# cc-ai/climategan

Measured on AMD Instinct MI355X. Metric: 640x640 images/sec (G+D step): per-domain sample slots per second of the joint Masker+Painter training step (update_G + update_D), global batch 32 per domain, higher is better.
Workload: dtype bf16

## Files before the change

climategan_amd/_lib.py:

```python
import ctypes as C
import os
from pathlib import Path

_HERE = Path(__file__).resolve().parent
LIB_PATH = Path(os.environ["CGAN_LIB"]).resolve() if os.environ.get("CGAN_LIB") else _HERE / "libcgan_hip.so"

CGAN_F16, CGAN_BF16, CGAN_F32 = 0, 1, 2
ACT_NONE, ACT_RELU, ACT_LRELU, ACT_TANH, ACT_SIGMOID = 0, 1, 2, 3, 4
PAD_ZERO, PAD_REFLECT = 0, 1
ABI_VERSION = 1


class ConvDesc(C.Structure):
    _fields_ = [
        ("dtype", C.c_int32), ("n", C.c_int32), ("h_in", C.c_int32), ("w_in", C.c_int32),
        ("c_in", C.c_int32), ("c_out", C.c_int32),
        ("kh", C.c_int32), ("kw", C.c_int32), ("stride", C.c_int32), ("pad", C.c_int32), ("dilation", C.c_int32),
        ("pad_mode", C.c_int32), ("h_out", C.c_int32), ("w_out", C.c_int32), ("in_upsample", C.c_int32),
        ("act", C.c_int32), ("act_slope", C.c_float), ("has_bias", C.c_int32), ("has_residual", C.c_int32),
        ("residual_upsample", C.c_int32),
    ]


class NormStatsDesc(C.Structure):
# ... 131 lines not shown
    "cgan_norm_act_apply": (C.c_int, [_P, _P, _P, _P, C.POINTER(NormStatsDesc), C.c_int32, C.c_float, _P]),
    "cgan_make_m_cond_bwd_nhwc": (C.c_int, [_P, _P, _P, _P, _P, C.c_int32, C.c_int32, C.c_int32, C.c_int32, C.c_int32,
                                            C.c_int32, _P]),
    "cgan_resize_nearest_bwd_nhwc": (C.c_int, [_P, _P, C.c_int32, C.c_int32, C.c_int32, C.c_int32, C.c_int32, C.c_int32,
                                               C.c_int32, C.c_int32, C.c_int32, _P]),
    "cgan_norm_add_act_apply": (C.c_int, [_P, _P, _P, _P, _P, C.POINTER(NormStatsDesc), C.c_int32, C.c_float, _P]),
    "cgan_spade_packed_weight_bytes": (C.c_size_t, [C.POINTER(SpadeDesc)]),
    "cgan_spade_pack_weights": (C.c_int, [_P, _P, _P, _P, _P, _P, _P, C.POINTER(SpadeDesc), _P]),
    "cgan_spade_fused_fwd": (C.c_int, [_P, _P, _P, _P, _P, _P, C.POINTER(SpadeDesc), _P]),
    "cgan_spade_fused_fwd_train": (C.c_int, [_P, _P, _P, _P, _P, _P, _P, C.POINTER(SpadeDesc), _P]),
    "cgan_spectral_norm_workspace_bytes": (C.c_size_t, [C.c_int32, C.c_int32]),
    "cgan_spectral_norm_power_iter": (C.c_int, [_P, _P, _P, _P, C.c_int32, C.c_int32, _P, C.c_size_t, _P]),
    "cgan_spectral_norm_power_iter_batched": (C.c_int, [_P, C.c_int32, C.c_int32, C.c_int32, _P]),
    "cgan_extra_adam_multi_tensor": (C.c_int, [_P, C.c_int32, C.c_int64, C.c_int32, C.c_int32, C.c_int32, C.c_double,
                                               C.c_double, C.c_double, C.c_double, C.c_double, _P]),
    "cgan_grads_nonfinite_check_multi_tensor": (C.c_int, [_P, C.c_int32, C.c_int64, C.c_double, C.c_int32, _P, _P]),
    "cgan_adam_multi_tensor": (C.c_int, [_P, C.c_int32, C.c_int64] + [C.c_double] * 6 + [_P, _P]),
    "cgan_rmsprop_multi_tensor": (C.c_int, [_P, C.c_int32, C.c_int64] + [C.c_double] * 5 + [_P, _P]),
    "cgan_amp_optim_finish": (C.c_int, [_P, C.c_int32, _P, _P]),
    "cgan_nchw_to_nhwc": (C.c_int, [_P, _P, _P, C.c_int32, C.c_int32, C.c_int32, C.c_int32, C.c_int32, C.c_int32, _P]),
    "cgan_nhwc_to_nchw": (C.c_int, [_P, _P, _P, _P, C.c_int32, C.c_int32, C.c_int32, C.c_int32, C.c_int32, C.c_int32, _P]),
    "cgan_resize_nearest_nhwc": (C.c_int, [_P, _P, C.c_int32, C.c_int32, C.c_int32, C.c_int32, C.c_int32, C.c_int32,
                                           C.c_int32, C.c_int32, C.c_int32, _P]),
    "cgan_avgpool3x3s2_nhwc": (C.c_int, [_P, _P, C.c_int32, C.c_int32, C.c_int32, C.c_int32, C.c_int32, _P]),
    "cgan_maxpool3x3s2_nhwc": (C.c_int, [_P, _P, C.c_int32, C.c_int32, C.c_int32, C.c_int32, C.c_int32, _P]),
    "cgan_resize_bilinear_nhwc": (C.c_int, [_P, _P, C.c_int32, C.c_int32, C.c_int32, C.c_int32, C.c_int32, C.c_int32,
                                            C.c_int32, C.c_int32, _P]),
    "cgan_resize_bicubic_nhwc": (C.c_int, [_P, _P, C.c_int32, C.c_int32, C.c_int32, C.c_int32, C.c_int32, C.c_int32,
                                           C.c_int32, _P]),
    "cgan_sumpool2x2_nhwc": (C.c_int, [_P, _P, C.c_int32, C.c_int32, C.c_int32, C.c_int32, C.c_int32, _P]),
    "cgan_reflect_pad_bwd_nhwc": (C.c_int, [_P, _P, C.c_int32, C.c_int32, C.c_int32, C.c_int32, C.c_int32, C.c_int32, _P]),
    "cgan_copy_channels_nhwc": (C.c_int, [_P, _P, C.c_int64, C.c_int32, C.c_int32, C.c_int32, C.c_int32, _P]),
    "cgan_eltwise_nhwc": (C.c_int, [_P, _P, _P, C.c_int32, C.c_int32, C.c_int64, _P]),
    "cgan_fold_bn": (C.c_int, [_P, _P, _P, _P, _P, _P, C.c_float, _P, _P, C.c_int32, C.c_int64, _P]),
    "cgan_act_bwd": (C.c_int, [_P, _P, _P, C.c_int32, C.c_int32, C.c_float, C.c_int64, _P]),
    "cgan_instnorm_act_bwd_workspace_bytes": (C.c_size_t, [C.POINTER(NormStatsDesc)]),
    "cgan_instnorm_act_bwd": (C.c_int, [_P, _P, _P, _P, C.POINTER(NormStatsDesc), C.c_int32, C.c_float, _P, C.c_size_t,
                                        _P]),
    "cgan_spade_bwd_prepare": (C.c_int, [_P, _P, _P, _P, _P, _P, _P, _P, _P, C.POINTER(SpadeDesc), _P]),
    "cgan_spade_hidden_bwd_workspace_bytes": (C.c_size_t, [C.POINTER(SpadeDesc)]),
    "cgan_spade_hidden_bwd": (C.c_int, [_P, _P, _P, _P, _P, _P, _P, _P, C.c_size_t, C.POINTER(SpadeDesc), _P]),
    "cgan_batchnorm_train_stats": (C.c_int, [_P, _P, _P, C.c_float, _P, _P, _P, _P, _P, _P, _P, C.POINTER(NormStatsDesc), _P,
                                             C.c_size_t, _P]),
    "cgan_batchnorm_train_stats_from_partials": (C.c_int, [_P, C.c_int32, _P, _P, C.c_float, _P, _P, _P, _P, _P, _P, _P,
                                                           C.POINTER(NormStatsDesc), _P]),
    "cgan_conv2d_stats_chunk_pixels": (C.c_int32, [C.POINTER(ConvDesc)]),
    "cgan_conv2d_nhwc_fwd_stats": (C.c_int, [_P, _P, _P, _P, _P, C.c_size_t, C.POINTER(ConvDesc), _P]),
    "cgan_bn_train_prepare": (C.c_int, [_P, _P, _P, _P, C.c_float, C.c_float, C.c_int64, _P, _P, _P, _P, _P, C.c_int32, _P]),
    "cgan_batchnorm_act_bwd_workspace_bytes": (C.c_size_t, [C.c_int32]),
    "cgan_batchnorm_act_bwd": (C.c_int, [_P, _P, _P, _P, _P, _P, _P, _P, _P, _P, _P, _P, C.c_int32, C.c_int64, C.c_int32,
                                         C.c_int32, C.c_float, _P, C.c_size_t, _P]),
    "cgan_batchnorm_act_bwd_grouped": (C.c_int, [_P, _P, _P, _P, _P, _P, _P, _P, _P, _P, _P, _P, C.c_int32, C.c_int64,
                                                 C.c_int32, C.c_int32, C.c_int32, C.c_float, _P, C.c_size_t, _P]),
    "cgan_bce_logits_nhwc": (C.c_int, [_P, C.c_int32, C.c_int64, C.c_int32, C.c_float, C.c_float, _P, _P, _P]),
    "cgan_hinge_nhwc": (C.c_int, [_P, C.c_int32, C.c_int64, C.c_int32, C.c_int32, C.c_int32, C.c_float, _P, _P, _P]),
    "cgan_l1_nhwc": (C.c_int, [_P, _P, C.c_int32, C.c_int64, C.c_float, _P, _P, _P]),
    "cgan_mse_const_nhwc": (C.c_int, [_P, C.c_int32, C.c_int64, C.c_int32, C.c_float, C.c_float, _P, _P, _P]),
    "cgan_painter_aux_losses": (C.c_int, [_P, _P, _P, C.c_int32, C.c_int32, C.c_int32, C.c_int32, C.c_float, C.c_float,
                                          C.c_float, C.c_float, _P, _P, _P]),
    "cgan_resize_bicubic_bwd_nhwc": (C.c_int, [_P, _P, C.c_int32, C.c_int32, C.c_int32, C.c_int32, C.c_int32, C.c_int32,
                                               C.c_int32, _P]),
    "cgan_spectral_norm_bwd": (C.c_int, [_P, _P, _P, _P, _P, C.c_int32, C.c_int32, _P, _P]),
    "cgan_painter_heads_fwd": (C.c_int, [_P, _P, _P, _P, _P, C.c_int32, C.c_int32, C.c_int32, C.c_int32, _P]),
    "cgan_painter_heads_bwd": (C.c_int, [_P, _P, _P, _P, C.c_int32, C.c_int32, C.c_int32, C.c_int32, _P]),
    "cgan_diffaug_fwd": (C.c_int, [_P, _P, _P, _P, C.c_int32, C.c_int32, C.c_int32, C.c_int32, C.c_int32, C.c_int32,
                                   C.c_int32, _P, _P]),
    "cgan_diffaug_bwd": (C.c_int, [_P, _P, _P, _P, C.c_int32, C.c_int32, C.c_int32, C.c_int32, C.c_int32, C.c_int32,
                                   C.c_int32, _P, _P]),
    "cgan_painter_heads_diffaug_fwd": (C.c_int, [_P, _P, _P, _P, _P, _P, _P, C.c_int32, C.c_int32, C.c_int32, C.c_int32,
                                                 C.c_int32, C.c_int32, C.c_int32, _P, _P]),
    "cgan_painter_heads_diffaug_bwd": (C.c_int, [_P, _P, _P, _P, _P, _P, C.c_int32, C.c_int32, C.c_int32, C.c_int32,
                                                 C.c_int32, C.c_int32, C.c_int32, _P, _P]),
    "cgan_data_transform": (C.c_int, [_P, _P, C.c_int32, C.c_int32, C.c_int32, C.c_int32, _P, _P, _P, C.c_int32, _P, _P]),
    "cgan_data_source_minmax": (C.c_int, [_P, _P, C.c_int32, C.c_int32, _P, _P]),
    "cgan_data_jitter": (C.c_int, [_P, _P, _P, C.c_int32, C.c_int32, C.c_int32, C.c_int32, _P, _P, _P, _P]),
    "cgan_avgpool3x3s2_bwd_nhwc": (C.c_int, [_P, _P, C.c_int32, C.c_int32, C.c_int32, C.c_int32, C.c_int32, _P]),
    "cgan_maxpool2x2_nhwc": (C.c_int, [_P, _P, C.c_int32, C.c_int32, C.c_int32, C.c_int32, C.c_int32, _P]),
    "cgan_maxpool2x2_bwd_nhwc": (C.c_int, [_P, _P, _P, C.c_int32, C.c_int32, C.c_int32, C.c_int32, C.c_int32, _P]),
    "cgan_maxpool2x2_relu_bwd_nhwc": (C.c_int, [_P, _P, _P, C.c_int32, C.c_int32, C.c_int32, C.c_int32, C.c_int32, _P]),
    "cgan_softmax_nhwc": (C.c_int, [_P, _P, C.c_int32, C.c_int64, C.c_int32, _P]),
    "cgan_softmax_bwd_nhwc": (C.c_int, [_P, _P, _P, C.c_int32, C.c_int64, C.c_int32, _P]),
    "cgan_sigmoid_pair_nhwc": (C.c_int, [_P, _P, C.c_int32, C.c_int64, _P]),
    "cgan_sigmoid_pair_bwd_nhwc": (C.c_int, [_P, _P, _P, C.c_int32, C.c_int64, _P]),
    "cgan_softmax_ce_nhwc": (C.c_int, [_P, _P, C.c_int32, C.c_int64, C.c_int32, C.c_float, _P, _P, _P]),
    "cgan_tv_nhwc": (C.c_int, [_P, C.c_int32, C.c_int32, C.c_int32, C.c_int32, C.c_int32, C.c_float, C.c_float, _P, _P, _P]),
    "cgan_advent_entropy_pair_nhwc": (C.c_int, [_P, _P, _P, C.c_int32, C.c_int64, C.c_int32, C.c_int32, _P]),
    "cgan_entropy_pair_from_nchw": (C.c_int, [_P, _P, _P, C.c_int32, C.c_int32, C.c_int32, C.c_int32, C.c_int32, _P]),
    "cgan_entropy_pair_from_nchw_bwd": (C.c_int, [_P, _P, _P, _P, C.c_int32, C.c_int32, C.c_int32, C.c_int32, C.c_int32, _P]),
    "cgan_advent_entropy_pair_bwd_nhwc": (C.c_int, [_P, _P, _P, _P, C.c_int32, C.c_int64, C.c_int32, C.c_int32, _P]),
    "cgan_entropy_map_nhwc": (C.c_int, [_P, _P, _P, C.c_int32, C.c_int64, C.c_int32, _P]),
    "cgan_entropy_map_bwd_nhwc": (C.c_int, [_P, _P, _P, _P, C.c_int32, C.c_int64, C.c_int32, _P]),
    "cgan_minent_nhwc": (C.c_int, [_P, C.c_int32, C.c_int64, C.c_int32, C.c_int32, C.c_float, C.c_float, _P, _P, _P, _P]),
    "cgan_bce_logits_map_nhwc": (C.c_int, [_P, _P, C.c_int32, C.c_int64, C.c_float, _P, _P, _P]),
    "cgan_ground_intersection_nhwc": (C.c_int, [_P, _P, C.c_int32, C.c_int64, C.c_float, _P, _P]),
    "cgan_affine_sum_nhwc": (C.c_int, [_P, C.c_int32, C.c_int64, C.c_int32, C.c_float, C.c_float, _P, _P, _P]),
    "cgan_resize_bilinear_bwd_workspace_bytes": (C.c_size_t, [C.c_int32] * 4),
    "cgan_resize_bilinear_bwd_nhwc": (C.c_int, [_P, _P] + [C.c_int32] * 8 + [_P, C.c_size_t, _P]),
    "cgan_maxpool3x3s2_bwd_nhwc": (C.c_int, [_P, _P, _P, C.c_int32, C.c_int32, C.c_int32, C.c_int32, C.c_int32, _P]),
    "cgan_add_act_nhwc": (C.c_int, [_P, _P, _P, C.c_int32, C.c_int32, C.c_float, C.c_int64, _P]),
    "cgan_slice_channels_nhwc": (C.c_int, [_P, _P, C.c_int64, C.c_int32, C.c_int32, C.c_int32, _P]),
    "cgan_sigm_loss_workspace_bytes": (C.c_size_t, [C.c_int32, C.c_int32, C.c_int32]),
    "cgan_sigm_loss_nhwc": (C.c_int, [_P, _P, C.c_int32, C.c_int32, C.c_int32, C.c_int32, C.c_float, C.c_int32, C.c_float,
                                      _P, _P, _P, C.c_size_t, _P]),
    "cgan_normalize_u8_workspace_bytes": (C.c_size_t, [C.c_int32]),
    "cgan_normalize_u8_nhwc": (C.c_int, [_P, C.c_int32, _P, C.c_int32, C.c_int32, C.c_int32, C.c_int32, _P, C.c_size_t,
                                         _P]),
# ... 133 lines not shown
```

climategan_amd/autograd.py:

```python
import ctypes as C

import os

import torch

from . import ops


GRAD_SCALE = 1.0


def set_grad_scale(s: float):
    global GRAD_SCALE
    GRAD_SCALE = float(s)


BN_GROUPS = 1


class bn_groups:

    def __init__(self, groups: int):
        self.groups = int(groups)

# ... 87 lines not shown
        ctx.cfg = (c, x_t.shape[1], x_t.shape[2], x_t.shape[3])
        return ops.resize_nearest(ops.NHWC(x_t, c), size, cs_out=cs_out).t

    @staticmethod
    def backward(ctx, dy_t):
        c, h, w, cs = ctx.cfg
        return ops.resize_nearest_bwd(ops.NHWC(dy_t.contiguous(), c), (h, w), cs).t, None, None, None


class ConvFn(torch.autograd.Function):

    @staticmethod
    def forward(ctx, x_t, weight, bias, res_t, packed, cfg, sn):
        x = ops.NHWC(x_t, cfg["c_in"])
        res = ops.NHWC(res_t, weight.shape[0]) if res_t is not None else None
        if cfg.get("mask_input") and (cfg.get("in_upsample", False) or cfg.get("pair_in", False)):
            raise NotImplementedError("ConvFn: mask_input with a folded upsample / a pair map")
        if cfg.get("want_stats") and res is None and cfg["act"] == ops.ACT_NONE and not cfg.get("in_upsample", False):
            y, cfg["stats_out"] = ops.conv2d_with_stats(x, packed, stride=cfg["stride"], pad=cfg["pad"],
                                                        dilation=cfg["dilation"], pad_mode=cfg.get("pad_mode", ops.PAD_ZERO),
                                                        groups=BN_GROUPS)
        else:
            y = ops.conv2d(x, packed, stride=cfg["stride"], pad=cfg["pad"], dilation=cfg["dilation"], act=cfg["act"],
                           slope=cfg["slope"], residual=res, in_upsample=cfg.get("in_upsample", False),
                           residual_upsample=cfg.get("residual_upsample", False),
                           pad_mode=cfg.get("pad_mode", ops.PAD_ZERO))
        ctx.cfg = cfg
        ctx.has_bias = bias is not None
        ctx.has_res = res_t is not None
        ctx.premasked = False
        ctx.sn = None if sn is None else (tuple(sn) if cfg.get("sn_owned") else tuple(t.clone() for t in sn))
        ctx.dgrad = None
        if ctx.needs_input_grad[0] and not cfg.get("pair_in", False):
            ctx.dgrad = ops.dgrad_register(weight, ctx.sn[0] if ctx.sn is not None else None, x_t.dtype, cfg["stride"])
        ctx.save_for_backward(x_t, weight, y.t if cfg["act"] != ops.ACT_NONE else None)
        return y.t

    @staticmethod
    def backward(ctx, dy_t):
        cfg = ctx.cfg
        x_t, weight, y_t = ctx.saved_tensors
        c_out = weight.shape[0]
        ups = cfg.get("in_upsample", False)
        dy = ops.NHWC(dy_t.contiguous(), c_out)
        if y_t is not None and not ctx.premasked:
            dy = ops.act_bwd(ops.NHWC(y_t, c_out), dy, cfg["act"], cfg["slope"])
        sigma = ctx.sn[0] if ctx.sn is not None else None
        dx_t = dres_t = None
        pair = cfg.get("pair_in", False)
        w_eff = torch.cat([weight.detach(), weight.detach()], 1) if pair else weight
        if ctx.needs_input_grad[0]:
            h_in, w_in = (x_t.shape[1] * 2, x_t.shape[2] * 2) if ups else (x_t.shape[1], x_t.shape[2])
            relu_out = ops.NHWC(x_t, cfg["c_in"]) if cfg.get("mask_input") else None
            dx = ops.conv2d_bwd_data(dy, w_eff, (x_t.shape[0], h_in, w_in), stride=cfg["stride"], pad=cfg["pad"],
                                     dilation=cfg["dilation"], sigma=sigma, pad_mode=cfg.get("pad_mode", ops.PAD_ZERO),
                                     prepacked=ctx.dgrad, relu_out=relu_out)
            dx_t = (ops.sumpool2x2(dx) if ups else dx).t
        if ctx.has_res and ctx.needs_input_grad[3]:
            dres_t = (ops.sumpool2x2(dy) if cfg.get("residual_upsample", False) else dy).t
        dw = db = None
        if ctx.needs_input_grad[1] or (ctx.has_bias and ctx.needs_input_grad[2]):
            def wgrad():
                dw, db = ops.conv2d_bwd_weight(ops.NHWC(x_t, cfg["c_in"]), dy, tuple(w_eff.shape), stride=cfg["stride"],
                                               pad=cfg["pad"], dilation=cfg["dilation"], want_bias=ctx.has_bias,
                                               in_upsample=ups, pad_mode=cfg.get("pad_mode", ops.PAD_ZERO))
                if pair:
                    dw = dw[:, :weight.shape[1]] + dw[:, weight.shape[1]:]
                if ctx.sn is not None:
                    dw = ops.spectral_norm_bwd(dw, weight.detach(), ctx.sn[1], ctx.sn[2], ctx.sn[0])
                return dw, db
            dw, db = wgrad()
        return dx_t, dw, db, dres_t, None, None, None


class ConvPassFn(torch.autograd.Function):

    @staticmethod
    def forward(ctx, x_t, weight, bias, packed, cfg):
        x = ops.NHWC(x_t, cfg["c_in"])
        if cfg.get("want_stats") and cfg.get("act", ops.ACT_NONE) != ops.ACT_NONE:
            raise NotImplementedError("ConvPassFn: the statistics epilogue belongs to a conv without an activation")
        if cfg.get("want_stats"):
            y, cfg["stats_out"] = ops.conv2d_with_stats(x, packed, stride=cfg["stride"], pad=cfg["pad"],
                                                        dilation=cfg["dilation"], pad_mode=cfg.get("pad_mode", ops.PAD_ZERO),
                                                        groups=BN_GROUPS)
        else:
            y = ops.conv2d(x, packed, stride=cfg["stride"], pad=cfg["pad"], dilation=cfg["dilation"],
                           act=cfg.get("act", ops.ACT_NONE), slope=cfg.get("slope", 0.0),
                           pad_mode=cfg.get("pad_mode", ops.PAD_ZERO))
        ctx.cfg = cfg
        ctx.has_bias = bias is not None
        ctx.premasked = False
        ctx.dgrad = ops.dgrad_register(weight, None, x_t.dtype, cfg["stride"]) if ctx.needs_input_grad[0] else None
        ctx.save_for_backward(x_t, weight, y.t if cfg.get("act", ops.ACT_NONE) != ops.ACT_NONE else None)
        return y.t, x_t

    @staticmethod
    def backward(ctx, dy_t, dpass_t):
        cfg = ctx.cfg
        x_t, weight, y_t = ctx.saved_tensors
        c_out = weight.shape[0]
        dy = ops.NHWC(dy_t.contiguous(), c_out)
        if y_t is not None and not ctx.premasked:
            dy = ops.act_bwd(ops.NHWC(y_t, c_out), dy, cfg["act"], cfg.get("slope", 0.0))
        dx_t = None
        if ctx.needs_input_grad[0]:
            add = ops.NHWC(dpass_t.contiguous(), cfg["c_in"]) if dpass_t is not None else None
            relu_out = ops.NHWC(x_t, cfg["c_in"]) if cfg.get("mask_input") else None
            dx_t = ops.conv2d_bwd_data(dy, weight, (x_t.shape[0], x_t.shape[1], x_t.shape[2]), stride=cfg["stride"],
                                       pad=cfg["pad"], dilation=cfg["dilation"],
                                       pad_mode=cfg.get("pad_mode", ops.PAD_ZERO), add=add, prepacked=ctx.dgrad,
                                       relu_out=relu_out).t
        dw = db = None
        if ctx.needs_input_grad[1] or (ctx.has_bias and ctx.needs_input_grad[2]):
            dw, db = ops.conv2d_bwd_weight(
                ops.NHWC(x_t, cfg["c_in"]), dy, tuple(weight.shape), stride=cfg["stride"], pad=cfg["pad"],
                dilation=cfg["dilation"], want_bias=ctx.has_bias, pad_mode=cfg.get("pad_mode", ops.PAD_ZERO))
        return dx_t, dw, db, None, None


class InstNormActFn(torch.autograd.Function):

    @staticmethod
    def forward(ctx, x_t, c, eps, act, slope):
        x = ops.NHWC(x_t, c)
        mean, rstd = ops.instnorm_stats(x, eps=eps)
        out = ops.norm_act_apply(x, mean, rstd, act=act, slope=slope)
        ctx.c, ctx.act, ctx.slope = c, act, slope
        ctx.save_for_backward(out.t, rstd)
        return out.t

    @staticmethod
    def backward(ctx, dy_t):
        out_t, rstd = ctx.saved_tensors
        dx = ops.instnorm_act_bwd(ops.NHWC(out_t, ctx.c), ops.NHWC(dy_t.contiguous(), ctx.c), rstd, act=ctx.act,
                                  slope=ctx.slope)
        return dx.t, None, None, None, None


_SPADE_REMAT_GAMMA = os.environ.get("CGAN_SPADE_REMAT_GAMMA") == "1"


_SPADE_FUSED_BWD = os.environ.get("CGAN_SPADE_FUSED_BWD", "1") != "0"


class SpadeFn(torch.autograd.Function):

    @staticmethod
    def forward(ctx, x_t, cond_t, mean, rstd, w_sh, b_sh, w_g, b_g, w_b, b_b, packed, cfg):
        x = ops.NHWC(x_t, cfg["c"])
        cond = ops.NHWC(cond_t, cfg["cond_c"])
        gamma_t = None
        if _SPADE_REMAT_GAMMA or not any(ctx.needs_input_grad):
            y = ops.spade_fused(x, mean, rstd, cond, packed, act=cfg["act"], slope=cfg["slope"],
                                x_upsample=cfg["x_upsample"])
        else:
            y, gamma = ops.spade_fused(x, mean, rstd, cond, packed, act=cfg["act"], slope=cfg["slope"],
                                       x_upsample=cfg["x_upsample"], want_gamma=True)
            gamma_t = gamma.t
        ctx.cfg = cfg
        ctx.save_for_backward(x_t, cond_t, mean, rstd, y.t, w_sh, b_sh, w_g, b_g, w_b, b_b, gamma_t)
        return y.t

    @staticmethod
    def backward(ctx, dy_t):
# ... 121 lines not shown
        ctx.c, ctx.hw = c, (x_t.shape[1], x_t.shape[2])
        return ops.avgpool3x3s2(ops.NHWC(x_t, c)).t

    @staticmethod
    def backward(ctx, dy_t):
        return ops.avgpool3x3s2_bwd(ops.NHWC(dy_t.contiguous(), ctx.c), ctx.hw).t, None


class MaxPool2x2Fn(torch.autograd.Function):

    @staticmethod
    def forward(ctx, x_t, c, mask_input=False):
        ctx.c = c
        ctx.mask_input = bool(mask_input)
        ctx.save_for_backward(x_t)
        return ops.maxpool2x2(ops.NHWC(x_t, c)).t

    @staticmethod
    def backward(ctx, dy_t):
        (x_t,) = ctx.saved_tensors
        return ops.maxpool2x2_bwd(ops.NHWC(x_t, ctx.c), ops.NHWC(dy_t.contiguous(), ctx.c), relu_input=ctx.mask_input).t, None, None


_BN_BWD_READS_OUT = os.environ.get("CGAN_BN_BWD_OUT") == "1"


class BatchNormActFn(torch.autograd.Function):

    @staticmethod
    def forward(ctx, x_t, gamma, beta, running_mean, running_var, c, eps, momentum, act, slope, nbt=None, res_t=None,
                conv_stats=None):
        n, h, w, cs = x_t.shape
        G = BN_GROUPS
        if n % G:
            raise ValueError("BatchNormActFn: batch %d does not divide into %d groups" % (n, G))
        npix = n * h * w // G
        x_t = x_t.contiguous()
        flat = ops.NHWC(x_t.view(G, npix, 1, cs), c)
        if conv_stats is not None and npix % conv_stats.chunk_pixels == 0:
            mean, rstd, mean_f, rstd_f = ops.batchnorm_train_stats_from_partials(
                conv_stats, G, npix, c, gamma, beta, running_mean, running_var, nbt, eps, momentum)
        else:
            mean, rstd, mean_f, rstd_f = ops.batchnorm_train_stats(flat, gamma, beta, running_mean, running_var, nbt, eps,
                                                                   momentum)
        res = None
        if res_t is not None:
            if res_t.shape != x_t.shape:
                raise ValueError("BatchNormActFn: residual %s does not match %s" % (tuple(res_t.shape), tuple(x_t.shape)))
            res = ops.NHWC(res_t.contiguous().view(G, npix, 1, cs), c)
        out = ops.norm_act_apply(flat, mean_f, rstd_f, act=act, slope=slope, residual=res).t.view(n, h, w, cs)
        ctx.cfg = (c, act, slope, G)
        ctx.has_res = res_t is not None
        ctx.premasked = False
        keep_out = res_t is not None or _BN_BWD_READS_OUT
        ctx.save_for_backward(x_t, out if keep_out else None, mean, rstd, gamma,
                              None if keep_out else mean_f, None if keep_out else rstd_f)
        return out

    @staticmethod
    def backward(ctx, dy_t):
        from . import _lib
        lib = _lib.load()
        x_t, out, mean, rstd, gamma, mean_f, rstd_f = ctx.saved_tensors
        c, act, slope, G = ctx.cfg
        if ctx.premasked:
            act = ops.ACT_NONE
        n, h, w, cs = x_t.shape
        nbytes = G * lib.cgan_batchnorm_act_bwd_workspace_bytes(c)
        ws = torch.empty(nbytes, dtype=torch.uint8, device=x_t.device)
        dx = torch.empty_like(x_t)
        want_res = ctx.has_res and ctx.needs_input_grad[11]
        dy_t = dy_t.contiguous()
        if want_res and act == ops.ACT_NONE:
            dres = dy_t
        else:
            dres = torch.empty_like(x_t) if want_res else None
        dg = db = None
        if gamma is not None:
            dg, db = torch.empty((2, c), dtype=torch.float32, device=x_t.device).unbind(0)
        _lib.check(lib.cgan_batchnorm_act_bwd_grouped(
            ops._ptr(x_t), ops._ptr(out), ops._ptr(dy_t), ops._ptr(mean), ops._ptr(rstd), ops._ptr(gamma),
            ops._ptr(mean_f), ops._ptr(rstd_f), ops._ptr(dx), ops._ptr(dg), ops._ptr(db), ops._ptr(dres) if dres is not None and dres is not dy_t else None,
            ops._DT[x_t.dtype], n * h * w, c, G, act, slope, ops._ptr(ws), nbytes, ops._stream()),
            "cgan_batchnorm_act_bwd_grouped")
        return dx, dg, db, None, None, None, None, None, None, None, None, dres, None


def claim_relu_mask(out_t: torch.Tensor) -> bool:
    fn = out_t.grad_fn
    if fn is None:
        return False
    if isinstance(fn, BatchNormActFn._backward_cls):
        if not fn.has_res or fn.cfg[1] != ops.ACT_RELU:
            return False
    elif isinstance(fn, (ConvFn._backward_cls, ConvPassFn._backward_cls)):
        if fn.cfg.get("act", ops.ACT_NONE) != ops.ACT_RELU:
            return False
    else:
        return False
    fn.premasked = True
    return True


def _scaled(dx, c, g):
    return None if dx is None else ops.scale_by_scalar(ops.NHWC(dx, c), g.reshape(1).float().contiguous()).t


class PainterAuxFn(torch.autograd.Function):

    @staticmethod
    def forward(ctx, fake_t, x, m, lam_tv, lam_ctx, lam_rec):
        from . import _lib
        n, h, w = fake_t.shape[0], fake_t.shape[1], fake_t.shape[2]
        x = x.contiguous().float()
        m = m.contiguous().float()
        cnt = float(n * 3 * h * w)
        wh = GRAD_SCALE * lam_tv * 2.0 / (3 * (h - 1) * w) / n
        ww = GRAD_SCALE * lam_tv * 2.0 / (3 * h * (w - 1)) / n
        acc = torch.zeros(3, dtype=torch.float32, device=fake_t.device)
        dfake = torch.empty_like(fake_t) if ctx.needs_input_grad[0] else None
        _lib.check(_lib.load().cgan_painter_aux_losses(ops._ptr(fake_t), ops._ptr(x), ops._ptr(m), ops._DT[fake_t.dtype], n, h, w,
                                                       wh, ww, GRAD_SCALE * lam_ctx / cnt, GRAD_SCALE * lam_rec / cnt,
                                                       ops._ptr(acc), ops._ptr(dfake), ops._stream()), "cgan_painter_aux_losses")
        ctx.save_for_backward(dfake)
        if GRAD_SCALE != 1.0:
            acc = acc / GRAD_SCALE
        ctx.mark_non_differentiable(acc)
        return acc.sum(), acc

    @staticmethod
    def backward(ctx, g, _g_parts):
        (dfake,) = ctx.saved_tensors
        return _scaled(dfake, 3, g), None, None, None, None, None


class ResizeBicubicFn(torch.autograd.Function):

    @staticmethod
# ... 363 lines not shown
```

climategan_amd/csrc/cgan_common.h:

```cpp
#pragma once
#include <hip/hip_runtime.h>
#include <stdarg.h>
#include <stdint.h>
#include <stdio.h>

#include "climategan_hip.h"

void cgan_set_error(const char* fmt, ...);

#define CGAN_REQUIRE(cond, ...)            \
  do {                                     \
    if (!(cond)) {                         \
      cgan_set_error(__VA_ARGS__);         \
      return CGAN_ERR_BAD_ARG;             \
    }                                      \
  } while (0)

#define CGAN_CHECK_LAUNCH(name)                                                    \
  do {                                                                             \
    hipError_t e__ = hipGetLastError();                                            \
    if (e__ != hipSuccess) {                                                       \
      cgan_set_error("%s: HIP launch failed: %s", name, hipGetErrorString(e__));   \
      return CGAN_ERR_HIP;                                                         \
    }                                                                              \
  } while (0)

__device__ __forceinline__ float cgan_res_apply(float v, float r, int mode) { return mode == 2 ? (r > 0.f ? v : 0.f) : v + r; }
__device__ __forceinline__ float cgan_res_apply3(float v, float r, float m) { return m > 0.f ? v + r : 0.f; }

#ifdef CGAN_DEV
#define CGAN_KNOB(type, name, init) type name = init
#define CGAN_DEV_ONLY(...) __VA_ARGS__
#define CGAN_DBG(p) ((p).dbg)
#define CGAN_TSBUF(p) ((p).tsbuf)
#else
#define CGAN_KNOB(type, name, init) [[maybe_unused]] constexpr type name = init
#define CGAN_DEV_ONLY(...)
#define CGAN_DBG(p) 0
#define CGAN_TSBUF(p) ((unsigned long long*)nullptr)
#endif

#ifndef CGAN_NO_NT
#define CGAN_LD_STREAM(p) __builtin_nontemporal_load(p)
#define CGAN_ST_STREAM(v, p) __builtin_nontemporal_store(v, p)
#else
#define CGAN_LD_STREAM(p) (*(p))
#define CGAN_ST_STREAM(v, p) (*(p) = (v))
#endif

typedef _Float16 f16x8 __attribute__((ext_vector_type(8)));
typedef __bf16 bf16x8 __attribute__((ext_vector_type(8)));
typedef float f32x4 __attribute__((ext_vector_type(4)));
typedef unsigned int u32x4 __attribute__((ext_vector_type(4)));
typedef unsigned int u32x2 __attribute__((ext_vector_type(2)));

struct F16 {
  using scalar = _Float16;
  using vec8 = f16x8;
  static constexpr int id = CGAN_F16;
};
struct BF16 {
  using scalar = __bf16;
  using vec8 = bf16x8;
  static constexpr int id = CGAN_BF16;
};

template <typename T> struct Split;
template <> struct Split<F16> {
  static constexpr int NC = 2, NB = 3, NS = 2;
  __host__ __device__ static constexpr int xcomp(int b) { return b == 1 ? 1 : 0; }
  __host__ __device__ static constexpr int wcomp(int b) { return b == 2 ? 1 : 0; }
};
template <> struct Split<BF16> {
  static constexpr int NC = 3, NB = 6, NS = 3;
  __host__ __device__ static constexpr int xcomp(int b) { return b == 1 || b == 4 ? 1 : (b == 2 ? 2 : 0); }
  __host__ __device__ static constexpr int wcomp(int b) { return b < 3 ? 0 : (b < 5 ? 1 : 2); }
};
static inline int cgan_split_blocks(int dtype) { return dtype == CGAN_BF16 ? 6 : 3; }
static inline int cgan_split_store_blocks(int dtype) { return dtype == CGAN_BF16 ? 3 : 2; }

__device__ __forceinline__ f32x4 mfma16(f16x8 a, f16x8 b, f32x4 c) {
// ... 69 lines not shown
```

climategan_amd/csrc/conv_gemm.h:

```cpp
#pragma once
#include "cgan_common.h"

struct ConvGemmArgs {
  const uint16_t* x;
  const u32x4* w;
  const float* bias;
  const uint16_t* res;
  const uint16_t* res2;
  uint16_t* y;
  int n, h_in, w_in, cin_s;
  int cout, cout_s, ctiles, ksteps;
  int kh, kw, stride, pad, dil, pad_mode;
  int h_out, w_out, npix;
  int act, has_res, res_ups;
  float slope;
  float* stats;
};

struct ConvGemmCls {
  int koff;
  int kh, kw;
  int offy, offx;
};
struct ConvGemmExtArgs {
  ConvGemmArgs a;
  int cls_s;
  int ksplit;
  int ks_per;
  float* ws;
  int pair;
  ConvGemmCls cls[4];
};
bool conv_gemm_ext_shape_ok(const ConvGemmArgs& a);
int conv_gemm_splitk_plan(const ConvGemmArgs& a);
size_t conv_gemm_splitk_workspace_bytes(const ConvGemmArgs& a, int ksplit);
int conv_gemm_splitk_launch(const ConvGemmArgs& a, int ksplit, float* ws, int dtype, hipStream_t s);
int conv_gemm_cls_launch(const ConvGemmArgs& a, int cls_s, const ConvGemmCls* cls, int dtype, hipStream_t s);
int conv_gemm_pair_launch(const ConvGemmArgs& a, int dtype, hipStream_t s);

bool conv_gemm_applicable(const CganConvDesc* d);
int conv_gemm_launch(const ConvGemmArgs& a, int dtype, hipStream_t s);
bool conv_gemm_res2_ok(const ConvGemmArgs& a, int dtype);
int conv_gemm_stats_chunk_pixels(const ConvGemmArgs& a, int dtype);
bool conv_gemm_big_ok(const ConvGemmArgs& a);
bool conv1x1_allc_ok(const ConvGemmArgs& a);
int conv1x1_allc_launch(const ConvGemmArgs& a, int dtype, hipStream_t s);
int conv_gemm_big_launch(const ConvGemmArgs& a, int dtype, hipStream_t s);
bool conv_gemm_big_pair_ok(const ConvGemmArgs& a, int dtype);
int conv_gemm_big_pair_launch(const ConvGemmArgs& a, int dtype, hipStream_t s);
bool conv1x1_xres_ok(const ConvGemmArgs& a);
int conv1x1_xres_launch(const ConvGemmArgs& a, int dtype, hipStream_t s);

#ifdef __HIPCC__
typedef float f32x2 __attribute__((ext_vector_type(2)));

__device__ __forceinline__ float row16_sum(float v) {
  v += __builtin_bit_cast(float, __builtin_amdgcn_update_dpp(0, __builtin_bit_cast(int, v), 0x128, 0xf, 0xf, false));
  v += __builtin_bit_cast(float, __builtin_amdgcn_update_dpp(0, __builtin_bit_cast(int, v), 0x124, 0xf, 0xf, false));
  v += __builtin_bit_cast(float, __builtin_amdgcn_update_dpp(0, __builtin_bit_cast(int, v), 0x122, 0xf, 0xf, false));
  v += __builtin_bit_cast(float, __builtin_amdgcn_update_dpp(0, __builtin_bit_cast(int, v), 0x121, 0xf, 0xf, false));
  return v;
}

template <typename T, int WC, int WP>
__device__ __forceinline__ void conv_gemm_stats_epilogue(f32x4 (&acc)[WC][WP], const ConvGemmArgs& p, int cout_base,
                                                         int chunk, int j, int g) {
  if (p.bias) {
#pragma unroll
    for (int c = 0; c < WC; ++c) {
      const int chb = cout_base + c * 16 + 4 * g;
      const f32x4 b = chb < p.cout_s ? *reinterpret_cast<const f32x4*>(p.bias + chb) : (f32x4){0.f, 0.f, 0.f, 0.f};
#pragma unroll
      for (int t = 0; t < WP; ++t) acc[c][t] += b;
    }
  }
  constexpr float inv_cnt = 1.f / (float)(WP * 16);
#pragma unroll
  for (int c = 0; c < WC; ++c) {
    f32x2 vr[WP][2];
#pragma unroll
    for (int t = 0; t < WP; ++t) {
#pragma unroll
      for (int hh = 0; hh < 2; ++hh) {
        float r0, r1;
        unpack2<T>(pack2<T>(acc[c][t][2 * hh], acc[c][t][2 * hh + 1]), r0, r1);
        vr[t][hh] = (f32x2){r0, r1};
      }
    }
    f32x2 s0[2] = {vr[0][0], vr[0][1]};
#pragma unroll
    for (int t = 1; t < WP; ++t) {
      s0[0] += vr[t][0];
      s0[1] += vr[t][1];
    }
    float sm[4], sq[4];
#pragma unroll
    for (int r = 0; r < 4; ++r) sm[r] = row16_sum(s0[r >> 1][r & 1]) * inv_cnt;
    const f32x2 m2[2] = {(f32x2){sm[0], sm[1]}, (f32x2){sm[2], sm[3]}};
    f32x2 s1[2];
#pragma unroll
    for (int hh = 0; hh < 2; ++hh) {
      const f32x2 dv = vr[0][hh] - m2[hh];
      s1[hh] = dv * dv;
    }
#pragma unroll
    for (int t = 1; t < WP; ++t)
#pragma unroll
      for (int hh = 0; hh < 2; ++hh) {
        const f32x2 dv = vr[t][hh] - m2[hh];
        s1[hh] += dv * dv;
      }
#pragma unroll
    for (int r = 0; r < 4; ++r) sq[r] = row16_sum(s1[r >> 1][r & 1]);
    const int ch = cout_base + c * 16 + 4 * g;
    if (j == 0 && ch < p.cout_s) {
      float o[8];
#pragma unroll
      for (int r = 0; r < 4; ++r) {
        o[2 * r] = sm[r];
        o[2 * r + 1] = sq[r];
      }
      float* dst = p.stats + ((size_t)chunk * p.cout_s + ch) * 2;
      *reinterpret_cast<f32x4*>(dst) = (f32x4){o[0], o[1], o[2], o[3]};
      *reinterpret_cast<f32x4*>(dst + 4) = (f32x4){o[4], o[5], o[6], o[7]};
    }
  }
}

template <typename T, int WC, int WP, int PP, bool RES2 = false>
__device__ __forceinline__ void conv_gemm_staged_store(const f32x4 (&acc)[WC][WP], const ConvGemmArgs& p,
                                                       unsigned char* stg, int pix0, int cout_base, const float* bias_ep,
                                                       int lane, int j, int g) {
  constexpr int ROWB = WC * 64 + 16;
  constexpr int CH = WC * 2;
  constexpr int NIT = PP * 16 * CH / 64;
  constexpr int NPASS = WP / PP;
  constexpr int PSTEP = 64 / CH;
  static_assert(64 % CH == 0 && WP % PP == 0, "a lane keeps its channel chunk over the iterations");
  const int qc = lane % CH, pl0 = lane / CH;
  const int ch = cout_base + qc * 8;
  const bool ch_ok = ch < p.cout_s;
  const bool plain = !bias_ep && !p.has_res && p.act == CGAN_ACT_NONE && p.cout == p.cout_s;
  f32x4 bb0 = (f32x4){0.f, 0.f, 0.f, 0.f}, bb1 = bb0;
  if (bias_ep && ch_ok) {
    bb0 = *reinterpret_cast<const f32x4*>(bias_ep + ch);
    bb1 = *reinterpret_cast<const f32x4*>(bias_ep + ch + 4);
  }
  u32x4 rv[NPASS][NIT];
  u32x4 rm[RES2 ? (NPASS > 1 ? 2 : 1) : 1][RES2 ? NIT : 1];
  auto load_rm = [&](int pass, u32x4 (&dst)[RES2 ? NIT : 1]) {
#pragma unroll
    for (int it = 0; it < (RES2 ? NIT : 0); ++it) {
      const int pix = pix0 + pass * PP * 16 + it * PSTEP + pl0;
      dst[it] = (u32x4){0u, 0u, 0u, 0u};
      if (pix < p.npix && ch_ok) dst[it] = CGAN_LD_STREAM(reinterpret_cast<const u32x4*>(p.res2 + (size_t)pix * p.cout_s + ch));
    }
  };
  if (p.has_res) {
#pragma unroll
    for (int pass = 0; pass < NPASS; ++pass)
#pragma unroll
      for (int it = 0; it < NIT; ++it) {
        const int pix = pix0 + pass * PP * 16 + it * PSTEP + pl0;
        rv[pass][it] = (u32x4){0u, 0u, 0u, 0u};
        if (pix < p.npix && ch_ok) {
          size_t rbase;
          if (p.res_ups) {
            const int ox = pix % p.w_out;
            const int r = pix / p.w_out;
            const int oy = r % p.h_out;
            const int nn = r / p.h_out;
            rbase = (((size_t)nn * (p.h_out >> 1) + (oy >> 1)) * (p.w_out >> 1) + (ox >> 1)) * p.cout_s;
          } else {
            rbase = (size_t)pix * p.cout_s;
          }
          rv[pass][it] = CGAN_LD_STREAM(reinterpret_cast<const u32x4*>(p.res + rbase + ch));
        }
      }
    if (RES2 && p.has_res == 3) load_rm(0, rm[0]);
    __builtin_amdgcn_sched_barrier(0);
  }
#pragma unroll
  for (int pass = 0; pass < NPASS; ++pass) {
#pragma unroll
    for (int tt = 0; tt < PP; ++tt)
#pragma unroll
      for (int c = 0; c < WC; ++c)
        *reinterpret_cast<f32x4*>(stg + (tt * 16 + j) * ROWB + c * 64 + g * 16) = acc[c][pass * PP + tt];
    asm volatile("s_waitcnt lgkmcnt(0)" ::: "memory");
    if (RES2 && NPASS > 1 && p.has_res == 3 && pass + 1 < NPASS) {
      __builtin_amdgcn_sched_barrier(0);
      load_rm(pass + 1, rm[(pass + 1) & 1]);
      __builtin_amdgcn_sched_barrier(0);
    }
    if (pass == 0 || (RES2 && p.has_res == 3 && pass >= 2)) __builtin_amdgcn_s_waitcnt(0x0F70);
#pragma unroll
    for (int it = 0; it < NIT; ++it) {
      const int pl = it * PSTEP + pl0;
      const int pix = pix0 + pass * PP * 16 + pl;
      const f32x4 v0 = *reinterpret_cast<const f32x4*>(stg + pl * ROWB + qc * 32);
      const f32x4 v1 = *reinterpret_cast<const f32x4*>(stg + pl * ROWB + qc * 32 + 16);
      float v[8] = {v0[0], v0[1], v0[2], v0[3], v1[0], v1[1], v1[2], v1[3]};
      if (!plain) {
        if (bias_ep) {
#pragma unroll
          for (int r = 0; r < 4; ++r) {
            v[r] += bb0[r];
            v[4 + r] += bb1[r];
          }
        }
        if (RES2 && p.has_res == 3) {
#pragma unroll
          for (int e = 0; e < 4; ++e) {
            float r0, r1, m0, m1;
            unpack2<T>(rv[pass][it][e], r0, r1);
            unpack2<T>(rm[RES2 && NPASS > 1 ? (pass & 1) : 0][RES2 ? it : 0][e], m0, m1);
            v[2 * e] = cgan_res_apply3(v[2 * e], r0, m0);
            v[2 * e + 1] = cgan_res_apply3(v[2 * e + 1], r1, m1);
          }
        } else if (p.has_res) {
#pragma unroll
          for (int e = 0; e < 4; ++e) {
            float r0, r1;
            unpack2<T>(rv[pass][it][e], r0, r1);
            v[2 * e] = cgan_res_apply(v[2 * e], r0, p.has_res);
            v[2 * e + 1] = cgan_res_apply(v[2 * e + 1], r1, p.has_res);
          }
        }
        act_apply_n(v, p.act, p.slope);
        if (p.cout < p.cout_s) {
#pragma unroll
          for (int r = 0; r < 8; ++r)
            if (ch + r >= p.cout) v[r] = 0.f;
        }
      }
      u32x4 o;
#pragma unroll
      for (int e = 0; e < 4; ++e) o[e] = pack2<T>(v[2 * e], v[2 * e + 1]);
      if (pix < p.npix && ch_ok) CGAN_ST_STREAM(o, reinterpret_cast<u32x4*>(p.y + (size_t)pix * p.cout_s + ch));
    }
    asm volatile("s_waitcnt lgkmcnt(0)" ::: "memory");
  }
}
#endif
```

climategan_amd/csrc/conv_gemm.hip:

```cpp
#include "conv_gemm.h"
#include <type_traits>

namespace {

__device__ __attribute__((aligned(16))) unsigned int g_gemm_zeros[4];

constexpr int NSTAGE = 3;
CGAN_KNOB(int, g_gemm_ws, 0);

__device__ __forceinline__ int reflect_i(int i, int n) {
  if (i < 0) i = -i;
  if (i >= n) i = 2 * n - 2 - i;
  return i;
}

template <typename T, int WAVES_C, int WC, int WP, bool REFLECT, int NS = NSTAGE, bool RES2 = false>
__global__ __launch_bounds__(256, 2) void conv_gemm_kernel(ConvGemmArgs p, int npb, int ncb) {
  constexpr int WAVES_P = 4 / WAVES_C;
  constexpr int CT_BLK = WAVES_C * WC;
  constexpr int PT_BLK = WAVES_P * WP;
  constexpr int STAGE_BYTES = (CT_BLK + PT_BLK) * 1024;
  constexpr int W_PER_WAVE = CT_BLK / 4;
  constexpr int P_PER_WAVE = PT_BLK / 4;
  constexpr int DMA_PER_WAVE = W_PER_WAVE + P_PER_WAVE;
  static_assert(CT_BLK % 4 == 0 && PT_BLK % 4 == 0, "tiles must split evenly over the 4 waves");
  extern __shared__ __attribute__((aligned(1024))) unsigned char smem[];

  const int lane = threadIdx.x & 63;
  const int wave = __builtin_amdgcn_readfirstlane(threadIdx.x >> 6);
  const int j = lane & 15;
  const int g = lane >> 4;
  const int wc = wave % WAVES_C, wp = wave / WAVES_C;

  const int xcd = blockIdx.x & 7, slot = blockIdx.x >> 3;
  const int cblk = slot % ncb;
  const int pblk = xcd * ((npb + 7) >> 3) + slot / ncb;
  if (pblk >= npb) return;

  int pbase[P_PER_WAVE], py0[P_PER_WAVE], px0[P_PER_WAVE];
#pragma unroll
  for (int m = 0; m < P_PER_WAVE; ++m) {
    int pix = (pblk * PT_BLK + wave + 4 * m) * 16 + j;
    bool v = pix < p.npix;
    int pc = v ? pix : 0;
    int ox = pc % p.w_out;
    int r = pc / p.w_out;
    int oy = r % p.h_out;
    int nn = r / p.h_out;
    pbase[m] = nn * p.h_in * p.w_in * p.cin_s + g * 8;
    py0[m] = v ? oy * p.stride - p.pad : -(1 << 28);
    px0[m] = ox * p.stride - p.pad;
  }
  const int ccn = p.cin_s >> 5;
  const long zero_off = reinterpret_cast<const unsigned char*>(g_gemm_zeros) - reinterpret_cast<const unsigned char*>(p.x);

  int i_ky = 0, i_kx = 0, i_cc = 0, i_buf = 0;
  auto issue_piece = [&](int piece) {
    unsigned char* buf = smem + i_buf * STAGE_BYTES;
    if (piece < W_PER_WAVE) {
      const int i = wave + 4 * piece;
      const int ct = min(cblk * CT_BLK + i, p.ctiles - 1);
      const u32x4* src = p.w + ((size_t)ct * p.ksteps + (i_ky * p.kw + i_kx) * ccn + i_cc) * 64 + lane;
      __builtin_amdgcn_global_load_lds((const __attribute__((address_space(1))) void*)src,
                                       (__attribute__((address_space(3))) void*)(buf + i * 1024), 16, 0, 0);
    } else {
      const int m = piece - W_PER_WAVE;
      const int i = wave + 4 * m;
      int iy = py0[m] + i_ky * p.dil, ix = px0[m] + i_kx * p.dil;
      bool ok;
// ... 26 lines not shown
    for (int q = 0; q < DMA_PER_WAVE; ++q) issue_piece(q);
    issue_advance();
  };

  f32x4 acc[WC][WP];
#pragma unroll
  for (int c = 0; c < WC; ++c)
#pragma unroll
    for (int t = 0; t < WP; ++t) acc[c][t] = (f32x4){0.f, 0.f, 0.f, 0.f};

  issue();
  if (NS > 2) issue();
  int r_buf = 0;
  for (int ks = 0; ks < p.ksteps; ++ks) {
    asm volatile("s_waitcnt vmcnt(%0) lgkmcnt(0)" ::"n"((NS - 2) * DMA_PER_WAVE) : "memory");
    __builtin_amdgcn_s_barrier();
    const unsigned char* buf = smem + r_buf * STAGE_BYTES;
    u32x4 a[WC], b[WP];
#pragma unroll
    for (int t = 0; t < WP; ++t)
      b[t] = *reinterpret_cast<const u32x4*>(buf + (CT_BLK + wp * WP + t) * 1024 + lane * 16);
#pragma unroll
    for (int c = 0; c < WC; ++c) a[c] = *reinterpret_cast<const u32x4*>(buf + (wc * WC + c) * 1024 + lane * 16);
    constexpr int NM = WC * WP;
    constexpr int GAP = NM / (DMA_PER_WAVE + 1);
    __builtin_amdgcn_sched_barrier(0);
#pragma unroll
    for (int i = 0; i < NM; ++i) {
      const int c = i / WP, t = i % WP;
      acc[c][t] = mfma16(as_vec8<T>(a[c]), as_vec8<T>(b[t]), acc[c][t]);
      if ((i + 1) % GAP == 0 && (i + 1) / GAP <= DMA_PER_WAVE) {
        issue_piece((i + 1) / GAP - 1);
        __builtin_amdgcn_sched_barrier(0);
      }
    }
    issue_advance();
    r_buf = (r_buf + 1 == NS) ? 0 : r_buf + 1;
  }

  constexpr int ROWB = WC * 64 + 16;
  constexpr int PP = (4 * 4 * 16 * ROWB <= NS * STAGE_BYTES && WP % 4 == 0) ? 4
                     : (4 * 2 * 16 * ROWB <= NS * STAGE_BYTES ? 2 : 1);
  static_assert(4 * PP * 16 * ROWB <= NS * STAGE_BYTES, "epilogue staging does not fit");
  static_assert(WP % PP == 0, "WP must be a multiple of PP");
  asm volatile("s_waitcnt vmcnt(0) lgkmcnt(0)" ::: "memory");
  __builtin_amdgcn_s_barrier();
  unsigned char* stg = smem + wave * (PP * 16 * ROWB);
  const int cout_base = (cblk * CT_BLK + wc * WC) * 16;
  const float* bias_ep = p.bias;
  if (p.stats && (pblk * PT_BLK + wp * WP) * 16 < p.npix) {
    conv_gemm_stats_epilogue<T, WC, WP>(acc, p, cout_base, pblk * WAVES_P + wp, j, g);
    if (p.bias) bias_ep = nullptr;
  }
  conv_gemm_staged_store<T, WC, WP, PP, RES2>(acc, p, stg, (pblk * PT_BLK + wp * WP) * 16, cout_base, bias_ep, lane, j, g);
}

template <typename T, int WC, int WP>
__global__ __launch_bounds__(512, 2) void conv_gemm_k64_kernel(ConvGemmArgs p, int npb, int ncb, int tiles_total) {
  constexpr int CT_BLK = 2 * WC, PT_BLK = 2 * WP;
  constexpr int W_BYTES = CT_BLK * 2048, STAGE_BYTES = (CT_BLK + PT_BLK) * 2048;
  constexpr int NS = 3;
  constexpr int W_PER = CT_BLK / 2, P_PER = PT_BLK / 2, PIECES = W_PER + P_PER;
  static_assert(PIECES <= 63, "vmcnt range");
  extern __shared__ __attribute__((aligned(1024))) unsigned char smem[];

  const int lane = threadIdx.x & 63;
  const int wave = __builtin_amdgcn_readfirstlane(threadIdx.x >> 6);
  const int xcd = blockIdx.x & 7, slot = blockIdx.x >> 3, nslot = gridDim.x >> 3;
  const int per = (tiles_total + 7) >> 3;
  const int t0 = xcd * per;
  const int t1 = min(t0 + per, tiles_total);
  const int my_n = (t1 - t0 > slot) ? (t1 - t0 - slot + nslot - 1) / nslot : 0;
  if (my_n <= 0) return;
  const int first = t0 + slot;
  const int cc2n = p.cin_s >> 6;
  const int n_st = p.kh * p.kw * cc2n;
  const int n_it = my_n * n_st;

  if (wave >= 4) {
    const int pw = wave - 4;
    const int half = pw & 1;
    const int ccn = p.cin_s >> 5;
    const long zero_off = reinterpret_cast<const unsigned char*>(g_gemm_zeros) - reinterpret_cast<const unsigned char*>(p.x);
    const int q = lane >> 3;
    const int kchunk = (lane & 7) ^ (4 * half + ((q >> 1) & 3));
    int poff[P_PER];
    unsigned vmask[P_PER];
    const u32x4* wtile[W_PER];
    auto set_tile = [&](int ti) {
      const int gt = first + ti * nslot;
      const int pblk = gt / ncb;
      const int cblk = gt - pblk * ncb;
#pragma unroll
      for (int m = 0; m < W_PER; ++m)
        wtile[m] = p.w + (size_t)min(cblk * CT_BLK + (pw >> 1) + 2 * m, p.ctiles - 1) * p.ksteps * 64 + half * 64 + lane;
#pragma unroll
      for (int m = 0; m < P_PER; ++m) {
        const int pix = (pblk * PT_BLK + (pw >> 1) + 2 * m) * 16 + 8 * half + q;
        const bool v = pix < p.npix;
        const int pc = v ? pix : 0;
        const int ox = pc % p.w_out;
        const int r = pc / p.w_out;
        const int oy = r % p.h_out;
        const int nn = r / p.h_out;
        const int py0 = oy * p.stride - p.pad, px0 = ox * p.stride - p.pad;
        poff[m] = ((nn * p.h_in * p.w_in + py0 * p.w_in + px0) * p.cin_s + kchunk * 8) * 2;
        unsigned mk = 0;
// ... 156 lines not shown
#pragma unroll
        for (int r = 0; r < 4; ++r) {
          v[r] = act_apply(v[r], p.act, p.slope);
          if (ch + r >= p.cout) v[r] = 0.f;
        }
        u32x2 o;
        o.x = pack2<T>(v[0], v[1]);
        o.y = pack2<T>(v[2], v[3]);
        CGAN_ST_STREAM(o, reinterpret_cast<u32x2*>(p.y + (size_t)pix * p.cout_s + ch));
      }
    }
  };

  for (int ti = 0; ti < my_n; ++ti) {
    first_read(ti > 0);
    for (int st = 0; st + 1 < n_st; ++st) {
      step(a0, b0, a1, b1, 1);
      step(a1, b1, a0, b0, 0);
    }
    step(a0, b0, a1, b1, 1);
    step(a1, b1, a0, b0, -1);
    epilogue(ti);
  }
}

template <typename T, int WC, int WP>
int launch_k64(const ConvGemmArgs& a, hipStream_t s) {
  constexpr int CT_BLK = 2 * WC, PT_BLK = 2 * WP;
  constexpr size_t smem = (size_t)3 * (CT_BLK + PT_BLK) * 2048;
  static bool attr_set = false;
  if (!attr_set) {
    hipError_t e = hipFuncSetAttribute(reinterpret_cast<const void*>(&conv_gemm_k64_kernel<T, WC, WP>),
                                       hipFuncAttributeMaxDynamicSharedMemorySize, 160 * 1024);
    if (e != hipSuccess) {
      cgan_set_error("conv_gemm_k64: hipFuncSetAttribute failed: %s", hipGetErrorString(e));
      return CGAN_ERR_HIP;
    }
    attr_set = true;
  }
  const int npb = ceil_div(ceil_div(a.npix, 16), PT_BLK);
  const int ncb = ceil_div(a.ctiles, CT_BLK);
  const int tiles = npb * ncb;
  const int per = ceil_div(tiles, 8);
  const int nslot = per < 32 ? per : 32;
  hipLaunchKernelGGL((conv_gemm_k64_kernel<T, WC, WP>), dim3(8 * nslot), dim3(512), smem, s, a, npb, ncb, tiles);
  return CGAN_OK;
}
bool k64_ok(const ConvGemmArgs& a) {
  return (a.cin_s & 63) == 0 && a.pad_mode != CGAN_PAD_REFLECT && a.kh * a.kw <= 32 &&
         (long)a.n * a.h_in * a.w_in * a.cin_s < (1L << 30) - (1L << 20);
}


template <typename T, int WAVES_C, int WC, int WP, bool REFLECT, int NS = NSTAGE, bool RES2 = false>
int launch_cfg2(const ConvGemmArgs& a, hipStream_t s) {
  constexpr int WAVES_P = 4 / WAVES_C;
  constexpr int CT_BLK = WAVES_C * WC, PT_BLK = WAVES_P * WP;
  constexpr size_t smem = (size_t)NS * (CT_BLK + PT_BLK) * 1024;
  static bool attr_set = false;
  if (!attr_set) {
    hipError_t e = hipFuncSetAttribute(reinterpret_cast<const void*>(&conv_gemm_kernel<T, WAVES_C, WC, WP, REFLECT, NS, RES2>),
                                       hipFuncAttributeMaxDynamicSharedMemorySize, 160 * 1024);
    if (e != hipSuccess) {
      cgan_set_error("conv_gemm: hipFuncSetAttribute failed: %s", hipGetErrorString(e));
      return CGAN_ERR_HIP;
    }
    attr_set = true;
  }
  const int npb = ceil_div(ceil_div(a.npix, 16), PT_BLK);
  const int ncb = ceil_div(a.ctiles, CT_BLK);
  const int grid = ceil_div(npb, 8) * 8 * ncb;
  hipLaunchKernelGGL((conv_gemm_kernel<T, WAVES_C, WC, WP, REFLECT, NS, RES2>), dim3(grid), dim3(256), smem, s, a, npb, ncb);
  return CGAN_OK;
}

template <typename T, int WAVES_C, int WC, int WP, int NS = NSTAGE>
int launch_cfg(const ConvGemmArgs& a, hipStream_t s) {
  return a.pad_mode == CGAN_PAD_REFLECT ? launch_cfg2<T, WAVES_C, WC, WP, true, NS>(a, s)
                                        : launch_cfg2<T, WAVES_C, WC, WP, false, NS>(a, s);
}

CGAN_KNOB(int, g_gemm_cfg, 0);

enum { KIND_PLAIN = 0, KIND_K64_256x128, KIND_K64_128x256, KIND_BIG, KIND_DIRECT, KIND_XRES };
struct Choice {
  int kind;
  int cfg;
};

Choice choose(const ConvGemmArgs& a, bool bf16) {
  const int ptiles = ceil_div(a.npix, 16);
  const bool no_big = g_gemm_ws == 9;
  const bool no_xres = g_gemm_ws == 9 || g_gemm_ws == 12;
  const int ws = (no_big || no_xres || g_gemm_ws == 13 || g_gemm_ws == 14) ? 0 : g_gemm_ws;
  switch (ws) {
    case 5: if (k64_ok(a)) return {KIND_K64_256x128, 0}; break;
    case 6: if (k64_ok(a)) return {KIND_K64_128x256, 0}; break;
    case 8: if (conv_gemm_big_ok(a)) return {KIND_BIG, 0}; break;
    case 10: if (conv1x1_allc_ok(a)) return {KIND_DIRECT, 0}; break;
    case 11: if (conv1x1_xres_ok(a)) return {KIND_XRES, 0}; break;
    default: break;
  }
  const bool automatic = ws == 0 && g_gemm_cfg == 0;
  (void)bf16;
  if (automatic && !no_big && conv1x1_allc_ok(a) && a.ctiles <= 4 && a.npix >= 16384) return {KIND_DIRECT, 0};
  if (automatic && !no_xres && conv1x1_xres_ok(a) && a.ctiles >= 16 && a.npix >= 16384) return {KIND_XRES, 0};
  const bool long_1x1 = a.kh * a.kw == 1 && g_gemm_ws != 13 &&
                        (g_gemm_ws == 14 ? (a.cin_s >= 2048 || (a.cin_s >= 512 && a.ctiles >= 128))
                                         : (a.cin_s >= 1024 || (a.cin_s >= 512 && a.ctiles >= 128)));
  if (automatic && !no_big && conv_gemm_big_ok(a) && a.npix >= 16384 &&
      ((a.cin_s * a.kh * a.kw >= 4096 && a.cin_s >= 512 && !(a.kh * a.kw >= 9 && a.cin_s >= 2048)) || long_1x1))
    return {KIND_BIG, 0};
  if (automatic && k64_ok(a) && a.kh * a.kw >= 9 && a.cin_s >= 512 && a.npix >= 16384) return {KIND_K64_256x128, 0};
  switch (g_gemm_cfg) {
    case 1: return {KIND_PLAIN, 1};
    case 2: if (a.ctiles <= 16) return {KIND_PLAIN, 2}; break;
    case 3: return {KIND_PLAIN, 3};
    case 4: return {KIND_PLAIN, 4};
    case 5: return {KIND_PLAIN, 5};
    default: break;
  }
  if (a.ctiles <= 4) return {KIND_PLAIN, 1};
  if (a.kh * a.kw == 1 && a.ksteps <= 16) return {KIND_PLAIN, 5};
  if (a.ctiles > 8 && a.ctiles <= 16 && ceil_div(ptiles, 8) >= 384) return {KIND_PLAIN, 2};
  if ((long)ceil_div(ptiles, 16) * ceil_div(a.ctiles, 8) >= 384) return {KIND_PLAIN, 3};
  return {KIND_PLAIN, 4};
}

template <typename T>
int launch(const ConvGemmArgs& a, hipStream_t s) {
  const Choice ch = choose(a, std::is_same<T, BF16>::value);
  switch (ch.kind) {
    case KIND_K64_256x128: return launch_k64<T, 8, 4>(a, s);
    case KIND_K64_128x256: return launch_k64<T, 4, 8>(a, s);
    case KIND_BIG: return conv_gemm_big_launch(a, T::id, s);
    case KIND_DIRECT: return conv1x1_allc_launch(a, T::id, s);
    case KIND_XRES: return conv1x1_xres_launch(a, T::id, s);
    default: break;
  }
  switch (ch.cfg) {
    case 1: return launch_cfg<T, 1, 4, 4>(a, s);
    case 2: return launch_cfg<T, 2, 8, 4>(a, s);
    case 3: return launch_cfg<T, 2, 4, 8>(a, s);
    case 5:
      if (a.has_res == 3) return launch_cfg2<T, 2, 4, 4, false, 2, true>(a, s);
      return launch_cfg<T, 2, 4, 4, 2>(a, s);
    default: return launch_cfg<T, 2, 4, 4>(a, s);
  }
}

}

bool conv_gemm_applicable(const CganConvDesc* d) {
  const int cin_s = cgan_cs(d->c_in), cout_s = cgan_cs(d->c_out);
  const long npix = (long)d->n * d->h_out * d->w_out;
  const long in_elems = (long)d->n * d->h_in * d->w_in * cin_s;
  return (cin_s % 32) == 0 && cout_s >= 64 && !d->in_upsample && npix >= 2048 && in_elems < (1L << 31) - (1L << 20) &&
         (long)ceil_div((int)ceil_div((int)npix, 16), 8) * ceil_div(ceil_div(cout_s, 16), 8) >= 128;
}

CGAN_DEV_ONLY(extern "C" void cgan_debug_set_gemm_cfg(int v) { g_gemm_cfg = v; })
CGAN_DEV_ONLY(extern "C" void cgan_debug_set_gemm_ws(int v) { g_gemm_ws = v; })

int conv_gemm_launch(const ConvGemmArgs& a, int dtype, hipStream_t s) {
  return dtype == CGAN_F16 ? launch<F16>(a, s) : launch<BF16>(a, s);
}

bool conv_gemm_res2_ok(const ConvGemmArgs& a, int dtype) {
  const Choice ch = choose(a, dtype == CGAN_BF16);
  return (ch.kind == KIND_PLAIN && ch.cfg == 5 && a.pad_mode != CGAN_PAD_REFLECT) || ch.kind == KIND_BIG;
}

int conv_gemm_stats_chunk_pixels(const ConvGemmArgs& a, int dtype) {
  const Choice ch = choose(a, dtype == CGAN_BF16);
  if (ch.kind == KIND_XRES) return a.npix % 128 == 0 ? 128 : 0;
  if (ch.kind == KIND_BIG) return a.npix % 64 == 0 ? 64 : 0;
  if (ch.kind != KIND_PLAIN) return 0;
  const int ppb = ch.cfg == 3 ? 128 : 64;
  return a.npix % ppb == 0 ? ppb : 0;
}
```

climategan_amd/csrc/conv_mfma.hip:

```cpp
#include "cgan_common.h"
#include "conv3x3_lds.h"
#include "conv_gemm.h"

namespace {

struct ConvParams {
  const uint16_t* x;
  const u32x4* w;
  const float* bias;
  const uint16_t* res;
  const uint16_t* res2;
  uint16_t* y;
  int n, h_in, w_in, hx, wx, cin_s, cin_p, cg;
  int cout, cout_s, ctiles;
  int kh, kw, stride, pad, dil, pad_mode;
  int h_out, w_out, npix;
  int kgroups, ksteps;
  int in_ups, act, has_res, res_ups;
  int in_zs;
  int cls_s;
  int cls_pad;
  float slope;
  float* stats;
  int pair;
// ... 708 lines not shown
}

template <typename T>
__global__ void pack_dgrad_subpixel_kernel(const float* __restrict__ w, const float* __restrict__ sigma,
                                           uint16_t* __restrict__ packed, int c_out, int c_in, int cin_p) {
  const int nq = cin_p / 32, total = 9 * nq * 64;
  const float sig = sigma ? sigma[0] : 1.f;
  for (int idx = blockIdx.x * blockDim.x + threadIdx.x; idx < total; idx += gridDim.x * blockDim.x) {
    const int lane = idx & 63, ks = idx >> 6;
    const int tap = ks / nq, q = ks - tap * nq;
    const int ty = tap / 3, tx = tap - ty * 3;
    const int row = lane & 15, a = row >> 3, b = (row >> 2) & 1, c = row & 3;
    const int ky = a + 3 - 2 * ty, kx = b + 3 - 2 * tx;
    const int k0 = q * 32 + (lane >> 4) * 8;
    uint16_t o[8];
#pragma unroll
    for (int e = 0; e < 8; ++e) {
      const int co = k0 + e;
      float v = 0.f;
      if (co < c_out && c < c_in && ky >= 0 && ky < 4 && kx >= 0 && kx < 4)
        v = __fdiv_rn(w[(((size_t)co * c_in + c) * 4 + ky) * 4 + kx], sig);
      o[e] = bits_of<T>(v);
    }
    u32x4 pk;
    pk[0] = o[0] | ((uint32_t)o[1] << 16);
    pk[1] = o[2] | ((uint32_t)o[3] << 16);
    pk[2] = o[4] | ((uint32_t)o[5] << 16);
    pk[3] = o[6] | ((uint32_t)o[7] << 16);
    reinterpret_cast<u32x4*>(packed)[idx] = pk;
  }
}

namespace {
enum ConvRoute {
  ROUTE_GEMM,
  ROUTE_SPLITK,
  ROUTE_LDS3X3,
  ROUTE_SMALLCIN,
  ROUTE_SUBPIXEL,
  ROUTE_CLS_GEMM,
  ROUTE_PAIR_BIG,
  ROUTE_PAIR_GEMM,
  ROUTE_GENERAL,
};
enum { FWD_PLAIN, FWD_STATS, FWD_PAIR };
enum { RES_NONE = 0, RES_ADD = 1, RES_RELU = 2, RES_ADD_RELU = 3 };

struct ConvPlan {
  ConvRoute route;
  ConvParams p;
  CganConvDesc d;
  int ksplit;
  float* ws;
};

ConvGemmArgs gemm_args(const ConvParams& p) {
  ConvGemmArgs a;
  a.x = p.x; a.w = p.w; a.bias = p.bias; a.res = p.res; a.res2 = p.res2; a.y = p.y;
  a.n = p.n; a.h_in = p.h_in; a.w_in = p.w_in; a.cin_s = p.cin_s;
  a.cout = p.cout; a.cout_s = p.cout_s; a.ctiles = p.ctiles; a.ksteps = p.ksteps;
  a.kh = p.kh; a.kw = p.kw; a.stride = p.stride; a.pad = p.pad; a.dil = p.dil; a.pad_mode = p.pad_mode;
  a.h_out = p.h_out; a.w_out = p.w_out; a.npix = p.npix;
  a.act = p.act; a.has_res = p.has_res; a.res_ups = p.res_ups; a.slope = p.slope;
  a.stats = p.stats;
  return a;
}

Conv3x3LdsArgs lds_args(const ConvPlan& pl) {
  const ConvParams& p = pl.p;
  Conv3x3LdsArgs a;
  a.x = p.x; a.w = p.w; a.bias = p.bias; a.res = p.res; a.y = p.y;
  a.n = p.n; a.h = p.h_out; a.w_ = p.w_out; a.hi = p.h_in; a.wi = p.w_in; a.pad = p.pad;
  a.reflect = p.pad_mode == CGAN_PAD_REFLECT;
  a.hx = p.hx; a.wx = p.wx; a.cin = pl.d.c_in; a.cin_s = p.cin_s; a.cin_p = p.cin_p;
  a.cout = p.cout; a.cout_s = p.cout_s; a.ctiles = p.ctiles; a.ksteps = p.ksteps;
  a.in_ups = p.in_ups; a.act = p.act; a.has_res = p.has_res; a.res_ups = p.res_ups; a.slope = p.slope;
  a.shuffle = 0; a.shuffle_w = 0; a.k = 0; a.stride = 0;
  if (pl.route == ROUTE_SMALLCIN) {
    a.k = p.kh; a.stride = p.stride; a.res_ups = 0;
  } else if (pl.route == ROUTE_SUBPIXEL) {
    a.h = a.hi = p.hx; a.w_ = a.wi = p.wx; a.pad = 1; a.slope = 0.f;
    a.cout = 16; a.cout_s = 16; a.ctiles = 1; a.ksteps = 9 * (a.cin_p / 32);
    a.shuffle = p.h_out; a.shuffle_w = p.w_out;
  }
  return a;
}

void cls_table(const ConvParams& p, ConvGemmCls (&cls)[4]) {
  int koff = 0;
  for (int c = 0; c < p.cls_s * p.cls_s; ++c) {
    const int ca = c / p.cls_s, cb = c % p.cls_s;
    int ry, rx, nty, ntx;
    cls_axis(p.cls_s, p.kh, p.cls_pad, ca, ry, nty);
    cls_axis(p.cls_s, p.kw, p.cls_pad, cb, rx, ntx);
    cls[c] = ConvGemmCls{koff, nty, ntx, (ca - p.cls_pad + ry) / p.cls_s, (cb - p.cls_pad + rx) / p.cls_s};
    if (nty * ntx == 0) cls[c].kh = cls[c].kw = 0;
    koff += cls_ksteps(p.cls_s, p.kh, p.kw, p.cls_pad, p.cg, c);
  }
}

ConvRoute route_stride1(ConvPlan& pl, bool stats, const WsSlot& ws) {
  const ConvParams& p = pl.p;
  const CganConvDesc* d = &pl.d;
  const bool lds = conv3x3_lds_applicable(d);
  const bool prefer_3x3 = lds && p.cin_s < 256 && g_conv_force != 3;
  if ((g_conv_force == 0 || g_conv_force == 3) && !prefer_3x3 && conv_gemm_applicable(d)) return ROUTE_GEMM;
// ... 53 lines not shown
  t.pad = p.pad = pad_t;
  t.h_out = p.h_out = f->h_in; t.w_out = p.w_out = f->w_in;
  p.npix = f->n * f->h_in * f->w_in;
  p.hx = f->h_out; p.wx = f->w_out;
  p.in_zs = f->stride;
  if (f->stride > 1 && f->dilation == 1 && pad_t >= 0 && g_dgrad_zero_insert == 0) {
    p.cls_s = f->stride; p.cls_pad = pad_t; p.in_zs = 1;
    p.h_in = p.hx; p.w_in = p.wx;
  }
  const bool plain = f->stride == 1 && pad_t >= 0 && t.h_in + 2 * pad_t - t.dilation * (t.kh - 1) == t.h_out &&
                     t.w_in + 2 * pad_t - t.dilation * (t.kw - 1) == t.w_out;
  if (res_mode != RES_NONE) {
    CGAN_REQUIRE(plain, "conv2d_nhwc_bwd_data_add / _relu: only for stride-1 'same' convolutions");
    p.has_res = res_mode == RES_ADD_RELU ? RES_ADD : res_mode;
    p.res_ups = 0;
    t.has_residual = 1;
  }
  if (plain) {
    pl.route = route_stride1(pl, false, ws);
    if (res_mode == RES_ADD_RELU && pl.route == ROUTE_GEMM && conv_gemm_res2_ok(gemm_args(p), t.dtype)) p.has_res = 3;
  } else if (dgrad_subpixel(f)) {
    pl.route = ROUTE_SUBPIXEL;
  } else if (p.cls_s && p.cls_s <= 2 && g_conv_force == 0 && p.cin_p == p.cin_s && conv_gemm_ext_shape_ok(gemm_args(p)) &&
             p.cout_s >= 64) {
    pl.route = ROUTE_CLS_GEMM;
  } else {
    pl.route = ROUTE_GENERAL;
  }
  return CGAN_OK;
}

int route_family(ConvRoute r) {
  switch (r) {
    case ROUTE_GENERAL: return CGAN_CONV_KERNEL_GENERAL;
    case ROUTE_LDS3X3: case ROUTE_SMALLCIN: case ROUTE_SUBPIXEL: return CGAN_CONV_KERNEL_LDS3X3;
    default: return CGAN_CONV_KERNEL_GEMM;
  }
}

int stats_chunk_pixels(const ConvPlan& pl) {
  const CganConvDesc& d = pl.d;
  if (pl.route != ROUTE_GEMM || d.has_residual || d.act != CGAN_ACT_NONE || d.in_upsample) return 0;
  static const float bias_present = 0.f;
  ConvGemmArgs a = gemm_args(pl.p);
  a.bias = d.has_bias ? &bias_present : nullptr;
  return conv_gemm_stats_chunk_pixels(a, d.dtype);
}

int launch_plan(const ConvPlan& pl, hipStream_t s, const char* what) {
  const ConvParams& p = pl.p;
  const int dt = pl.d.dtype;
  int rc = CGAN_OK;
  switch (pl.route) {
    case ROUTE_GEMM: rc = conv_gemm_launch(gemm_args(p), dt, s); break;
    case ROUTE_SPLITK: rc = conv_gemm_splitk_launch(gemm_args(p), pl.ksplit, pl.ws, dt, s); break;
    case ROUTE_LDS3X3: case ROUTE_SUBPIXEL: rc = conv3x3_lds_launch(lds_args(pl), dt, s); break;
    case ROUTE_SMALLCIN: rc = conv_smallcin_launch(lds_args(pl), dt, s); break;
    case ROUTE_CLS_GEMM: {
      ConvGemmCls cls[4];
      cls_table(p, cls);
      rc = conv_gemm_cls_launch(gemm_args(p), p.cls_s, cls, dt, s);
      break;
    }
    case ROUTE_PAIR_BIG: rc = conv_gemm_big_pair_launch(gemm_args(p), dt, s); break;
    case ROUTE_PAIR_GEMM: rc = conv_gemm_pair_launch(gemm_args(p), dt, s); break;
    case ROUTE_GENERAL:
      if (dt == CGAN_F16) launch<F16>(p, s);
      else launch<BF16>(p, s);
      break;
  }
  if (rc != CGAN_OK) return rc;
  CGAN_CHECK_LAUNCH(what);
  return CGAN_OK;
}

void bind(ConvParams& p, const void* x, const void* w, const float* bias, const void* res, void* y) {
  p.x = (const uint16_t*)x; p.w = (const u32x4*)w; p.bias = bias; p.res = (const uint16_t*)res; p.y = (uint16_t*)y;
}
}

extern "C" int cgan_conv2d_nhwc_fwd(const void* x, const void* packed_w, const float* bias_padded, const void* residual,
                                    void* y, const CganConvDesc* d, void* stream) {
  CGAN_REQUIRE(x && packed_w && y, "conv2d_nhwc_fwd: null pointer");
  ConvPlan pl;
  int rc = plan_fwd(pl, d, FWD_PLAIN, ws_lookup(stream));
  if (rc != CGAN_OK) return rc;
  CGAN_REQUIRE(!d->has_bias || bias_padded, "conv2d_nhwc_fwd: has_bias but bias is null");
  CGAN_REQUIRE(!d->has_residual || residual, "conv2d_nhwc_fwd: has_residual but residual is null");
  bind(pl.p, x, packed_w, d->has_bias ? bias_padded : nullptr, residual, y);
  return launch_plan(pl, (hipStream_t)stream, "conv2d_nhwc_fwd");
}

extern "C" int cgan_conv2d_nhwc_fwd_pair(const void* x3, const void* packed_w3, const float* bias_padded,
                                         const void* residual3, void* y3, const CganConvDesc* d, void* stream) {
  CGAN_REQUIRE(x3 && packed_w3 && y3, "conv2d_nhwc_fwd_pair: null pointer");
  ConvPlan pl;
  int rc = plan_fwd(pl, d, FWD_PAIR, WsSlot{});
  if (rc != CGAN_OK) return rc;
  CGAN_REQUIRE(!d->has_bias || bias_padded, "conv2d_nhwc_fwd_pair: has_bias but bias is null");
  CGAN_REQUIRE(!d->has_residual || residual3, "conv2d_nhwc_fwd_pair: has_residual but residual is null");
  bind(pl.p, x3, packed_w3, d->has_bias ? bias_padded : nullptr, residual3, y3);
  return launch_plan(pl, (hipStream_t)stream, "conv2d_nhwc_fwd_pair");
}

extern "C" int32_t cgan_conv2d_stats_chunk_pixels(const CganConvDesc* d) {
  ConvPlan pl;
  if (plan_fwd(pl, d, FWD_STATS, WsSlot{}) != CGAN_OK) return 0;
// ... 47 lines not shown
  const ConvParams& p = pl.p;
  const CganConvDesc& t = pl.d;
  hipStream_t s = (hipStream_t)stream;
  if (pl.route == ROUTE_SUBPIXEL) {
    const int cin_p = lds_args(pl).cin_p;
    const int tot = 9 * (cin_p / 32) * 64;
    if (fwd->dtype == CGAN_F16)
      hipLaunchKernelGGL(pack_dgrad_subpixel_kernel<F16>, dim3(ceil_div(tot, 256)), dim3(256), 0, s, w_oihw, sigma,
                         (uint16_t*)packed, fwd->c_out, fwd->c_in, cin_p);
    else
      hipLaunchKernelGGL(pack_dgrad_subpixel_kernel<BF16>, dim3(ceil_div(tot, 256)), dim3(256), 0, s, w_oihw, sigma,
                         (uint16_t*)packed, fwd->c_out, fwd->c_in, cin_p);
  } else if (p.cls_s) {
    int max_ks = 1;
    for (int c = 0; c < p.cls_s * p.cls_s; ++c) {
      const int k = cls_ksteps(p.cls_s, p.kh, p.kw, p.cls_pad, p.cg, c);
      max_ks = k > max_ks ? k : max_ks;
    }
    const int tot = p.ctiles * max_ks * 64;
    const dim3 grid(ceil_div(tot, 256) < 1024 ? ceil_div(tot, 256) : 1024, p.cls_s * p.cls_s);
    if (fwd->dtype == CGAN_F16)
      hipLaunchKernelGGL(pack_dgrad_classes_kernel<F16>, grid, dim3(256), 0, s, w_oihw, sigma, (uint16_t*)packed, t.c_out,
                         t.c_in, p.cin_p, t.kh, t.kw, p.ctiles, p.cls_s, p.cls_pad);
    else
      hipLaunchKernelGGL(pack_dgrad_classes_kernel<BF16>, grid, dim3(256), 0, s, w_oihw, sigma, (uint16_t*)packed, t.c_out,
                         t.c_in, p.cin_p, t.kh, t.kw, p.ctiles, p.cls_s, p.cls_pad);
  } else {
    const int total = p.ctiles * p.ksteps * 64;
    const int blocks = ceil_div(total, 256) < 2048 ? ceil_div(total, 256) : 2048;
    if (fwd->dtype == CGAN_F16)
      hipLaunchKernelGGL(pack_conv_weight_kernel<F16>, dim3(blocks), dim3(256), 0, s, w_oihw, (const float*)nullptr, sigma,
                         (uint16_t*)packed, (float*)nullptr, t.c_out, t.c_in, p.cin_p, t.kh, t.kw, p.ctiles, p.ksteps, 1);
    else
      hipLaunchKernelGGL(pack_conv_weight_kernel<BF16>, dim3(blocks), dim3(256), 0, s, w_oihw, (const float*)nullptr, sigma,
                         (uint16_t*)packed, (float*)nullptr, t.c_out, t.c_in, p.cin_p, t.kh, t.kw, p.ctiles, p.ksteps, 1);
  }
  CGAN_CHECK_LAUNCH("conv2d_pack_weight_dgrad");
  return CGAN_OK;
}

static int kernel_kind_impl(const CganConvDesc* d, int32_t bwd_data, const WsSlot& ws) {
  ConvPlan pl;
  const int rc = bwd_data ? plan_dgrad(pl, d, RES_NONE, ws) : plan_fwd(pl, d, FWD_PLAIN, ws);
  return rc != CGAN_OK ? rc : route_family(pl.route);
}

extern "C" int cgan_conv2d_kernel_kind_on(const CganConvDesc* d, int32_t bwd_data, void* stream) {
  return kernel_kind_impl(d, bwd_data, ws_lookup(stream));
}
extern "C" int cgan_conv2d_kernel_kind(const CganConvDesc* d, int32_t bwd_data) {
  return kernel_kind_impl(d, bwd_data, WsSlot{0, nullptr, nullptr, ws_max_bytes()});
}

static int bwd_data_impl(const void* dy, const void* packed_w_dgrad, const void* res, const void* relu_out, void* dx,
                         const CganConvDesc* fwd, void* stream, int res_mode) {
  CGAN_REQUIRE(dy && packed_w_dgrad && dx, "conv2d_nhwc_bwd_data: null pointer");
  ConvPlan pl;
  int rc = plan_dgrad(pl, fwd, res_mode, ws_lookup(stream));
  if (rc != CGAN_OK) return rc;
  bind(pl.p, dy, packed_w_dgrad, nullptr, res, dx);
  if (pl.p.has_res == 3) pl.p.res2 = (const uint16_t*)relu_out;
  rc = launch_plan(pl, (hipStream_t)stream, "conv2d_nhwc_bwd_data");
  if (rc != CGAN_OK || res_mode != RES_ADD_RELU || pl.p.has_res == 3) return rc;
  return cgan_act_bwd(relu_out, dx, dx, fwd->dtype, CGAN_ACT_RELU, 0.f,
                      (int64_t)fwd->n * fwd->h_in * fwd->w_in * cgan_cs(fwd->c_in), stream);
}

extern "C" int cgan_conv2d_nhwc_bwd_data(const void* dy, const void* packed_w_dgrad, void* dx, const CganConvDesc* fwd,
                                         void* stream) {
  return bwd_data_impl(dy, packed_w_dgrad, nullptr, nullptr, dx, fwd, stream, RES_NONE);
}

extern "C" int cgan_conv2d_nhwc_bwd_data_relu(const void* dy, const void* packed_w_dgrad, const void* relu_out, void* dx,
                                              const CganConvDesc* fwd, void* stream) {
  CGAN_REQUIRE(relu_out != nullptr, "conv2d_nhwc_bwd_data_relu: null pointer");
  return bwd_data_impl(dy, packed_w_dgrad, relu_out, nullptr, dx, fwd, stream, RES_RELU);
}

extern "C" int cgan_conv2d_nhwc_bwd_data_add_relu(const void* dy, const void* packed_w_dgrad, const void* dx_add,
                                                  const void* relu_out, void* dx, const CganConvDesc* fwd, void* stream) {
  CGAN_REQUIRE(dx_add != nullptr && relu_out != nullptr, "conv2d_nhwc_bwd_data_add_relu: null pointer");
  return bwd_data_impl(dy, packed_w_dgrad, dx_add, relu_out, dx, fwd, stream, RES_ADD_RELU);
}

extern "C" int cgan_conv2d_nhwc_bwd_data_add(const void* dy, const void* packed_w_dgrad, const void* dx_add, void* dx,
                                             const CganConvDesc* fwd, void* stream) {
  CGAN_REQUIRE(dx_add != nullptr, "conv2d_nhwc_bwd_data_add: null pointer");
  return bwd_data_impl(dy, packed_w_dgrad, dx_add, nullptr, dx, fwd, stream, RES_ADD);
}
```

climategan_amd/csrc/train_ops.hip:

```cpp
#include "cgan_common.h"

namespace {

__host__ __device__ inline int grid_for_n(long total) {
  long g = (total + 255) / 256;
  return (int)(g < 1 ? 1 : (g > 8192 ? 8192 : g));
}

__device__ __forceinline__ float act_grad_from_out(float out, int act, float slope) {
  switch (act) {
    case CGAN_ACT_RELU: return out > 0.f ? 1.f : 0.f;
    case CGAN_ACT_LRELU: return out > 0.f ? 1.f : slope;
    case CGAN_ACT_TANH: return 1.f - out * out;
    case CGAN_ACT_SIGMOID: return out * (1.f - out);
    default: return 1.f;
  }
}

template <typename T>
__global__ void act_bwd_kernel(const uint16_t* __restrict__ out, const uint16_t* dy, uint16_t* dx, int act, float slope,
                               long groups) {
  for (long i = (long)blockIdx.x * blockDim.x + threadIdx.x; i < groups; i += (long)gridDim.x * blockDim.x) {
    const u32x4 o = CGAN_LD_STREAM(reinterpret_cast<const u32x4*>(out) + i);
    const u32x4 g = CGAN_LD_STREAM(reinterpret_cast<const u32x4*>(dy) + i);
// ... 216 lines not shown
    CGAN_ST_STREAM(oxh, reinterpret_cast<u32x4*>(xhat) + i);
    CGAN_ST_STREAM(odx, reinterpret_cast<u32x4*>(dxhat) + i);
    uint16_t* row = dgb + pix * cs2;
    if (cg * 8 + 8 <= c) {
      *reinterpret_cast<u32x4*>(row + cg * 8) = odg;
    } else {
#pragma unroll
      for (int e = 0; e < 8; ++e)
        if (cg * 8 + e < c) row[cg * 8 + e] = (uint16_t)((odg[e >> 1] >> ((e & 1) * 16)) & 0xffffu);
    }
    if (cg * 8 + 8 <= c && (c & 3) == 0) {
      const u32x4 obt = {pack2<T>(dbeta[0], dbeta[1]), pack2<T>(dbeta[2], dbeta[3]), pack2<T>(dbeta[4], dbeta[5]),
                         pack2<T>(dbeta[6], dbeta[7])};
      if ((c & 7) == 0) {
        *reinterpret_cast<u32x4*>(row + c + cg * 8) = obt;
      } else {
        *reinterpret_cast<u32x2*>(row + c + cg * 8) = (u32x2){obt[0], obt[1]};
        *reinterpret_cast<u32x2*>(row + c + cg * 8 + 4) = (u32x2){obt[2], obt[3]};
      }
    } else {
#pragma unroll
      for (int e = 0; e < 8; ++e)
        if (cg * 8 + e < c) row[c + cg * 8 + e] = bits_of<T>(dbeta[e]);
    }
  }
}

__global__ void bn_train_prepare_kernel(const float* __restrict__ mean, const float* __restrict__ rstd,
                                        const float* __restrict__ gamma, const float* __restrict__ beta, float eps,
                                        float momentum, float count, float* __restrict__ running_mean,
                                        float* __restrict__ running_var, float* __restrict__ mean_out,
                                        float* __restrict__ rstd_out, long long* __restrict__ num_batches_tracked, int c,
                                        int cs) {
  const int ch = blockIdx.x * blockDim.x + threadIdx.x;
  if (ch == 0 && num_batches_tracked) *num_batches_tracked += 1;
  if (ch >= cs) return;
  float m = 0.f, r = 0.f;
  if (ch < c) {
    const float mu = mean[ch], rs = rstd[ch];
    r = rs * (gamma ? gamma[ch] : 1.f);
    m = mu - ((beta && r != 0.f) ? beta[ch] / r : 0.f);
    if (running_mean) {
      const float var_b = 1.f / (rs * rs) - eps;
      const float var_u = count > 1.f ? var_b * count / (count - 1.f) : var_b;
      running_mean[ch] = (1.f - momentum) * running_mean[ch] + momentum * mu;
      running_var[ch] = (1.f - momentum) * running_var[ch] + momentum * var_u;
    }
  }
  mean_out[ch] = m;
  rstd_out[ch] = r;
}

constexpr int BN_BWD_MAX_CHUNKS = 512;
template <int MASK>
__device__ __forceinline__ float bn_bwd_act_grad(float ov, float xv, float fm, float fr, float gneg) {
  if (MASK == 0) return 1.f;
  if (MASK == 1) return ov > 0.f ? 1.f : gneg;
  return (xv - fm) * fr > 0.f ? 1.f : gneg;
}

template <typename T, int MASK>
__global__ __launch_bounds__(256) void bn_bwd_reduce_kernel(const uint16_t* __restrict__ x, const uint16_t* __restrict__ out,
                                                            const uint16_t* __restrict__ dy, const float* __restrict__ mean,
                                                            const float* __restrict__ rstd, const float* __restrict__ fmean,
                                                            const float* __restrict__ frstd, float* __restrict__ partial,
                                                            uint16_t* __restrict__ dz_out, long npix, int cs, int ppb,
                                                            float gneg) {
  extern __shared__ __attribute__((aligned(16))) float sm[];
  const int cg_total = cs / 8;
  const int cgb = cg_total < 256 ? cg_total : 256;
  const int PL = 256 / cgb;
  const int cg0 = blockIdx.y * cgb;
  const size_t gofs = (size_t)blockIdx.z * npix * cs;
  x += gofs; dy += gofs;
  if (MASK == 1) out += gofs;
  if (dz_out) dz_out += gofs;
  mean += (size_t)blockIdx.z * cs; rstd += (size_t)blockIdx.z * cs;
  if (MASK == 2) { fmean += (size_t)blockIdx.z * cs; frstd += (size_t)blockIdx.z * cs; }
  partial += (size_t)blockIdx.z * gridDim.x * cs * 2;
  const long p0 = (long)blockIdx.x * ppb, p1 = min(npix, p0 + ppb);
  const int t = threadIdx.x, cgl = t % cgb, pl = t / cgb;
  const int cg = cg0 + cgl;
  float s1[8], s2[8];
#pragma unroll
  for (int e = 0; e < 8; ++e) s1[e] = s2[e] = 0.f;
  if (pl < PL && cg < cg_total) {
    float mu[8], rs[8], fm[8], fr[8];
#pragma unroll
    for (int e = 0; e < 8; ++e) {
      mu[e] = mean[cg * 8 + e];
      rs[e] = rstd[cg * 8 + e];
      fm[e] = MASK == 2 ? fmean[cg * 8 + e] : 0.f;
      fr[e] = MASK == 2 ? frstd[cg * 8 + e] : 0.f;
    }
    const uint16_t* xp = x + cg * 8;
    const uint16_t* op = out + cg * 8;
    const uint16_t* gp = dy + cg * 8;
#pragma unroll 2
    for (long p = p0 + pl; p < p1; p += PL) {
      const size_t off = (size_t)p * cs;
      const u32x4 vx = CGAN_LD_STREAM(reinterpret_cast<const u32x4*>(xp + off));
      u32x4 vo = {0, 0, 0, 0};
      if (MASK == 1) vo = CGAN_LD_STREAM(reinterpret_cast<const u32x4*>(op + off));
      const u32x4 vg = CGAN_LD_STREAM(reinterpret_cast<const u32x4*>(gp + off));
      u32x4 z;
#pragma unroll
      for (int e = 0; e < 4; ++e) {
        float xv[2], ov[2], gv[2], dzv[2];
        unpack2<T>(vx[e], xv[0], xv[1]);
        unpack2<T>(vo[e], ov[0], ov[1]);
        unpack2<T>(vg[e], gv[0], gv[1]);
#pragma unroll
// ... 44 lines not shown
    const float* rows = partial + ((size_t)grp * chunks * cs + ch) * 2;
    float a = 0.f, b = 0.f;
    for (int k0 = kl; k0 < chunks; k0 += 256) {
      float2 v[8];
#pragma unroll
      for (int j = 0; j < 8; ++j) {
        const int k = k0 + 32 * j;
        v[j] = k < chunks ? *reinterpret_cast<const float2*>(rows + (size_t)k * cs * 2) : make_float2(0.f, 0.f);
      }
#pragma unroll
      for (int j = 0; j < 8; ++j) {
        a += v[j].x;
        b += v[j].y;
      }
    }
#pragma unroll
    for (int off = 32; off >= 8; off >>= 1) {
      a += __shfl_down(a, off, 64);
      b += __shfl_down(b, off, 64);
    }
    if (lane < 8) {
      red[grp][wave][chl][0] = a;
      red[grp][wave][chl][1] = b;
    }
  }
  __syncthreads();
  if (threadIdx.x >= 8) return;
  float dg_sum = 0.f, db_sum = 0.f;
  for (int grp = 0; grp < groups; ++grp) {
    float s1 = 0.f, s2 = 0.f;
#pragma unroll
    for (int w = 0; w < 4; ++w) {
      s1 += red[grp][w][chl][0];
      s2 += red[grp][w][chl][1];
    }
    float A = 0.f, B = 0.f, C = 0.f;
    if (ch < c) {
      dg_sum += s2;
      db_sum += s1;
      const float rs = rstd[ch], mu = mean[ch];
      A = rs * (gamma ? gamma[ch] : 1.f);
      const float m1 = s1 * inv_count, m2 = s2 * inv_count;
      B = -A * rs * m2;
      C = A * (mu * rs * m2 - m1);
    }
    coef[ch] = A;
    coef[cs + ch] = B;
    coef[2 * cs + ch] = C;
    mean += cs; rstd += cs; coef += 3 * (size_t)cs;
  }
  if (ch < c) {
    if (dgamma) dgamma[ch] = dg_sum;
    if (dbeta) dbeta[ch] = db_sum;
  }
}

template <typename T, int MASK>
__global__ __launch_bounds__(256) void bn_bwd_apply_kernel(const uint16_t* __restrict__ x, const uint16_t* __restrict__ out,
                                                           const uint16_t* __restrict__ dy, const float* __restrict__ coef,
                                                           const float* __restrict__ fmean, const float* __restrict__ frstd,
                                                           uint16_t* __restrict__ dx, uint16_t* __restrict__ dz_out,
                                                           long npix, int cs, float gneg) {
  const int cg_total = cs / 8;
  const int tpp = cg_total < 256 ? cg_total : 256;
  const int rows = 256 / tpp;
  const int cgl = threadIdx.x % tpp, prow = threadIdx.x / tpp;
  if (prow >= rows) return;
  {
    const size_t gofs = (size_t)blockIdx.y * npix * cs;
    x += gofs; dy += gofs; dx += gofs;
    if (MASK == 1) out += gofs;
    if (dz_out) dz_out += gofs;
    coef += (size_t)blockIdx.y * 3 * cs;
    if (MASK == 2) { fmean += (size_t)blockIdx.y * cs; frstd += (size_t)blockIdx.y * cs; }
  }
  for (int cg = cgl; cg < cg_total; cg += tpp) {
    float A[8], B[8], Cc[8], fm[8], fr[8];
#pragma unroll
    for (int e = 0; e < 8; ++e) {
      A[e] = coef[cg * 8 + e];
      B[e] = coef[cs + cg * 8 + e];
      Cc[e] = coef[2 * cs + cg * 8 + e];
      fm[e] = MASK == 2 ? fmean[cg * 8 + e] : 0.f;
      fr[e] = MASK == 2 ? frstd[cg * 8 + e] : 0.f;
    }
#pragma unroll 2
    for (long p = (long)blockIdx.x * rows + prow; p < npix; p += (long)gridDim.x * rows) {
      const size_t off = (size_t)p * cs + cg * 8;
      const u32x4 vx = CGAN_LD_STREAM(reinterpret_cast<const u32x4*>(x + off));
      u32x4 vo = {0, 0, 0, 0};
      if (MASK == 1) vo = CGAN_LD_STREAM(reinterpret_cast<const u32x4*>(out + off));
      const u32x4 vg = CGAN_LD_STREAM(reinterpret_cast<const u32x4*>(dy + off));
      u32x4 r, z;
#pragma unroll
      for (int e = 0; e < 4; ++e) {
        float xv[2], ov[2], gv[2], res[2], dzv[2];
        unpack2<T>(vx[e], xv[0], xv[1]);
        unpack2<T>(vo[e], ov[0], ov[1]);
        unpack2<T>(vg[e], gv[0], gv[1]);
#pragma unroll
        for (int hh = 0; hh < 2; ++hh) {
          const int k = 2 * e + hh;
          dzv[hh] = gv[hh] * bn_bwd_act_grad<MASK>(ov[hh], xv[hh], fm[k], fr[k], gneg);
          res[hh] = A[k] * dzv[hh] + B[k] * xv[hh] + Cc[k];
        }
        r[e] = pack2<T>(res[0], res[1]);
// ... 102 lines not shown
  hipLaunchKernelGGL(in_bwd_finalize_kernel, dim3(d->n * cs / 8), dim3(256), 0, s, (const float*)partial, sums,
                     d->n, cs, chunks);
  {
    const int tpp = cg_total < 256 ? cg_total : 256, rows = 256 / tpp;
    long blocks = (d->hw + (long)rows * 4 - 1) / ((long)rows * 4);
    const long cap = 8192 / d->n > 0 ? 8192 / d->n : 1;
    blocks = blocks < 1 ? 1 : (blocks > cap ? cap : blocks);
    DISPATCH_T(d->dtype, in_bwd_apply_kernel, dim3((unsigned)blocks, d->n), dim3(256), 0, s, (const uint16_t*)out,
               (const uint16_t*)dy, rstd, (const float*)workspace, (uint16_t*)dx, d->hw, cs, d->c, act, act_slope);
  }
  CGAN_CHECK_LAUNCH("instnorm_act_bwd");
  return CGAN_OK;
}

extern "C" int cgan_spade_bwd_prepare(const void* dy, const void* y, const void* x, const float* mean, const float* rstd,
                                      const void* gamma, void* dgb, void* xhat, void* dxhat, const CganSpadeDesc* d,
                                      void* stream) {
  CGAN_REQUIRE(d && dy && y && x && mean && rstd && gamma && dgb && xhat && dxhat, "spade_bwd_prepare: null pointer");
  CGAN_REQUIRE(d->dtype == CGAN_F16 || d->dtype == CGAN_BF16, "spade_bwd_prepare: bad dtype %d", d->dtype);
  CGAN_REQUIRE(d->n > 0 && d->h > 0 && d->w > 0 && d->c > 0, "spade_bwd_prepare: bad shape");
  CGAN_REQUIRE(d->act == CGAN_ACT_NONE || d->act == CGAN_ACT_LRELU, "spade_bwd_prepare: Unsupported activation: %d", d->act);
  if (d->x_upsample) CGAN_REQUIRE((d->h % 2) == 0 && (d->w % 2) == 0, "spade_bwd_prepare: x_upsample needs even h/w");
  const int cs = cgan_cs(d->c), cs2 = cgan_cs(2 * d->c);
  const long npix = (long)d->n * d->h * d->w;
  hipStream_t s = (hipStream_t)stream;
  if (cs2 != 2 * d->c) {
    hipError_t e = hipMemsetAsync(dgb, 0, (size_t)npix * cs2 * 2, s);
    if (e != hipSuccess) {
      cgan_set_error("spade_bwd_prepare: hipMemsetAsync failed: %s", hipGetErrorString(e));
      return CGAN_ERR_HIP;
    }
  }
  const long groups = npix * (cs / 8);
  DISPATCH_T(d->dtype, spade_bwd_prepare_kernel, dim3(grid_for_n(groups)), dim3(256), 0, s, (const uint16_t*)dy,
             (const uint16_t*)y, (const uint16_t*)x, mean, rstd, (const uint16_t*)gamma, (uint16_t*)dgb, (uint16_t*)xhat,
             (uint16_t*)dxhat, d->h, d->w, d->c, cs, cs2, d->x_upsample, d->act, d->act_slope, groups);
  CGAN_CHECK_LAUNCH("spade_bwd_prepare");
  return CGAN_OK;
}

extern "C" int cgan_bn_train_prepare(const float* batch_mean, const float* batch_rstd, const float* gamma,
                                     const float* beta, float eps, float momentum, int64_t count, float* running_mean,
                                     float* running_var, float* mean_out, float* rstd_out,
                                     int64_t* num_batches_tracked, int32_t c, void* stream) {
  CGAN_REQUIRE(batch_mean && batch_rstd && mean_out && rstd_out, "bn_train_prepare: null pointer");
  CGAN_REQUIRE((running_mean == nullptr) == (running_var == nullptr), "bn_train_prepare: running stats go together");
  CGAN_REQUIRE(c > 0 && count > 0, "bn_train_prepare: bad shape");
  const int cs = cgan_cs(c);
  hipLaunchKernelGGL(bn_train_prepare_kernel, dim3((cs + 255) / 256), dim3(256), 0, (hipStream_t)stream, batch_mean,
                     batch_rstd, gamma, beta, eps, momentum, (float)count, running_mean, running_var, mean_out, rstd_out,
                     (long long*)num_batches_tracked, c, cs);
  CGAN_CHECK_LAUNCH("bn_train_prepare");
  return CGAN_OK;
}

extern "C" size_t cgan_batchnorm_act_bwd_workspace_bytes(int32_t c) {
  return c > 0 ? (size_t)cgan_cs(c) * (3 + 2 * (size_t)BN_BWD_MAX_CHUNKS) * sizeof(float) : 0;
}

extern "C" int cgan_batchnorm_act_bwd(const void* x, const void* out, const void* dy, const float* batch_mean,
                                      const float* batch_rstd, const float* gamma, const float* fold_mean,
                                      const float* fold_rstd, void* dx, float* dgamma, float* dbeta, void* dz_out,
                                      int32_t dtype, int64_t npix, int32_t c, int32_t act, float act_slope,
                                      void* workspace, size_t workspace_bytes, void* stream) {
  return cgan_batchnorm_act_bwd_grouped(x, out, dy, batch_mean, batch_rstd, gamma, fold_mean, fold_rstd, dx, dgamma, dbeta,
                                        dz_out, dtype, npix, c, 1, act, act_slope, workspace, workspace_bytes, stream);
}

extern "C" int cgan_batchnorm_act_bwd_grouped(const void* x, const void* out, const void* dy, const float* batch_mean,
                                              const float* batch_rstd, const float* gamma, const float* fold_mean,
                                              const float* fold_rstd, void* dx, float* dgamma, float* dbeta,
                                              void* dz_out, int32_t dtype, int64_t npix_total, int32_t c, int32_t groups,
                                              int32_t act, float act_slope, void* workspace, size_t workspace_bytes,
                                              void* stream) {
  CGAN_REQUIRE(x && dy && batch_mean && batch_rstd && dx && workspace, "batchnorm_act_bwd: null pointer");
  CGAN_REQUIRE(out || !dz_out, "batchnorm_act_bwd: a fused residual (dz_out) needs out");
  CGAN_REQUIRE(out || act == CGAN_ACT_NONE || (fold_mean && fold_rstd),
               "batchnorm_act_bwd: without out the activation mask needs fold_mean / fold_rstd");
  CGAN_REQUIRE(dtype == CGAN_F16 || dtype == CGAN_BF16, "batchnorm_act_bwd: bad dtype %d", dtype);
  CGAN_REQUIRE(groups >= 1 && groups <= 16 && npix_total > 0 && c > 0 && npix_total % groups == 0,
               "batchnorm_act_bwd: bad shape (the pixel count must divide into the groups)");
  CGAN_REQUIRE(act == CGAN_ACT_NONE || act == CGAN_ACT_RELU || act == CGAN_ACT_LRELU,
               "batchnorm_act_bwd: Unsupported activation: %d", act);
  CGAN_REQUIRE(workspace_bytes >= (size_t)groups * cgan_batchnorm_act_bwd_workspace_bytes(c),
               "batchnorm_act_bwd: workspace too small");
  const long npix = npix_total / groups;
  const int cs = cgan_cs(c);
  hipStream_t s = (hipStream_t)stream;
  float* coef = (float*)workspace;
  float* partial = coef + (size_t)groups * 3 * cs;
  const int cg_total = cs / 8;
  const int cgb = cg_total < 256 ? cg_total : 256;
  const int PL = 256 / cgb;
  const int cgblocks = ceil_div(cg_total, cgb);
  long chunks = BN_BWD_MAX_CHUNKS / cgblocks;
  if (chunks < 1) chunks = 1;
  long ppb = (npix + chunks - 1) / chunks;
  if (ppb < 8 * PL) ppb = 8 * PL;
  chunks = (npix + ppb - 1) / ppb;
  const size_t smem = (size_t)PL * cgb * 8 * 2 * sizeof(float);
  const int mask = act == CGAN_ACT_NONE ? 0 : (out ? 1 : 2);
  const float gneg = act == CGAN_ACT_RELU ? 0.f : act_slope;
  uint16_t* dz_early = (mask == 1 && dz_out && act == CGAN_ACT_RELU) ? (uint16_t*)dz_out : nullptr;
#define BN_BWD_REDUCE(M)                                                                                              \
  DISPATCH_T2(dtype, bn_bwd_reduce_kernel, M, dim3((unsigned)chunks, cgblocks, groups), dim3(256), smem, s,           \
              (const uint16_t*)x, (const uint16_t*)out, (const uint16_t*)dy, batch_mean, batch_rstd, fold_mean,       \
              fold_rstd, partial, dz_early, (long)npix, cs, (int)ppb, gneg)
  if (mask == 0) { BN_BWD_REDUCE(0); } else if (mask == 1) { BN_BWD_REDUCE(1); } else { BN_BWD_REDUCE(2); }
#undef BN_BWD_REDUCE
  hipLaunchKernelGGL(bn_bwd_finalize_kernel, dim3(cs / 8), dim3(256), 0, s, (const float*)partial, (int)chunks,
                     batch_mean, batch_rstd, gamma, 1.f / (float)npix, coef, dgamma, dbeta, (int)c, cs, (int)groups);
  const int tpp = cg_total < 256 ? cg_total : 256;
  const int rows = 256 / tpp;
  long blocks = (npix + (long)rows * 4 - 1) / ((long)rows * 4);
  blocks = blocks < 1 ? 1 : (blocks > 4096 / groups ? 4096 / groups : blocks);
#define BN_BWD_APPLY(M)                                                                                               \
  DISPATCH_T2(dtype, bn_bwd_apply_kernel, M, dim3((unsigned)blocks, groups), dim3(256), 0, s, (const uint16_t*)x,     \
              (const uint16_t*)out, (const uint16_t*)dy, (const float*)coef, fold_mean, fold_rstd, (uint16_t*)dx,     \
              (uint16_t*)dz_out, (long)npix, cs, gneg)
  if (dz_early) {
    DISPATCH_T2(dtype, bn_bwd_apply_kernel, 0, dim3((unsigned)blocks, groups), dim3(256), 0, s, (const uint16_t*)x,
                (const uint16_t*)nullptr, (const uint16_t*)dz_early, (const float*)coef, fold_mean, fold_rstd,
                (uint16_t*)dx, (uint16_t*)nullptr, (long)npix, cs, gneg);
  } else if (mask == 0) { BN_BWD_APPLY(0); } else if (mask == 1) { BN_BWD_APPLY(1); } else { BN_BWD_APPLY(2); }
#undef BN_BWD_APPLY
  CGAN_CHECK_LAUNCH("batchnorm_act_bwd");
  return CGAN_OK;
}

extern "C" int cgan_spectral_norm_bwd(float* grad_w, const float* w_bar, const float* u, const float* v,
                                      const float* sigma, int32_t rows, int32_t cols, float* workspace,
                                      void* stream) {
  CGAN_REQUIRE(grad_w && w_bar && u && v && sigma && workspace, "spectral_norm_bwd: null pointer");
  CGAN_REQUIRE(rows > 0 && cols > 0, "spectral_norm_bwd: bad shape");
  hipStream_t s = (hipStream_t)stream;
  const long numel = (long)rows * cols;
  int g = grid_for_n(numel);
  if (g > SN_BWD_ROWS) g = SN_BWD_ROWS;
  hipLaunchKernelGGL(sn_bwd_dot_kernel, dim3(g), dim3(256), 0, s, (const float*)grad_w, w_bar, workspace, numel);
  hipLaunchKernelGGL(sn_bwd_apply_kernel, dim3(grid_for_n(numel)), dim3(256), 0, s, grad_w, u, v, sigma,
                     (const float*)workspace, g, cols, numel);
  CGAN_CHECK_LAUNCH("spectral_norm_bwd");
  return CGAN_OK;
}
```

climategan_amd/deeplab/resnet101_v3.py:

```python
import torch.nn as nn

from .. import functional as Fn
from .. import ops
from ..norms import DEFAULT_COMPUTE_DTYPE, _PackCache, conv_bn_forward, needs_grad


FUSE_RESIDUAL_GRADIENT = True


class Bottleneck(nn.Module):
    expansion = 4

    def __init__(self, inplanes, planes, stride=1, dilation=1, downsample=None, BatchNorm=None):
        super().__init__()
        self.conv1 = nn.Conv2d(inplanes, planes, kernel_size=1, bias=False)
        self.bn1 = BatchNorm(planes)
        self.conv2 = nn.Conv2d(planes, planes, kernel_size=3, stride=stride, dilation=dilation, padding=dilation,
                               bias=False)
        self.bn2 = BatchNorm(planes)
        self.conv3 = nn.Conv2d(planes, planes * 4, kernel_size=1, bias=False)
        self.bn3 = BatchNorm(planes * 4)
        self.relu = nn.ReLU(inplace=True)
        self.downsample = downsample
        self.stride = stride
        self.dilation = dilation
        self._c = [_PackCache() for _ in range(4)]

    def forward_nhwc(self, x, sole_consumer=False):
        residual = x
        if FUSE_RESIDUAL_GRADIENT and self.bn1.training and needs_grad(self, x.t):
            out, residual = conv_bn_forward(self.conv1, self.bn1, self._c[0], x, act=ops.ACT_RELU, passthrough=True,
                                            sole_consumer=sole_consumer)
            x = residual
        else:
            out = conv_bn_forward(self.conv1, self.bn1, self._c[0], x, act=ops.ACT_RELU)
        out = conv_bn_forward(self.conv2, self.bn2, self._c[1], out, act=ops.ACT_RELU)
        if self.downsample is not None:
            residual = conv_bn_forward(self.downsample[0], self.downsample[1], self._c[3], x)
        return conv_bn_forward(self.conv3, self.bn3, self._c[2], out, act=ops.ACT_RELU, residual=residual)


class ResNet(nn.Module):

    def __init__(self, block, layers, output_stride, BatchNorm, verbose=0, no_init=False):
        self.inplanes = 64
        self.verbose = verbose
        super().__init__()
        blocks = [1, 2, 4]
        if output_stride == 16:
            strides, dilations = [1, 2, 2, 1], [1, 1, 1, 2]
        elif output_stride == 8:
            strides, dilations = [1, 2, 1, 1], [1, 1, 2, 4]
        else:
            raise NotImplementedError
        self.conv1 = nn.Conv2d(3, 64, kernel_size=7, stride=2, padding=3, bias=False)
        self.bn1 = BatchNorm(64)
        self.relu = nn.ReLU(inplace=True)
        self.maxpool = nn.MaxPool2d(kernel_size=3, stride=2, padding=1)
        self.layer1 = self._make_layer(block, 64, layers[0], strides[0], dilations[0], BatchNorm)
        self.layer2 = self._make_layer(block, 128, layers[1], strides[1], dilations[1], BatchNorm)
        self.layer3 = self._make_layer(block, 256, layers[2], strides[2], dilations[2], BatchNorm)
        self.layer4 = self._make_MG_unit(block, 512, blocks, strides[3], dilations[3], BatchNorm)
        self.compute_dtype = DEFAULT_COMPUTE_DTYPE
        self.pair_precision = False
        self._stem = _PackCache()

    def _downsample(self, block, planes, stride, BatchNorm):
        if stride != 1 or self.inplanes != planes * block.expansion:
            return nn.Sequential(nn.Conv2d(self.inplanes, planes * block.expansion, kernel_size=1, stride=stride, bias=False),
                                 BatchNorm(planes * block.expansion))
        return None

    def _make_layer(self, block, planes, blocks, stride=1, dilation=1, BatchNorm=None):
        layers = [block(self.inplanes, planes, stride, dilation, self._downsample(block, planes, stride, BatchNorm), BatchNorm)]
        self.inplanes = planes * block.expansion
        for _ in range(1, blocks):
            layers.append(block(self.inplanes, planes, dilation=dilation, BatchNorm=BatchNorm))
        return nn.Sequential(*layers)

    def _make_MG_unit(self, block, planes, blocks, stride=1, dilation=1, BatchNorm=None):
        layers = [block(self.inplanes, planes, stride, dilation=blocks[0] * dilation,
                        downsample=self._downsample(block, planes, stride, BatchNorm), BatchNorm=BatchNorm)]
        self.inplanes = planes * block.expansion
        for i in range(1, len(blocks)):
            layers.append(block(self.inplanes, planes, stride=1, dilation=blocks[i] * dilation, BatchNorm=BatchNorm))
        return nn.Sequential(*layers)

    def forward_nhwc(self, x: ops.NHWC):
        x = conv_bn_forward(self.conv1, self.bn1, self._stem, x, act=ops.ACT_RELU)
        x = Fn.maxpool3x3s2(x)
        sole = False
        for b in self.layer1:
# ... 23 lines not shown
```

climategan_amd/norms.py:

```python
import torch
import torch.nn as nn

from . import ops

DEFAULT_COMPUTE_DTYPE = torch.float16


def _grad_guard(module: nn.Module):
    if torch.is_grad_enabled() and any(p.requires_grad for p in module.parameters()):
        raise NotImplementedError(
            "climategan_amd: only the forward (inference) path is implemented in HIP so far; call under "
            "torch.no_grad() (the reference's infer_all does, trainer.py:217) or set requires_grad=False")


def needs_grad(module: nn.Module, *tensors) -> bool:
    if not torch.is_grad_enabled():
        return False
    return any(t is not None and t.requires_grad for t in tensors) or any(p.requires_grad for p in module.parameters())


def _conv_train(x: ops.NHWC, weight, bias, packed, sn, stride, pad, dilation, kw) -> ops.NHWC:
    from .autograd import ConvFn

    pad_mode = kw.get("pad_mode", ops.PAD_ZERO)
    if pad_mode == ops.PAD_REFLECT and kw.get("in_upsample"):
        raise NotImplementedError("climategan_amd: reflect padding on a folded upsample has no backward kernel")
    res = kw.get("residual")
    cfg = dict(c_in=x.c, stride=stride, pad=pad, dilation=dilation, act=kw.get("act", ops.ACT_NONE),
               slope=kw.get("slope", 0.2), in_upsample=bool(kw.get("in_upsample", False)),
               residual_upsample=bool(kw.get("residual_upsample", False)), pad_mode=pad_mode,
               sn_owned=bool(kw.get("sn_owned", False)), pair_in=bool(kw.get("pair_in", False)),
               want_stats=bool(kw.get("want_stats", False)))
    y_t = ConvFn.apply(x.t, weight, bias, res.t if res is not None else None, packed, cfg, sn)
    if kw.get("want_stats"):
        return ops.NHWC(y_t, weight.shape[0]), cfg.get("stats_out")
    return ops.NHWC(y_t, weight.shape[0])


class _PackCache:

    _plain = {}

    def __init__(self):
        self.key = None
        self.value = None
        self._plain_src = None

    @staticmethod
    def _key_of(params, dtype):
        return tuple((p.data_ptr(), p._version, p.dtype, str(p.device)) if torch.is_tensor(p) else p
                     for p in params if p is not None) + (dtype,)

    def get(self, params, dtype, build):
        key = self._key_of(params, dtype)
        if key != self.key:
            self.value = build()
            self.key = key
        return self.value

    def get_plain(self, weight, bias, dtype):
        import weakref

        key = self._key_of((weight, bias, "plain"), dtype)
        if key == self.key:
            return self.value
        self._plain_src = (weakref.ref(weight), weakref.ref(bias) if bias is not None else None, dtype)
        _PackCache._plain[id(self)] = weakref.ref(self)
        _PackCache.repack_stale(dtype, weight.device)
        return self.value

    @staticmethod
    def repack_stale(dtype, device) -> int:
        self = _PackCache
        stale = []
        for cid, ref in list(_PackCache._plain.items()):
            c = ref()
            src = c._plain_src if c is not None else None
            w = src[0]() if src is not None else None
            if c is None or w is None:
                del _PackCache._plain[cid]
                continue
            b = src[1]() if src[1] is not None else None
            if src[2] != dtype or w.device != device:
                continue
            k = self._key_of((w, b, "plain"), dtype)
# ... 92 lines not shown
        pw = self.packed(x.t.dtype)
        pad = conv_kwargs.pop("pad", m.padding[0])
        if self.trainable and needs_grad(self, x.t):
            snap, self._sn_snapshot = self._sn_snapshot, None
            if self._pre_used and snap is not None:
                sn = snap
                conv_kwargs = dict(conv_kwargs, sn_owned=True)
            else:
                sn = (self._sigma, getattr(m, self.name + "_u").data, getattr(m, self.name + "_v").data)
            return _conv_train(x, getattr(m, self.name + "_bar"), m.bias, pw, sn, m.stride[0], pad, m.dilation[0],
                               conv_kwargs)
        return ops.conv2d(x, pw, stride=m.stride[0], pad=pad, dilation=m.dilation[0], **conv_kwargs)


class PlainConv(nn.Module):

    def __init__(self, conv: nn.Conv2d):
        super().__init__()
        self.conv = conv
        self._cache = _PackCache()

    def packed(self, dtype):
        c = self.conv
        return self._cache.get((c.weight, c.bias), dtype,
                               lambda: ops.pack_conv_weight(c.weight.data, c.bias.data if c.bias is not None else None,
                                                            dtype))


def conv_forward(conv: nn.Module, cache: _PackCache, x: ops.NHWC, **kw) -> ops.NHWC:
    if isinstance(conv, SpectralNorm):
        return conv(x, **kw)
    trainable = kw.pop("trainable", False)
    if not trainable:
        _grad_guard(conv)
    if trainable and needs_grad(conv, x.t):
        pw = cache.get_plain(conv.weight, conv.bias, x.t.dtype)
        return _conv_train(x, conv.weight, conv.bias, pw, None, conv.stride[0], conv.padding[0], conv.dilation[0], kw)
    pair = isinstance(x, ops.PairMap)
    pw = cache.get((conv.weight, conv.bias) + (("pair",) if pair else ()), x.t.dtype,
                   lambda: ops.pack_conv_weight(conv.weight.data, conv.bias.data if conv.bias is not None else None,
                                                x.t.dtype, pair=pair))
    if trainable and needs_grad(conv, x.t):
        return _conv_train(x, conv.weight, conv.bias, pw, None, conv.stride[0], conv.padding[0], conv.dilation[0], kw)
    return ops.conv2d(x, pw, stride=conv.stride[0], pad=conv.padding[0], dilation=conv.dilation[0], **kw)


FUSE_BN_RESIDUAL = True
import os as _os
FUSE_BN_STATS = _os.environ.get("CGAN_FUSE_BN_STATS", "1") != "0"
FUSE_RELU_MASK = _os.environ.get("CGAN_FUSE_RELU_MASK", "1") != "0"


def conv_bn_forward(conv: nn.Conv2d, bn, cache: _PackCache, x: ops.NHWC, pad_mode=ops.PAD_ZERO, pad=None, **kw) -> ops.NHWC:
    train_bn = bn is not None and bn.training
    grad = needs_grad(conv, x.t) or (bn is not None and needs_grad(bn))
    p = conv.padding[0] if pad is None else pad
    if not train_bn and not grad:
        pair = isinstance(x, ops.PairMap)

        def build():
            if bn is None:
                return ops.pack_conv_weight(conv.weight.data, conv.bias.data if conv.bias is not None else None, x.t.dtype,
                                            pair=pair)
            w, b = ops.fold_bn(conv.weight.data, conv.bias.data if conv.bias is not None else None,
                               bn.weight.data if bn.affine else None, bn.bias.data if bn.affine else None,
                               bn.running_mean, bn.running_var, bn.eps)
            return ops.pack_conv_weight(w, b, x.t.dtype, pair=pair)

        params = [conv.weight, conv.bias]
        if bn is not None:
            params += [bn.weight, bn.bias, bn.running_mean, bn.running_var]
        if pair:
            params = params + ["pair"]
        pw = cache.get(params, x.t.dtype, build)
        return ops.conv2d(x, pw, stride=conv.stride[0], pad=p, dilation=conv.dilation[0], pad_mode=pad_mode, **kw)

    if bn is not None and not bn.training:
        raise NotImplementedError("climategan_amd: an eval-mode BatchNorm under autograd has no HIP backward (the "
                                  "reference trains with BatchNorm in training mode)")
    from .autograd import BatchNormActFn

    act, slope, residual = kw.pop("act", ops.ACT_NONE), kw.pop("slope", 0.2), kw.pop("residual", None)
    sole_consumer = kw.pop("sole_consumer", False)
    if kw.get("in_upsample") or kw.get("residual_upsample"):
        raise NotImplementedError("conv_bn_forward: folded upsamples are not used on the training path")
    pw = cache.get_plain(conv.weight, conv.bias, x.t.dtype)
    passthrough = None
    if kw.pop("passthrough", False):
        from .autograd import ConvPassFn

        assert bn is not None and residual is None
        pcfg = dict(c_in=x.c, stride=conv.stride[0], pad=p, dilation=conv.dilation[0], pad_mode=pad_mode, want_stats=FUSE_BN_STATS)
        if sole_consumer and FUSE_RELU_MASK:
            from .autograd import claim_relu_mask
            pcfg["mask_input"] = claim_relu_mask(x.t)
        y_t, pass_t = ConvPassFn.apply(x.t, conv.weight, conv.bias, pw, pcfg)
        y, passthrough = ops.NHWC(y_t, conv.weight.shape[0]), ops.NHWC(pass_t, x.c)
        conv_stats = pcfg.get("stats_out")
    if bn is None:
        return _conv_train(x, conv.weight, conv.bias, pw, None, conv.stride[0], p, conv.dilation[0],
                           dict(act=act, slope=slope, residual=residual, pad_mode=pad_mode))
    if passthrough is None:
        conv_stats = None
        if FUSE_BN_STATS:
            y, conv_stats = _conv_train(x, conv.weight, conv.bias, pw, None, conv.stride[0], p, conv.dilation[0],
                                        dict(pad_mode=pad_mode, want_stats=True))
        else:
            y = _conv_train(x, conv.weight, conv.bias, pw, None, conv.stride[0], p, conv.dilation[0], dict(pad_mode=pad_mode))
    if residual is not None and not FUSE_BN_RESIDUAL:
        from . import functional as Fn
        out_t = BatchNormActFn.apply(y.t, bn.weight if bn.affine else None, bn.bias if bn.affine else None,
                                     bn.running_mean, bn.running_var, y.c, bn.eps,
                                     bn.momentum if bn.momentum is not None else 0.1, ops.ACT_NONE, slope,
                                     bn.num_batches_tracked if bn.track_running_stats else None)
        return Fn.add_act(ops.NHWC(out_t, y.c), residual, act, slope)
    if residual is not None and (residual.c != y.c or residual.t.shape != y.t.shape):
        raise ValueError("conv_bn_forward: residual %s does not match the conv output %s"
                         % (tuple(residual.t.shape), tuple(y.t.shape)))
    out_t = BatchNormActFn.apply(y.t, bn.weight if bn.affine else None, bn.bias if bn.affine else None, bn.running_mean,
                                 bn.running_var, y.c, bn.eps, bn.momentum if bn.momentum is not None else 0.1, act,
                                 slope, bn.num_batches_tracked if bn.track_running_stats else None,
                                 residual.t if residual is not None else None, conv_stats)
    return ops.NHWC(out_t, y.c) if passthrough is None else (ops.NHWC(out_t, y.c), passthrough)


class SPADE(nn.Module):

    def __init__(self, param_free_norm_type, kernel_size, norm_nc, cond_nc):
        super().__init__()
        if param_free_norm_type == "instance":
            self.param_free_norm = nn.InstanceNorm2d(norm_nc, affine=False)
        elif param_free_norm_type == "batch":
            self.param_free_norm = nn.BatchNorm2d(norm_nc, affine=False)
        else:
            raise ValueError("%s is not a recognized param-free norm type in SPADE" % param_free_norm_type)
        self.param_free_norm_type = param_free_norm_type
        nhidden = 128
        pw = kernel_size // 2
        self.mlp_shared = nn.Sequential(nn.Conv2d(cond_nc, nhidden, kernel_size=kernel_size, padding=pw), nn.ReLU())
        self.mlp_gamma = nn.Conv2d(nhidden, norm_nc, kernel_size=kernel_size, padding=pw)
        self.mlp_beta = nn.Conv2d(nhidden, norm_nc, kernel_size=kernel_size, padding=pw)
        self.kernel_size = kernel_size
        self._cache = _PackCache()

    def packed(self, dtype) -> ops.PackedSpade:
        ps = (self.mlp_shared[0].weight, self.mlp_shared[0].bias, self.mlp_gamma.weight, self.mlp_gamma.bias,
              self.mlp_beta.weight, self.mlp_beta.bias)
        return self._cache.get(ps, dtype, lambda: ops.pack_spade_weights(*[p.data for p in ps], dtype))

    def forward_nhwc(self, x: ops.NHWC, cond: ops.NHWC, stats=None, act=ops.ACT_NONE, x_upsample=False) -> ops.NHWC:
        if self.kernel_size != 3:
            raise NotImplementedError("SPADE: only kernel_size 3 is supported")
        if isinstance(x, ops.PairMap):
            return self._forward_pair(x, cond, stats, act, x_upsample)
        batch_stats = False
        if self.param_free_norm_type == "batch":
            bn = self.param_free_norm
            if bn.training:
                from . import autograd as _ag
                if _ag.BN_GROUPS != 1:
                    raise NotImplementedError("SPADE with a batch param-free norm inside autograd.bn_groups(%d): run the "
# ... 90 lines not shown
```

climategan_amd/ops.py:

```python
import collections
import ctypes as C
import functools
import inspect
import os
from dataclasses import dataclass
from typing import Optional, Tuple

import torch

from . import _lib
from ._lib import (ACT_LRELU, ACT_NONE, ACT_RELU, ACT_SIGMOID, ACT_TANH, CGAN_BF16, CGAN_F16, PAD_REFLECT,
                   PAD_ZERO, ConvDesc, NormStatsDesc, PackItem, SnItem, SpadeDesc)

_DT = {torch.float16: CGAN_F16, torch.bfloat16: CGAN_BF16}


def touch(*tensors) -> None:
    ts = [t for t in tensors if t is not None]
    if ts:
        torch.autograd.graph.increment_version(ts)


MAX_MAP_BYTES = 2 ** 31
ABI_MAX_BYTES = 2 ** 31
# ... 1067 lines not shown

@dataclass
class ConvStats:
    partial: torch.Tensor
    chunk_pixels: int


def conv2d_with_stats(x: NHWC, pw: PackedConv, stride=1, pad=0, dilation=1, pad_mode=PAD_ZERO, groups: int = 1):
    _need_cuda(x.t)
    _need_cs8("conv2d", x)
    if x.c != pw.c_in:
        raise RuntimeError("conv2d: input has %d channels, weight expects %d" % (x.c, pw.c_in))
    if x.t.dtype != pw.dtype:
        raise RuntimeError("conv2d: activation dtype %s != packed weight dtype %s" % (x.t.dtype, pw.dtype))
    d = _conv_desc(x.dtype_id, x.n, x.h, x.w, pw.c_in, pw.c_out, pw.kh, pw.kw, stride, pad, dilation, pad_mode,
                   has_bias=pw.has_bias)
    lib = _lib.load()
    ppb = lib.cgan_conv2d_stats_chunk_pixels(C.byref(d))
    npix = x.n * d.h_out * d.w_out
    if ppb <= 0 or x.n % groups or (npix // groups) % ppb:
        return conv2d(x, pw, stride=stride, pad=pad, dilation=dilation, pad_mode=pad_mode), None
    y = _empty((x.n, d.h_out, d.w_out, cs8(pw.c_out)), dtype=x.t.dtype, device=x.t.device)
    partial = _empty((npix // ppb, cs8(pw.c_out), 2), dtype=torch.float32, device=x.t.device)
    _lib.check(lib.cgan_conv2d_nhwc_fwd_stats(_ptr(x.t), _ptr(pw.w), _ptr(pw.bias), _ptr(y), _ptr(partial),
                                              partial.numel() * 4, C.byref(d), _stream()), "cgan_conv2d_nhwc_fwd_stats")
    return NHWC(y, pw.c_out), ConvStats(partial, ppb)


def batchnorm_train_stats_from_partials(st: ConvStats, groups: int, pix_per_group: int, c: int, gamma, beta, running_mean,
                                        running_var, num_batches_tracked, eps, momentum):
    lib = _lib.load()
    cs = st.partial.shape[1]
    d = NormStatsDesc(CGAN_BF16, groups, pix_per_group, c, float(eps))
    stats = _empty((4, groups, cs), dtype=torch.float32, device=st.partial.device)
    _lib.check(lib.cgan_batchnorm_train_stats_from_partials(
        _ptr(st.partial), int(st.chunk_pixels), _ptr(gamma), _ptr(beta), float(momentum), _ptr(running_mean),
        _ptr(running_var), _ptr(num_batches_tracked), _ptr(stats[0]), _ptr(stats[1]), _ptr(stats[2]), _ptr(stats[3]),
        C.byref(d), _stream()), "cgan_batchnorm_train_stats_from_partials")
    touch(running_mean, running_var, num_batches_tracked)
    return stats[0], stats[1], stats[2], stats[3]


@_batch_chunked("dxp")
def reflect_pad_bwd(dxp: NHWC, pad: int) -> NHWC:
    _need_cuda(dxp.t)
    h, w = dxp.h - 2 * pad, dxp.w - 2 * pad
    dx = _empty((dxp.n, h, w, dxp.cs), dtype=dxp.t.dtype, device=dxp.t.device)
    lib = _lib.load()
    _lib.check(lib.cgan_reflect_pad_bwd_nhwc(_ptr(dxp.t), _ptr(dx), dxp.dtype_id, dxp.n, dxp.c, h, w, int(pad), _stream()),
               "cgan_reflect_pad_bwd_nhwc")
    return NHWC(dx, dxp.c)


def conv2d_bwd_data(dy: NHWC, w: torch.Tensor, x_shape, stride=1, pad=0, dilation=1,
                    sigma: Optional[torch.Tensor] = None, pad_mode=PAD_ZERO, add: Optional[NHWC] = None,
                    prepacked: Optional[DgradPack] = None, relu_out: Optional[NHWC] = None) -> NHWC:
    same = stride == 1 and pad_mode == PAD_ZERO and 2 * pad == dilation * (w.shape[2] - 1) and w.shape[2] == w.shape[3]
    if relu_out is not None:
        if not same:
            dx = conv2d_bwd_data(dy, w, x_shape, stride, pad, dilation, sigma, pad_mode, add=add, prepacked=prepacked)
            return act_bwd(relu_out, dx, ACT_RELU)
    per_sample = max(dy.t.nbytes // max(dy.n, 1), (x_shape[1] + 2 * pad) * (x_shape[2] + 2 * pad) * cs8(w.shape[1]) * 2)
    if x_shape[0] * per_sample >= MAX_MAP_BYTES:
        k = (MAX_MAP_BYTES - 1) // per_sample
        if k < 1:
            raise RuntimeError("conv2d_bwd_data: ONE sample's map exceeds the 2 GiB a C-ABI call covers")
        return _run_chunks(x_shape[0], k, lambda lo, cnt: conv2d_bwd_data(
            NHWC(dy.t[lo:lo + cnt], dy.c), w, (cnt, x_shape[1], x_shape[2]), stride, pad, dilation, sigma, pad_mode,
            NHWC(add.t[lo:lo + cnt], add.c) if add is not None else None, prepacked,
            NHWC(relu_out.t[lo:lo + cnt], relu_out.c) if relu_out is not None else None))
    if add is not None and not same:
        dx = conv2d_bwd_data(dy, w, x_shape, stride, pad, dilation, sigma, pad_mode, prepacked=prepacked)
        return NHWC(dx.t + add.t, dx.c)
    if pad_mode == PAD_REFLECT and pad > 0:
        n, h_in, w_in = x_shape
        dxp = conv2d_bwd_data(dy, w, (n, h_in + 2 * pad, w_in + 2 * pad), stride=stride, pad=0, dilation=dilation,
                              sigma=sigma, prepacked=prepacked)
        return reflect_pad_bwd(dxp, pad)
    _need_cuda(dy.t, w, sigma)
    _need_cs8("conv2d_bwd_data", dy)
    w = w.detach().contiguous().float()
    c_out, c_in, kh, kw = w.shape
    n, h_in, w_in = x_shape
    d = _conv_desc(dy.dtype_id, n, h_in, w_in, c_in, c_out, kh, kw, stride, pad, dilation, PAD_ZERO, has_bias=False)
    if (d.h_out, d.w_out) != (dy.h, dy.w) or dy.c != c_out or dy.n != n:
        raise RuntimeError("conv2d_bwd_data: dy shape %s does not match the forward conv" % (tuple(dy.t.shape),))
    lib = _lib.load()
    nbytes = lib.cgan_conv2d_dgrad_packed_weight_bytes(C.byref(d))
    if nbytes == 0:
        _lib.check(-1, "cgan_conv2d_dgrad_packed_weight_bytes")
    if (prepacked is not None and prepacked.packed is not None and stride == 1 and prepacked.dtype == dy.t.dtype
            and prepacked.packed.numel() == nbytes and tuple(prepacked.w.shape) == tuple(w.shape)):
        packed = prepacked.packed
    else:
        packed = _empty(nbytes, dtype=torch.uint8, device=w.device)
        _lib.check(lib.cgan_conv2d_pack_weight_dgrad(_ptr(w), _ptr(sigma), _ptr(packed), C.byref(d), _stream()),
                   "cgan_conv2d_pack_weight_dgrad")
    dx = _empty((n, h_in, w_in, cs8(c_in)), dtype=dy.t.dtype, device=dy.t.device)
    _conv_ws()
    if relu_out is not None:
        if relu_out.t.shape != dx.shape or relu_out.t.dtype != dx.dtype or not relu_out.t.is_contiguous():
            raise RuntimeError("conv2d_bwd_data: ``relu_out`` %s does not match dx %s" % (tuple(relu_out.t.shape), tuple(dx.shape)))
        if add is not None:
            if add.t.shape != dx.shape or add.t.dtype != dx.dtype or not add.t.is_contiguous():
                raise RuntimeError("conv2d_bwd_data: ``add`` %s does not match dx %s" % (tuple(add.t.shape), tuple(dx.shape)))
            _lib.check(lib.cgan_conv2d_nhwc_bwd_data_add_relu(_ptr(dy.t), _ptr(packed), _ptr(add.t), _ptr(relu_out.t), _ptr(dx),
                                                              C.byref(d), _stream()), "cgan_conv2d_nhwc_bwd_data_add_relu")
            return NHWC(dx, c_in)
        _lib.check(lib.cgan_conv2d_nhwc_bwd_data_relu(_ptr(dy.t), _ptr(packed), _ptr(relu_out.t), _ptr(dx), C.byref(d), _stream()),
                   "cgan_conv2d_nhwc_bwd_data_relu")
        return NHWC(dx, c_in)
    if add is not None:
        if add.t.shape != dx.shape or add.t.dtype != dx.dtype or not add.t.is_contiguous():
            raise RuntimeError("conv2d_bwd_data: ``add`` %s does not match dx %s" % (tuple(add.t.shape), tuple(dx.shape)))
        _lib.check(lib.cgan_conv2d_nhwc_bwd_data_add(_ptr(dy.t), _ptr(packed), _ptr(add.t), _ptr(dx), C.byref(d), _stream()),
                   "cgan_conv2d_nhwc_bwd_data_add")
        return NHWC(dx, c_in)
    _lib.check(lib.cgan_conv2d_nhwc_bwd_data(_ptr(dy.t), _ptr(packed), _ptr(dx), C.byref(d), _stream()),
               "cgan_conv2d_nhwc_bwd_data")
    return NHWC(dx, c_in)


@_batch_chunked("x")
def sumpool2x2(x: NHWC) -> NHWC:
    _need_cuda(x.t)
    if x.h % 2 or x.w % 2 or x.cs != cs8(x.c):
        raise RuntimeError("sumpool2x2: even extent and round_up(c, 8) storage expected")
    y = _empty((x.n, x.h // 2, x.w // 2, x.cs), dtype=x.t.dtype, device=x.t.device)
    lib = _lib.load()
    _lib.check(lib.cgan_sumpool2x2_nhwc(_ptr(x.t), _ptr(y), x.dtype_id, x.n, x.c, x.h // 2, x.w // 2, _stream()),
               "cgan_sumpool2x2_nhwc")
    return NHWC(y, x.c)


class ZeroArena:

    def __init__(self, numel: int, device):
        self.buf = torch.zeros(int(numel), dtype=torch.float32, device=device)
        self.off = 0

    def take(self, n: int):
        n_al = (n + 63) // 64 * 64
        if self.off + n_al > self.buf.numel():
            return None
        t = self.buf[self.off:self.off + n]
        self.off += n_al
        return t


_ZERO_ARENA = None


def set_zero_arena(arena):
    global _ZERO_ARENA
    prev, _ZERO_ARENA = _ZERO_ARENA, arena
    return prev


def zeros_f32(n: int, device) -> torch.Tensor:
    if _ZERO_ARENA is not None and _ZERO_ARENA.buf.device == device:
        t = _ZERO_ARENA.take(n)
        if t is not None:
            return t
    return torch.zeros(n, dtype=torch.float32, device=device)


def conv2d_bwd_weight(x: NHWC, dy: NHWC, w_shape, stride=1, pad=0, dilation=1, want_bias=True,
                      dw: Optional[torch.Tensor] = None, dbias: Optional[torch.Tensor] = None, in_upsample=False,
                      pad_mode=PAD_ZERO, use_workspace=True):
    per_sample = max(x.t.nbytes, dy.t.nbytes) // max(x.n, 1)
# ... 764 lines not shown
```

include/climategan_hip.h:

```cpp
#ifndef CLIMATEGAN_HIP_H
#define CLIMATEGAN_HIP_H

#include <stddef.h>
#include <stdint.h>

#ifdef __cplusplus
extern "C" {
#endif

#define CGAN_ABI_VERSION 1

typedef enum {
  CGAN_OK = 0,
  CGAN_ERR_BAD_ARG = -1,
  CGAN_ERR_UNSUPPORTED = -2,
  CGAN_ERR_WORKSPACE = -3,
  CGAN_ERR_HIP = -4,
  CGAN_ERR_INTERNAL = -5
} cgan_status_t;

typedef enum { CGAN_F16 = 0, CGAN_BF16 = 1, CGAN_F32 = 2  } cgan_dtype_t;
typedef enum { CGAN_ACT_NONE = 0, CGAN_ACT_RELU = 1, CGAN_ACT_LRELU = 2, CGAN_ACT_TANH = 3, CGAN_ACT_SIGMOID = 4 } cgan_act_t;
typedef enum { CGAN_PAD_ZERO = 0, CGAN_PAD_REFLECT = 1 } cgan_pad_t;

// ... 3 lines not shown
const char* cgan_last_error(void);

typedef struct {
  int32_t dtype;
  int32_t n, h_in, w_in;
  int32_t c_in, c_out;
  int32_t kh, kw, stride, pad, dilation;
  int32_t pad_mode;
  int32_t h_out, w_out;
  int32_t in_upsample;
  int32_t act;
  float act_slope;
  int32_t has_bias;
  int32_t has_residual;
  int32_t residual_upsample;
} CganConvDesc;

size_t cgan_conv2d_packed_weight_bytes(const CganConvDesc* d);
int cgan_conv2d_pack_weight(const float* w_oihw, const float* bias, const float* sigma, void* packed,
                            float* bias_out, const CganConvDesc* d, void* stream);
int cgan_conv2d_nhwc_fwd(const void* x, const void* packed_w, const float* bias_padded, const void* residual,
                         void* y, const CganConvDesc* d, void* stream);
typedef struct {
  const float* w_oihw;
  const float* bias;
  const float* sigma;
  void* packed;
  float* bias_out;
  int32_t c_out, c_in, kh, kw;
  int32_t transposed;
} CganPackItem;
int cgan_conv2d_pack_weight_batched(const CganPackItem* items_device, int32_t count, int32_t dtype,
                                    int32_t max_fragments, void* stream);

int32_t cgan_conv2d_stats_chunk_pixels(const CganConvDesc* d);
int cgan_conv2d_nhwc_fwd_stats(const void* x, const void* packed_w, const float* bias_padded, void* y, float* partial,
                               size_t partial_bytes, const CganConvDesc* d, void* stream);

enum { CGAN_CONV_KERNEL_GENERAL = 0, CGAN_CONV_KERNEL_LDS3X3 = 1, CGAN_CONV_KERNEL_GEMM = 2 };
int cgan_conv2d_bind_workspace(void* stream, void* workspace, size_t bytes);
int cgan_conv2d_kernel_kind(const CganConvDesc* d, int32_t bwd_data);
int cgan_conv2d_kernel_kind_on(const CganConvDesc* d, int32_t bwd_data, void* stream);
size_t cgan_conv2d_dgrad_packed_weight_bytes(const CganConvDesc* fwd);
int cgan_conv2d_pack_weight_dgrad(const float* w_oihw, const float* sigma, void* packed, const CganConvDesc* fwd,
                                  void* stream);
int cgan_conv2d_nhwc_bwd_data(const void* dy, const void* packed_w_dgrad, void* dx, const CganConvDesc* fwd,
                              void* stream);
int cgan_conv2d_nhwc_bwd_data_add(const void* dy, const void* packed_w_dgrad, const void* dx_add, void* dx,
                                  const CganConvDesc* fwd, void* stream);
int cgan_conv2d_nhwc_bwd_data_relu(const void* dy, const void* packed_w_dgrad, const void* relu_out, void* dx,
                                   const CganConvDesc* fwd, void* stream);
int cgan_conv2d_nhwc_bwd_data_add_relu(const void* dy, const void* packed_w_dgrad, const void* dx_add, const void* relu_out,
                                       void* dx, const CganConvDesc* fwd, void* stream);
size_t cgan_conv2d_bwd_weight_workspace_bytes(const CganConvDesc* fwd);
int cgan_conv2d_nhwc_bwd_weight(const void* x, const void* dy, float* dw_oihw, float* dbias, const CganConvDesc* fwd,
                                void* workspace, size_t workspace_bytes,
                                void* stream);

typedef struct {
  int32_t dtype;
  int32_t n, hw, c;
  float eps;
} CganNormStatsDesc;
size_t cgan_instnorm_stats_workspace_bytes(const CganNormStatsDesc* d);
int cgan_instnorm_stats(const void* x, float* mean, float* rstd, const CganNormStatsDesc* d, void* workspace,
                        size_t workspace_bytes, void* stream);
int cgan_norm_act_apply(const void* x, const float* mean, const float* rstd, void* y, const CganNormStatsDesc* d,
                        int32_t act, float act_slope, void* stream);
int cgan_norm_add_act_apply(const void* x, const float* mean, const float* rstd, const void* residual, void* y,
                            const CganNormStatsDesc* d, int32_t act, float act_slope, void* stream);

typedef struct {
  int32_t dtype;
  int32_t n, h, w, c;
  int32_t x_upsample;
  int32_t cond_h, cond_w, cond_c;
  int32_t hidden;
  int32_t ksize;
  int32_t act;
  float act_slope;
} CganSpadeDesc;
static inline int cgan_cond_cs(int c) { return (c + 3) & ~3; }
size_t cgan_spade_packed_weight_bytes(const CganSpadeDesc* d);
int cgan_spade_pack_weights(const float* w_shared, const float* b_shared, const float* w_gamma, const float* b_gamma,
                            const float* w_beta, const float* b_beta, void* packed, const CganSpadeDesc* d,
                            void* stream);
int cgan_spade_fused_fwd(const void* x, const float* mean, const float* rstd, const void* cond, const void* packed,
                         void* y, const CganSpadeDesc* d, void* stream);
int cgan_spade_fused_fwd_train(const void* x, const float* mean, const float* rstd, const void* cond, const void* packed,
                               void* y, void* gamma_out, const CganSpadeDesc* d, void* stream);

size_t cgan_spectral_norm_workspace_bytes(int32_t rows, int32_t cols);
int cgan_spectral_norm_power_iter(const float* w_bar, float* u, float* v, float* sigma, int32_t rows, int32_t cols,
                                  void* workspace, size_t workspace_bytes, void* stream);
typedef struct {
  const float* w_bar;
  float* u;
  float* v;
  float* sigma;
  float* workspace;
  int32_t rows, cols;
} CganSnItem;
int cgan_spectral_norm_power_iter_batched(const CganSnItem* items_device, int32_t count, int32_t max_rows,
                                          int32_t max_cols, void* stream);

typedef struct {
// ... 34 lines not shown
int cgan_resize_nearest_nhwc(const void* x, void* y, int32_t dtype, int32_t n, int32_t c, int32_t h_in, int32_t w_in,
                             int32_t cs_in, int32_t h_out, int32_t w_out, int32_t cs_out, void* stream);
int cgan_avgpool3x3s2_nhwc(const void* x, void* y, int32_t dtype, int32_t n, int32_t c, int32_t h_in, int32_t w_in,
                           void* stream);

int cgan_maxpool3x3s2_nhwc(const void* x, void* y, int32_t dtype, int32_t n, int32_t c, int32_t h_in, int32_t w_in,
                           void* stream);
int cgan_resize_bilinear_nhwc(const void* x, void* y, int32_t dtype, int32_t n, int32_t c, int32_t h_in, int32_t w_in,
                              int32_t h_out, int32_t w_out, int32_t align_corners, void* stream);
int cgan_resize_bicubic_nhwc(const void* x, void* y, int32_t dtype, int32_t n, int32_t c, int32_t h_in, int32_t w_in,
                             int32_t h_out, int32_t w_out, void* stream);
int cgan_sumpool2x2_nhwc(const void* x, void* y, int32_t dtype, int32_t n, int32_t c, int32_t h_out, int32_t w_out,
                         void* stream);
int cgan_reflect_pad_bwd_nhwc(const void* dx_padded, void* dx, int32_t dtype, int32_t n, int32_t c, int32_t h, int32_t w,
                              int32_t pad, void* stream);
int cgan_copy_channels_nhwc(const void* src, void* dst, int64_t npix, int32_t c, int32_t cs_src, int32_t cs_dst,
                            int32_t c_off, void* stream);
int cgan_eltwise_nhwc(const void* a, const void* b, void* y, int32_t dtype, int32_t op, int64_t numel, void* stream);
int cgan_fold_bn(const float* w, const float* bias, const float* gamma, const float* beta, const float* mean,
                 const float* var, float eps, float* w_out, float* b_out, int32_t c_out, int64_t per_out, void* stream);

int cgan_act_bwd(const void* out, const void* dy, void* dx, int32_t dtype, int32_t act, float act_slope,
                 int64_t numel, void* stream);
size_t cgan_instnorm_act_bwd_workspace_bytes(const CganNormStatsDesc* d);
int cgan_instnorm_act_bwd(const void* out, const void* dy, const float* rstd, void* dx, const CganNormStatsDesc* d,
                          int32_t act, float act_slope, void* workspace, size_t workspace_bytes, void* stream);
int cgan_spade_bwd_prepare(const void* dy, const void* y, const void* x, const float* mean, const float* rstd,
                           const void* gamma, void* dgb, void* xhat, void* dxhat, const CganSpadeDesc* d, void* stream);
size_t cgan_spade_hidden_bwd_workspace_bytes(const CganSpadeDesc* d);
int cgan_spade_hidden_bwd(const void* dgb, const void* packed_dgrad_gb, const void* cond_hw, const void* packed_w_shared,
                          const float* bias_shared_padded, float* dw_shared, float* db_shared, void* workspace,
                          size_t workspace_bytes, const CganSpadeDesc* d, void* stream);
int cgan_bn_train_prepare(const float* batch_mean, const float* batch_rstd, const float* gamma, const float* beta,
                          float eps, float momentum, int64_t count, float* running_mean, float* running_var,
                          float* mean_out, float* rstd_out, int64_t* num_batches_tracked, int32_t c, void* stream);
int cgan_batchnorm_train_stats(const void* x, const float* gamma, const float* beta, float momentum, float* running_mean,
                               float* running_var, int64_t* num_batches_tracked, float* batch_mean, float* batch_rstd,
                               float* mean_out, float* rstd_out, const CganNormStatsDesc* d, void* workspace,
                               size_t workspace_bytes, void* stream);
int cgan_batchnorm_train_stats_from_partials(float* partial, int32_t chunk_pixels, const float* gamma,
                                             const float* beta, float momentum, float* running_mean, float* running_var,
                                             int64_t* num_batches_tracked, float* batch_mean, float* batch_rstd,
                                             float* mean_out, float* rstd_out, const CganNormStatsDesc* d, void* stream);
size_t cgan_batchnorm_act_bwd_workspace_bytes(int32_t c);
int cgan_batchnorm_act_bwd(const void* x, const void* out, const void* dy, const float* batch_mean,
                           const float* batch_rstd, const float* gamma, const float* fold_mean, const float* fold_rstd,
                           void* dx, float* dgamma, float* dbeta, void* dz_out, int32_t dtype, int64_t npix, int32_t c,
                           int32_t act, float act_slope, void* workspace, size_t workspace_bytes, void* stream);
int cgan_batchnorm_act_bwd_grouped(const void* x, const void* out, const void* dy, const float* batch_mean,
                                   const float* batch_rstd, const float* gamma, const float* fold_mean,
                                   const float* fold_rstd, void* dx, float* dgamma, float* dbeta, void* dz_out,
                                   int32_t dtype, int64_t npix_total, int32_t c, int32_t groups, int32_t act,
                                   float act_slope, void* workspace, size_t workspace_bytes, void* stream);
int cgan_bce_logits_nhwc(const void* x, int32_t dtype, int64_t npix, int32_t c, float target, float weight,
                         float* loss_accum, void* dx, void* stream);
int cgan_hinge_nhwc(const void* x, int32_t dtype, int64_t npix, int32_t c, int32_t target_is_real,
                    int32_t for_discriminator, float weight, float* loss_accum, void* dx, void* stream);
int cgan_mse_const_nhwc(const void* x, int32_t dtype, int64_t npix, int32_t c, float target, float weight, float* loss_accum,
                        void* dx, void* stream);
int cgan_painter_aux_losses(const void* fake_nhwc, const float* x_nchw, const float* m_nchw, int32_t dtype, int32_t n,
                            int32_t h, int32_t w, float w_tv_h, float w_tv_w, float w_context, float w_reconstruction,
                            float* loss3, void* d_fake, void* stream);
int cgan_resize_bicubic_bwd_nhwc(const void* dy, void* dx, int32_t dtype, int32_t n, int32_t c, int32_t h_in, int32_t w_in,
                                 int32_t h_out, int32_t w_out, void* stream);
int cgan_l1_nhwc(const void* a, const void* b, int32_t dtype, int64_t numel, float weight, float* loss_accum, void* da,
                 void* stream);
#define CGAN_SN_BWD_WORKSPACE_FLOATS 1024
int cgan_spectral_norm_bwd(float* grad_w, const float* w_bar, const float* u, const float* v, const float* sigma,
                           int32_t rows, int32_t cols, float* workspace, void* stream);

int cgan_painter_heads_fwd(const void* fake_nhwc, const float* x_nchw, const float* m_nchw, void* d_in, void* vgg_in,
                           int32_t dtype, int32_t n, int32_t h, int32_t w, void* stream);
int cgan_painter_heads_bwd(const void* d_d_in, const void* d_vgg_in, const float* m_nchw, void* d_fake, int32_t dtype,
                           int32_t n, int32_t h, int32_t w, void* stream);
#define CGAN_DA_BRIGHTNESS 1
#define CGAN_DA_CONTRAST 2
#define CGAN_DA_SATURATION 4
#define CGAN_DA_TRANSLATION 8
#define CGAN_DA_CUTOUT 16
#define CGAN_DA_ALL 31
#define CGAN_DIFFAUG_PARTS 256
int cgan_diffaug_fwd(const float* x, float* y, const float* color, const int64_t* geo, int32_t flags, int32_t cut_h,
                     int32_t cut_w, int32_t n, int32_t c, int32_t h, int32_t w, float* ws, void* stream);
int cgan_diffaug_bwd(const float* dy, float* dx, const float* color, const int64_t* geo, int32_t flags, int32_t cut_h,
                     int32_t cut_w, int32_t n, int32_t c, int32_t h, int32_t w, float* ws, void* stream);
int cgan_painter_heads_diffaug_fwd(const void* fake_nhwc, const float* x_nchw, const float* m_nchw, void* d_in, void* vgg_in,
                                   const float* color, const int64_t* geo, int32_t flags, int32_t cut_h, int32_t cut_w,
                                   int32_t dtype, int32_t n, int32_t h, int32_t w, float* ws, void* stream);
int cgan_painter_heads_diffaug_bwd(const void* d_d_in, const void* d_vgg_in, const float* m_nchw, void* d_fake,
                                   const float* color, const int64_t* geo, int32_t flags, int32_t cut_h, int32_t cut_w,
                                   int32_t dtype, int32_t n, int32_t h, int32_t w, float* ws, void* stream);
int cgan_avgpool3x3s2_bwd_nhwc(const void* dy, void* dx, int32_t dtype, int32_t n, int32_t c, int32_t h_in,
                               int32_t w_in, void* stream);
int cgan_maxpool2x2_nhwc(const void* x, void* y, int32_t dtype, int32_t n, int32_t c, int32_t h_in, int32_t w_in,
                         void* stream);
int cgan_maxpool2x2_bwd_nhwc(const void* x, const void* dy, void* dx, int32_t dtype, int32_t n, int32_t c, int32_t h_in,
                             int32_t w_in, void* stream);
int cgan_maxpool2x2_relu_bwd_nhwc(const void* x, const void* dy, void* dx, int32_t dtype, int32_t n, int32_t c, int32_t h_in,
                                  int32_t w_in, void* stream);

int cgan_softmax_nhwc(const void* x, void* y, int32_t dtype, int64_t npix, int32_t c, void* stream);
int cgan_softmax_bwd_nhwc(const void* y, const void* dy, void* dx, int32_t dtype, int64_t npix, int32_t c, void* stream);
int cgan_sigmoid_pair_nhwc(const void* x, void* y, int32_t dtype, int64_t npix, void* stream);
int cgan_sigmoid_pair_bwd_nhwc(const void* y, const void* dy, void* dx, int32_t dtype, int64_t npix, void* stream);
int cgan_softmax_ce_nhwc(const void* logits, const int64_t* target, int32_t dtype, int64_t npix, int32_t c, float weight,
                         float* loss_accum, void* dlogits, void* stream);
// ... 271 lines not shown
```

Before: 57.51.

## Fuse BatchNorm backward reduction statistics into the dgrad conv epilogue

The conv backward-data GEMM epilogue now also reads the saved BN input x and accumulates per-channel sums of dz and dz*xhat into per-tile partials, applying the activation mask where needed. The following BatchNorm backward consumes those partials and skips its own reduction pass over x and dy. The aim is to remove one full read of the activation and gradient tensors per BN layer in backward. In exchange the epilogue gains extra loads and registers, and the autograd nodes now hand state to each other through a pointer-and-shape token with a fallback path.

```diff
diff --git a/climategan_amd/_lib.py b/climategan_amd/_lib.py
--- a/climategan_amd/_lib.py
+++ b/climategan_amd/_lib.py
@@ -207,6 +207,12 @@
                                          C.c_int32, C.c_float, _P, C.c_size_t, _P]),
     "cgan_batchnorm_act_bwd_grouped": (C.c_int, [_P, _P, _P, _P, _P, _P, _P, _P, _P, _P, _P, _P, C.c_int32, C.c_int64,
                                                  C.c_int32, C.c_int32, C.c_int32, C.c_float, _P, C.c_size_t, _P]),
+    "cgan_conv2d_bwd_data_bn_stats_rows": (C.c_int32, [C.POINTER(ConvDesc), C.c_int32, C.c_int32, _P]),
+    "cgan_conv2d_bwd_data_bn_stats_bind": (C.c_int, [_P, _P, _P, _P, _P, _P, C.c_float, C.c_int32, C.c_int32, _P, C.c_size_t]),
+    "cgan_batchnorm_act_bwd_from_partials_workspace_bytes": (C.c_size_t, [C.c_int32, C.c_int32]),
+    "cgan_batchnorm_act_bwd_from_partials": (C.c_int, [_P, _P, _P, C.c_int32, _P, _P, _P, _P, _P, _P, _P, _P, C.c_int32,
+                                                       C.c_int64, C.c_int32, C.c_int32, C.c_int32, C.c_float, _P, C.c_size_t,
+                                                       _P]),
     "cgan_bce_logits_nhwc": (C.c_int, [_P, C.c_int32, C.c_int64, C.c_int32, C.c_float, C.c_float, _P, _P, _P]),
     "cgan_hinge_nhwc": (C.c_int, [_P, C.c_int32, C.c_int64, C.c_int32, C.c_int32, C.c_int32, C.c_float, _P, _P, _P]),
     "cgan_l1_nhwc": (C.c_int, [_P, _P, C.c_int32, C.c_int64, C.c_float, _P, _P, _P]),
diff --git a/climategan_amd/autograd.py b/climategan_amd/autograd.py
--- a/climategan_amd/autograd.py
+++ b/climategan_amd/autograd.py
@@ -163,10 +163,12 @@
         if ctx.needs_input_grad[0]:
             h_in, w_in = (x_t.shape[1] * 2, x_t.shape[2] * 2) if ups else (x_t.shape[1], x_t.shape[2])
             relu_out = ops.NHWC(x_t, cfg["c_in"]) if cfg.get("mask_input") else None
+            offer = None if ups or pair else _bn_bwd_stats_offer(cfg)
             dx = ops.conv2d_bwd_data(dy, w_eff, (x_t.shape[0], h_in, w_in), stride=cfg["stride"], pad=cfg["pad"],
                                      dilation=cfg["dilation"], sigma=sigma, pad_mode=cfg.get("pad_mode", ops.PAD_ZERO),
-                                     prepacked=ctx.dgrad, relu_out=relu_out)
+                                     prepacked=ctx.dgrad, relu_out=relu_out, bn_stats=offer)
             dx_t = (ops.sumpool2x2(dx) if ups else dx).t
+            _bn_bwd_stats_deliver(cfg, offer, dx_t)
         if ctx.has_res and ctx.needs_input_grad[3]:
             dres_t = (ops.sumpool2x2(dy) if cfg.get("residual_upsample", False) else dy).t
         dw = db = None
@@ -218,10 +220,12 @@
         if ctx.needs_input_grad[0]:
             add = ops.NHWC(dpass_t.contiguous(), cfg["c_in"]) if dpass_t is not None else None
             relu_out = ops.NHWC(x_t, cfg["c_in"]) if cfg.get("mask_input") else None
+            offer = _bn_bwd_stats_offer(cfg)
             dx_t = ops.conv2d_bwd_data(dy, weight, (x_t.shape[0], x_t.shape[1], x_t.shape[2]), stride=cfg["stride"],
                                        pad=cfg["pad"], dilation=cfg["dilation"],
                                        pad_mode=cfg.get("pad_mode", ops.PAD_ZERO), add=add, prepacked=ctx.dgrad,
-                                       relu_out=relu_out).t
+                                       relu_out=relu_out, bn_stats=offer).t
+            _bn_bwd_stats_deliver(cfg, offer, dx_t)
         dw = db = None
         if ctx.needs_input_grad[1] or (ctx.has_bias and ctx.needs_input_grad[2]):
             dw, db = ops.conv2d_bwd_weight(
@@ -449,6 +453,8 @@
         ctx.cfg = (c, act, slope, G)
         ctx.has_res = res_t is not None
         ctx.premasked = False
+        ctx.stats_claimed = False
+        ctx.bwd_stats = None
         keep_out = res_t is not None or _BN_BWD_READS_OUT
         ctx.save_for_backward(x_t, out if keep_out else None, mean, rstd, gamma,
                               None if keep_out else mean_f, None if keep_out else rstd_f)
@@ -463,10 +469,29 @@
         if ctx.premasked:
             act = ops.ACT_NONE
         n, h, w, cs = x_t.shape
+        dx = torch.empty_like(x_t)
+        want_res = ctx.has_res and ctx.needs_input_grad[11]
+        st, ctx.bwd_stats = ctx.bwd_stats, None
+        if st is not None:
+            partial, rows, token = st
+            if token == (dy_t.data_ptr(), tuple(dy_t.shape)) and dy_t.is_contiguous():
+                dres = dy_t if want_res else None
+                nbytes = G * lib.cgan_batchnorm_act_bwd_from_partials_workspace_bytes(c, rows)
+                ws = torch.empty(nbytes, dtype=torch.uint8, device=x_t.device)
+                dg = db = None
+                if gamma is not None:
+                    dg, db = torch.empty((2, c), dtype=torch.float32, device=x_t.device).unbind(0)
+                _lib.check(lib.cgan_batchnorm_act_bwd_from_partials(
+                    ops._ptr(x_t), ops._ptr(dy_t), ops._ptr(partial), rows, ops._ptr(mean), ops._ptr(rstd), ops._ptr(gamma),
+                    ops._ptr(mean_f), ops._ptr(rstd_f), ops._ptr(dx), ops._ptr(dg), ops._ptr(db), ops._DT[x_t.dtype],
+                    n * h * w, c, G, act, slope, ops._ptr(ws), nbytes, ops._stream()),
+                    "cgan_batchnorm_act_bwd_from_partials")
+                return dx, dg, db, None, None, None, None, None, None, None, None, dres, None
+            if _DEBUG:
+                raise RuntimeError("BatchNormActFn: partial rows were left for the gradient tensor %s, another one arrived: %s"
+                                   % (token, (dy_t.data_ptr(), tuple(dy_t.shape))))
         nbytes = G * lib.cgan_batchnorm_act_bwd_workspace_bytes(c)
         ws = torch.empty(nbytes, dtype=torch.uint8, device=x_t.device)
-        dx = torch.empty_like(x_t)
-        want_res = ctx.has_res and ctx.needs_input_grad[11]
         dy_t = dy_t.contiguous()
         if want_res and act == ops.ACT_NONE:
             dres = dy_t
@@ -481,6 +506,45 @@
             ops._DT[x_t.dtype], n * h * w, c, G, act, slope, ops._ptr(ws), nbytes, ops._stream()),
             "cgan_batchnorm_act_bwd_grouped")
         return dx, dg, db, None, None, None, None, None, None, None, None, dres, None
+
+
+_DEBUG = os.environ.get("CGAN_DEBUG", "0") not in ("", "0")
+FUSE_BN_BWD_STATS = os.environ.get("CGAN_FUSE_BN_BWD_STATS", "1") != "0"
+
+
+def claim_bn_bwd_stats(out_t: torch.Tensor, masked: bool = False):
+    fn = out_t.grad_fn
+    if not FUSE_BN_BWD_STATS or fn is None or not isinstance(fn, BatchNormActFn._backward_cls) or fn.stats_claimed:
+        return None
+    act = fn.cfg[1]
+    if fn.has_res:
+        if not (masked and fn.premasked):
+            return None
+    elif act not in (ops.ACT_RELU, ops.ACT_LRELU) or _BN_BWD_READS_OUT:
+        return None
+    fn.stats_claimed = True
+    return fn
+
+
+def _bn_bwd_stats_offer(cfg):
+    fn = cfg.get("bn_src")
+    if fn is None or not FUSE_BN_BWD_STATS:
+        return None
+    x_t, _, mean, rstd, _, mean_f, rstd_f = fn.saved_tensors
+    c, act, slope, G = fn.cfg
+    if fn.has_res:
+        return ops.BnBwdStats(x_t, mean, rstd, None, None, 0, 0.0, G)
+    return ops.BnBwdStats(x_t, mean, rstd, mean_f, rstd_f, 2, 0.0 if act == ops.ACT_RELU else slope, G)
+
+
+def _bn_bwd_stats_deliver(cfg, offer, dx_t):
+    fn = cfg.get("bn_src")
+    if fn is None:
+        return
+    if _DEBUG and fn.bwd_stats is not None:
+        raise RuntimeError("BatchNormActFn: partial rows delivered twice (the node was not reached in between)")
+    if offer is not None and offer.partial is not None:
+        fn.bwd_stats = (offer.partial, offer.rows, (dx_t.data_ptr(), tuple(dx_t.shape)))
 
 
 def claim_relu_mask(out_t: torch.Tensor) -> bool:
diff --git a/climategan_amd/csrc/cgan_common.h b/climategan_amd/csrc/cgan_common.h
--- a/climategan_amd/csrc/cgan_common.h
+++ b/climategan_amd/csrc/cgan_common.h
@@ -27,6 +27,13 @@
 
 __device__ __forceinline__ float cgan_res_apply(float v, float r, int mode) { return mode == 2 ? (r > 0.f ? v : 0.f) : v + r; }
 __device__ __forceinline__ float cgan_res_apply3(float v, float r, float m) { return m > 0.f ? v + r : 0.f; }
+
+template <int MASK>
+__device__ __forceinline__ float bn_bwd_act_grad(float ov, float xv, float fm, float fr, float gneg) {
+  if (MASK == 0) return 1.f;
+  if (MASK == 1) return ov > 0.f ? 1.f : gneg;
+  return (xv - fm) * fr > 0.f ? 1.f : gneg;
+}
 
 #ifdef CGAN_DEV
 #define CGAN_KNOB(type, name, init) type name = init
diff --git a/climategan_amd/csrc/conv_gemm.h b/climategan_amd/csrc/conv_gemm.h
--- a/climategan_amd/csrc/conv_gemm.h
+++ b/climategan_amd/csrc/conv_gemm.h
@@ -1,5 +1,17 @@
 #pragma once
 #include "cgan_common.h"
+
+struct ConvGemmBnStats {
+  const uint16_t* x;
+  const float* mean;
+  const float* rstd;
+  const float* fmean;
+  const float* frstd;
+  float* partial;
+  float gneg;
+  int mask;
+  int gpix;
+};
 
 struct ConvGemmArgs {
   const uint16_t* x;
@@ -15,6 +27,7 @@
   int act, has_res, res_ups;
   float slope;
   float* stats;
+  ConvGemmBnStats bns = {};
 };
 
 struct ConvGemmCls {
@@ -42,6 +55,7 @@
 int conv_gemm_launch(const ConvGemmArgs& a, int dtype, hipStream_t s);
 bool conv_gemm_res2_ok(const ConvGemmArgs& a, int dtype);
 int conv_gemm_stats_chunk_pixels(const ConvGemmArgs& a, int dtype);
+int conv_gemm_bn_stats_tile_pixels(const ConvGemmArgs& a, int dtype);
 bool conv_gemm_big_ok(const ConvGemmArgs& a);
 bool conv1x1_allc_ok(const ConvGemmArgs& a);
 int conv1x1_allc_launch(const ConvGemmArgs& a, int dtype, hipStream_t s);
@@ -127,7 +141,8 @@
   }
 }
 
-template <typename T, int WC, int WP, int PP, bool RES2 = false>
+#define HAS_RES(p) (BNS ? (RES2 ? 3 : 0) : (p).has_res)
+template <typename T, int WC, int WP, int PP, bool RES2 = false, bool BNS = false>
 __device__ __forceinline__ void conv_gemm_staged_store(const f32x4 (&acc)[WC][WP], const ConvGemmArgs& p,
                                                        unsigned char* stg, int pix0, int cout_base, const float* bias_ep,
                                                        int lane, int j, int g) {
@@ -140,7 +155,7 @@
   const int qc = lane % CH, pl0 = lane / CH;
   const int ch = cout_base + qc * 8;
   const bool ch_ok = ch < p.cout_s;
-  const bool plain = !bias_ep && !p.has_res && p.act == CGAN_ACT_NONE && p.cout == p.cout_s;
+  const bool plain = !bias_ep && !HAS_RES(p) && p.act == CGAN_ACT_NONE && p.cout == p.cout_s;
   f32x4 bb0 = (f32x4){0.f, 0.f, 0.f, 0.f}, bb1 = bb0;
   if (bias_ep && ch_ok) {
     bb0 = *reinterpret_cast<const f32x4*>(bias_ep + ch);
@@ -156,7 +171,20 @@
       if (pix < p.npix && ch_ok) dst[it] = CGAN_LD_STREAM(reinterpret_cast<const u32x4*>(p.res2 + (size_t)pix * p.cout_s + ch));
     }
   };
-  if (p.has_res) {
+  constexpr bool XALL = WC * WP <= 16;
+  constexpr int NXB = !BNS ? 1 : (XALL ? NPASS : (NPASS > 1 ? 2 : 1));
+  u32x4 xq[NXB][BNS ? NIT : 1];
+  float bmu[BNS ? 8 : 1], brs[BNS ? 8 : 1], bfm[BNS ? 8 : 1], bfr[BNS ? 8 : 1], bs1[BNS ? 8 : 1], bs2[BNS ? 8 : 1];
+  const bool bns_tile = BNS && pix0 < p.npix;
+  auto load_xq = [&](int pass, u32x4 (&dst)[BNS ? NIT : 1]) {
+#pragma unroll
+    for (int it = 0; it < (BNS ? NIT : 0); ++it) {
+      const int pix = pix0 + pass * PP * 16 + it * PSTEP + pl0;
+      dst[it] = (u32x4){0u, 0u, 0u, 0u};
+      if (pix < p.npix && ch_ok) dst[it] = CGAN_LD_STREAM(reinterpret_cast<const u32x4*>(p.bns.x + (size_t)pix * p.cout_s + ch));
+    }
+  };
+  if (HAS_RES(p)) {
 #pragma unroll
     for (int pass = 0; pass < NPASS; ++pass)
 #pragma unroll
@@ -177,7 +205,29 @@
           rv[pass][it] = CGAN_LD_STREAM(reinterpret_cast<const u32x4*>(p.res + rbase + ch));
         }
       }
-    if (RES2 && p.has_res == 3) load_rm(0, rm[0]);
+    if (RES2 && HAS_RES(p) == 3) load_rm(0, rm[0]);
+    __builtin_amdgcn_sched_barrier(0);
+  }
+  if constexpr (BNS) {
+#pragma unroll
+    for (int e = 0; e < 8; ++e) bmu[e] = brs[e] = bfm[e] = bfr[e] = bs1[e] = bs2[e] = 0.f;
+    if (bns_tile && ch_ok) {
+      const size_t row = (size_t)(pix0 / p.bns.gpix) * p.cout_s + ch;
+#pragma unroll
+      for (int e = 0; e < 8; ++e) {
+        bmu[e] = p.bns.mean[row + e];
+        brs[e] = p.bns.rstd[row + e];
+      }
+      if (p.bns.mask == 2) {
+#pragma unroll
+        for (int e = 0; e < 8; ++e) {
+          bfm[e] = p.bns.fmean[row + e];
+          bfr[e] = p.bns.frstd[row + e];
+        }
+      }
+    }
+#pragma unroll
+    for (int pass = 0; pass < (XALL ? NPASS : 1); ++pass) load_xq(pass, xq[pass]);
     __builtin_amdgcn_sched_barrier(0);
   }
 #pragma unroll
@@ -188,12 +238,20 @@
       for (int c = 0; c < WC; ++c)
         *reinterpret_cast<f32x4*>(stg + (tt * 16 + j) * ROWB + c * 64 + g * 16) = acc[c][pass * PP + tt];
     asm volatile("s_waitcnt lgkmcnt(0)" ::: "memory");
-    if (RES2 && NPASS > 1 && p.has_res == 3 && pass + 1 < NPASS) {
+    if (RES2 && NPASS > 1 && HAS_RES(p) == 3 && pass + 1 < NPASS) {
       __builtin_amdgcn_sched_barrier(0);
       load_rm(pass + 1, rm[(pass + 1) & 1]);
       __builtin_amdgcn_sched_barrier(0);
     }
-    if (pass == 0 || (RES2 && p.has_res == 3 && pass >= 2)) __builtin_amdgcn_s_waitcnt(0x0F70);
+    if constexpr (BNS && !XALL) {
+      if (pass + 1 < NPASS) {
+        __builtin_amdgcn_sched_barrier(0);
+        load_xq(pass + 1, xq[(pass + 1) & (NXB - 1)]);
+        __builtin_amdgcn_sched_barrier(0);
+      }
+    }
+    if (pass == 0 || (((RES2 && HAS_RES(p) == 3) || (BNS && !XALL)) && pass >= 2))
+      __builtin_amdgcn_s_waitcnt(0x0F70);
 #pragma unroll
     for (int it = 0; it < NIT; ++it) {
       const int pl = it * PSTEP + pl0;
@@ -209,7 +267,7 @@
             v[4 + r] += bb1[r];
           }
         }
-        if (RES2 && p.has_res == 3) {
+        if (RES2 && HAS_RES(p) == 3) {
 #pragma unroll
           for (int e = 0; e < 4; ++e) {
             float r0, r1, m0, m1;
@@ -218,13 +276,13 @@
             v[2 * e] = cgan_res_apply3(v[2 * e], r0, m0);
             v[2 * e + 1] = cgan_res_apply3(v[2 * e + 1], r1, m1);
           }
-        } else if (p.has_res) {
+        } else if (HAS_RES(p)) {
 #pragma unroll
           for (int e = 0; e < 4; ++e) {
             float r0, r1;
             unpack2<T>(rv[pass][it][e], r0, r1);
-            v[2 * e] = cgan_res_apply(v[2 * e], r0, p.has_res);
-            v[2 * e + 1] = cgan_res_apply(v[2 * e + 1], r1, p.has_res);
+            v[2 * e] = cgan_res_apply(v[2 * e], r0, HAS_RES(p));
+            v[2 * e + 1] = cgan_res_apply(v[2 * e + 1], r1, HAS_RES(p));
           }
         }
         act_apply_n(v, p.act, p.slope);
@@ -238,8 +296,51 @@
 #pragma unroll
       for (int e = 0; e < 4; ++e) o[e] = pack2<T>(v[2 * e], v[2 * e + 1]);
       if (pix < p.npix && ch_ok) CGAN_ST_STREAM(o, reinterpret_cast<u32x4*>(p.y + (size_t)pix * p.cout_s + ch));
+      if constexpr (BNS) {
+        const bool live = pix < p.npix && ch_ok;
+        const u32x4& xv4 = xq[XALL ? pass : (pass & (NXB - 1))][it];
+#pragma unroll
+        for (int e = 0; e < 4; ++e) {
+          float dz[2], xv[2];
+          unpack2<T>(o[e], dz[0], dz[1]);
+          unpack2<T>(xv4[e], xv[0], xv[1]);
+#pragma unroll
+          for (int hh = 0; hh < 2; ++hh) {
+            const int k = 2 * e + hh;
+            if (p.bns.mask == 2) dz[hh] *= bn_bwd_act_grad<2>(0.f, xv[hh], bfm[k], bfr[k], p.bns.gneg);
+            const float xh = (xv[hh] - bmu[k]) * brs[k];
+            if (live) {
+              bs1[k] += dz[hh];
+              bs2[k] += dz[hh] * xh;
+            }
+          }
+        }
+      }
     }
     asm volatile("s_waitcnt lgkmcnt(0)" ::: "memory");
   }
+  if constexpr (BNS) {
+    constexpr int NO = CH / 4;
+    static_assert(CH % 4 == 0 && 64 * 64 <= PP * 16 * ROWB, "the lane sums fit the wave's staging rows");
+    float* red = reinterpret_cast<float*>(stg);
+#pragma unroll
+    for (int e = 0; e < 8; e += 2)
+      *reinterpret_cast<f32x4*>(red + lane * 16 + 2 * e) = (f32x4){bs1[e], bs2[e], bs1[e + 1], bs2[e + 1]};
+    asm volatile("s_waitcnt lgkmcnt(0)" ::: "memory");
+    float tot[NO];
+#pragma unroll
+    for (int k = 0; k < NO; ++k) tot[k] = 0.f;
+#pragma unroll
+    for (int l = 0; l < PSTEP; ++l)
+#pragma unroll
+      for (int k = 0; k < NO; ++k) tot[k] += red[l * CH * 16 + lane * NO + k];
+    const int och = cout_base + lane * NO / 2;
+    if (bns_tile && och < p.cout_s) {
+      float* dst = p.bns.partial + ((size_t)(pix0 / (WP * 16)) * p.cout_s + och) * 2;
+#pragma unroll
+      for (int k = 0; k < NO; k += 2) *reinterpret_cast<f32x2*>(dst + k) = (f32x2){tot[k], tot[k + 1]};
+    }
+  }
 }
+#undef HAS_RES
 #endif
diff --git a/climategan_amd/csrc/conv_gemm.hip b/climategan_amd/csrc/conv_gemm.hip
--- a/climategan_amd/csrc/conv_gemm.hip
+++ b/climategan_amd/csrc/conv_gemm.hip
@@ -14,7 +14,7 @@
   return i;
 }
 
-template <typename T, int WAVES_C, int WC, int WP, bool REFLECT, int NS = NSTAGE, bool RES2 = false>
+template <typename T, int WAVES_C, int WC, int WP, bool REFLECT, int NS = NSTAGE, bool RES2 = false, bool BNS = false>
 __global__ __launch_bounds__(256, 2) void conv_gemm_kernel(ConvGemmArgs p, int npb, int ncb) {
   constexpr int WAVES_P = 4 / WAVES_C;
   constexpr int CT_BLK = WAVES_C * WC;
@@ -147,7 +147,7 @@
     conv_gemm_stats_epilogue<T, WC, WP>(acc, p, cout_base, pblk * WAVES_P + wp, j, g);
     if (p.bias) bias_ep = nullptr;
   }
-  conv_gemm_staged_store<T, WC, WP, PP, RES2>(acc, p, stg, (pblk * PT_BLK + wp * WP) * 16, cout_base, bias_ep, lane, j, g);
+  conv_gemm_staged_store<T, WC, WP, PP, RES2, BNS>(acc, p, stg, (pblk * PT_BLK + wp * WP) * 16, cout_base, bias_ep, lane, j, g);
 }
 
 template <typename T, int WC, int WP>
@@ -410,14 +410,14 @@
 }
 
 
-template <typename T, int WAVES_C, int WC, int WP, bool REFLECT, int NS = NSTAGE, bool RES2 = false>
+template <typename T, int WAVES_C, int WC, int WP, bool REFLECT, int NS = NSTAGE, bool RES2 = false, bool BNS = false>
 int launch_cfg2(const ConvGemmArgs& a, hipStream_t s) {
   constexpr int WAVES_P = 4 / WAVES_C;
   constexpr int CT_BLK = WAVES_C * WC, PT_BLK = WAVES_P * WP;
   constexpr size_t smem = (size_t)NS * (CT_BLK + PT_BLK) * 1024;
   static bool attr_set = false;
   if (!attr_set) {
-    hipError_t e = hipFuncSetAttribute(reinterpret_cast<const void*>(&conv_gemm_kernel<T, WAVES_C, WC, WP, REFLECT, NS, RES2>),
+    hipError_t e = hipFuncSetAttribute(reinterpret_cast<const void*>(&conv_gemm_kernel<T, WAVES_C, WC, WP, REFLECT, NS, RES2, BNS>),
                                        hipFuncAttributeMaxDynamicSharedMemorySize, 160 * 1024);
     if (e != hipSuccess) {
       cgan_set_error("conv_gemm: hipFuncSetAttribute failed: %s", hipGetErrorString(e));
@@ -428,7 +428,7 @@
   const int npb = ceil_div(ceil_div(a.npix, 16), PT_BLK);
   const int ncb = ceil_div(a.ctiles, CT_BLK);
   const int grid = ceil_div(npb, 8) * 8 * ncb;
-  hipLaunchKernelGGL((conv_gemm_kernel<T, WAVES_C, WC, WP, REFLECT, NS, RES2>), dim3(grid), dim3(256), smem, s, a, npb, ncb);
+  hipLaunchKernelGGL((conv_gemm_kernel<T, WAVES_C, WC, WP, REFLECT, NS, RES2, BNS>), dim3(grid), dim3(256), smem, s, a, npb, ncb);
   return CGAN_OK;
 }
 
@@ -496,6 +496,19 @@
     case KIND_XRES: return conv1x1_xres_launch(a, T::id, s);
     default: break;
   }
+  if (a.bns.partial) {
+    switch (ch.cfg) {
+      case 2: return launch_cfg2<T, 2, 8, 4, false, NSTAGE, false, true>(a, s);
+      case 3: return launch_cfg2<T, 2, 4, 8, false, NSTAGE, false, true>(a, s);
+      case 5:
+        if (a.has_res == 3) return launch_cfg2<T, 2, 4, 4, false, 2, true, true>(a, s);
+        return launch_cfg2<T, 2, 4, 4, false, 2, false, true>(a, s);
+      case 4: return launch_cfg2<T, 2, 4, 4, false, NSTAGE, false, true>(a, s);
+      default:
+        cgan_set_error("conv_gemm: this kernel has no BatchNorm-backward statistics store path");
+        return CGAN_ERR_INTERNAL;
+    }
+  }
   switch (ch.cfg) {
     case 1: return launch_cfg<T, 1, 4, 4>(a, s);
     case 2: return launch_cfg<T, 2, 8, 4>(a, s);
@@ -537,3 +550,16 @@
   const int ppb = ch.cfg == 3 ? 128 : 64;
   return a.npix % ppb == 0 ? ppb : 0;
 }
+
+int conv_gemm_bn_stats_tile_pixels(const ConvGemmArgs& a, int dtype) {
+  if (a.pad_mode == CGAN_PAD_REFLECT || a.bias || a.act != CGAN_ACT_NONE || a.stats || a.res_ups) return 0;
+  if (a.has_res != 0 && a.has_res != 3) return 0;
+  const Choice ch = choose(a, dtype == CGAN_BF16);
+  if (ch.kind != KIND_PLAIN) return 0;
+  if (a.has_res == 3) return ch.cfg == 5 ? 64 : 0;
+  switch (ch.cfg) {
+    case 2: case 4: case 5: return 64;
+    case 3: return 128;
+    default: return 0;
+  }
+}
diff --git a/climategan_amd/csrc/conv_mfma.hip b/climategan_amd/csrc/conv_mfma.hip
--- a/climategan_amd/csrc/conv_mfma.hip
+++ b/climategan_amd/csrc/conv_mfma.hip
@@ -784,6 +784,7 @@
   CganConvDesc d;
   int ksplit;
   float* ws;
+  ConvGemmBnStats bns = {};
 };
 
 ConvGemmArgs gemm_args(const ConvParams& p) {
@@ -943,7 +944,12 @@
   const int dt = pl.d.dtype;
   int rc = CGAN_OK;
   switch (pl.route) {
-    case ROUTE_GEMM: rc = conv_gemm_launch(gemm_args(p), dt, s); break;
+    case ROUTE_GEMM: {
+      ConvGemmArgs a = gemm_args(p);
+      a.bns = pl.bns;
+      rc = conv_gemm_launch(a, dt, s);
+      break;
+    }
     case ROUTE_SPLITK: rc = conv_gemm_splitk_launch(gemm_args(p), pl.ksplit, pl.ws, dt, s); break;
     case ROUTE_LDS3X3: case ROUTE_SUBPIXEL: rc = conv3x3_lds_launch(lds_args(pl), dt, s); break;
     case ROUTE_SMALLCIN: rc = conv_smallcin_launch(lds_args(pl), dt, s); break;
@@ -1097,13 +1103,78 @@
   return kernel_kind_impl(d, bwd_data, WsSlot{0, nullptr, nullptr, ws_max_bytes()});
 }
 
+namespace {
+struct BnsArm { int device; void* stream; ConvGemmBnStats b; int groups; size_t bytes; };
+constexpr int BNS_SLOTS = 16;
+BnsArm g_bns[BNS_SLOTS];
+int g_bns_n = 0;
+std::mutex g_bns_mu;
+
+bool bns_take(void* stream, BnsArm* out) {
+  const int dev = ws_device();
+  std::lock_guard<std::mutex> lk(g_bns_mu);
+  for (int i = 0; i < g_bns_n; ++i)
+    if (g_bns[i].stream == stream && g_bns[i].device == dev) {
+      *out = g_bns[i];
+      g_bns[i] = g_bns[--g_bns_n];
+      return true;
+    }
+  return false;
+}
+
+int bn_stats_rows(const ConvPlan& pl, int groups) {
+  if (pl.route != ROUTE_GEMM || groups < 1 || pl.d.n % groups) return 0;
+  const int tile = conv_gemm_bn_stats_tile_pixels(gemm_args(pl.p), pl.d.dtype);
+  const int gpix = pl.p.npix / groups;
+  return tile > 0 && gpix % tile == 0 ? gpix / tile : 0;
+}
+}
+
+extern "C" int32_t cgan_conv2d_bwd_data_bn_stats_rows(const CganConvDesc* fwd, int32_t res_mode, int32_t groups, void* stream) {
+  if (!fwd || (res_mode != RES_NONE && res_mode != RES_ADD && res_mode != RES_ADD_RELU)) return 0;
+  if (res_mode != RES_NONE && !(fwd->stride == 1 && 2 * fwd->pad == fwd->dilation * (fwd->kh - 1))) return 0;
+  ConvPlan pl;
+  if (plan_dgrad(pl, fwd, res_mode, ws_lookup(stream)) != CGAN_OK) return 0;
+  return bn_stats_rows(pl, groups);
+}
+
+extern "C" int cgan_conv2d_bwd_data_bn_stats_bind(void* stream, const void* x, const float* mean, const float* rstd,
+                                                  const float* fmean, const float* frstd, float gneg, int32_t mask_mode,
+                                                  int32_t groups, float* partial, size_t partial_bytes) {
+  CGAN_REQUIRE(x && mean && rstd && partial, "conv2d_bwd_data_bn_stats_bind: null pointer");
+  CGAN_REQUIRE(mask_mode == 0 || mask_mode == 2, "conv2d_bwd_data_bn_stats_bind: mask_mode must be 0 or 2, got %d", mask_mode);
+  CGAN_REQUIRE(mask_mode != 2 || (fmean && frstd), "conv2d_bwd_data_bn_stats_bind: mask_mode 2 needs fmean / frstd");
+  CGAN_REQUIRE(groups >= 1 && groups <= 16, "conv2d_bwd_data_bn_stats_bind: bad group count %d", groups);
+  CGAN_REQUIRE((reinterpret_cast<size_t>(partial) & 15) == 0, "conv2d_bwd_data_bn_stats_bind: partial must be 16-byte aligned");
+  BnsArm arm{ws_device(), stream,
+             ConvGemmBnStats{(const uint16_t*)x, mean, rstd, fmean, frstd, partial, gneg, mask_mode, 0}, groups, partial_bytes};
+  std::lock_guard<std::mutex> lk(g_bns_mu);
+  for (int i = 0; i < g_bns_n; ++i)
+    if (g_bns[i].stream == stream && g_bns[i].device == arm.device) {
+      g_bns[i] = arm;
+      return CGAN_OK;
+    }
+  if (g_bns_n == BNS_SLOTS) --g_bns_n;
+  g_bns[g_bns_n++] = arm;
+  return CGAN_OK;
+}
+
 static int bwd_data_impl(const void* dy, const void* packed_w_dgrad, const void* res, const void* relu_out, void* dx,
                          const CganConvDesc* fwd, void* stream, int res_mode) {
+  BnsArm arm;
+  const bool armed = bns_take(stream, &arm);
   CGAN_REQUIRE(dy && packed_w_dgrad && dx, "conv2d_nhwc_bwd_data: null pointer");
   ConvPlan pl;
   int rc = plan_dgrad(pl, fwd, res_mode, ws_lookup(stream));
   if (rc != CGAN_OK) return rc;
   bind(pl.p, dy, packed_w_dgrad, nullptr, res, dx);
+  if (armed && res_mode != RES_RELU) {
+    const int rows = bn_stats_rows(pl, arm.groups);
+    if (rows > 0 && arm.bytes >= (size_t)arm.groups * rows * pl.p.cout_s * 2 * sizeof(float)) {
+      pl.bns = arm.b;
+      pl.bns.gpix = pl.p.npix / arm.groups;
+    }
+  }
   if (pl.p.has_res == 3) pl.p.res2 = (const uint16_t*)relu_out;
   rc = launch_plan(pl, (hipStream_t)stream, "conv2d_nhwc_bwd_data");
   if (rc != CGAN_OK || res_mode != RES_ADD_RELU || pl.p.has_res == 3) return rc;
diff --git a/climategan_amd/csrc/train_ops.hip b/climategan_amd/csrc/train_ops.hip
--- a/climategan_amd/csrc/train_ops.hip
+++ b/climategan_amd/csrc/train_ops.hip
@@ -292,12 +292,6 @@
 }
 
 constexpr int BN_BWD_MAX_CHUNKS = 512;
-template <int MASK>
-__device__ __forceinline__ float bn_bwd_act_grad(float ov, float xv, float fm, float fr, float gneg) {
-  if (MASK == 0) return 1.f;
-  if (MASK == 1) return ov > 0.f ? 1.f : gneg;
-  return (xv - fm) * fr > 0.f ? 1.f : gneg;
-}
 
 template <typename T, int MASK>
 __global__ __launch_bounds__(256) void bn_bwd_reduce_kernel(const uint16_t* __restrict__ x, const uint16_t* __restrict__ out,
@@ -448,6 +442,27 @@
   if (ch < c) {
     if (dgamma) dgamma[ch] = dg_sum;
     if (dbeta) dbeta[ch] = db_sum;
+  }
+}
+
+constexpr int BN_BWD_MERGE = 16;
+constexpr int BN_BWD_MERGE_FROM = 512;
+__global__ __launch_bounds__(256) void bn_bwd_premerge_kernel(const float* __restrict__ partial, float* __restrict__ merged,
+                                                              int rows, int cs) {
+  const int mrows = gridDim.x;
+  const int r0 = blockIdx.x * BN_BWD_MERGE, r1 = min(rows, r0 + BN_BWD_MERGE);
+  const f32x4* src = reinterpret_cast<const f32x4*>(partial + (size_t)blockIdx.y * rows * cs * 2);
+  f32x4* dst = reinterpret_cast<f32x4*>(merged + ((size_t)blockIdx.y * mrows + blockIdx.x) * cs * 2);
+  const int w4 = cs / 2;
+  for (int i = threadIdx.x; i < w4; i += 256) {
+    f32x4 v[BN_BWD_MERGE];
+#pragma unroll
+    for (int r = 0; r < BN_BWD_MERGE; ++r)
+      v[r] = r0 + r < r1 ? src[(size_t)(r0 + r) * w4 + i] : (f32x4){0.f, 0.f, 0.f, 0.f};
+    f32x4 a = v[0];
+#pragma unroll
+    for (int r = 1; r < BN_BWD_MERGE; ++r) a += v[r];
+    dst[i] = a;
   }
 }
 
@@ -656,6 +671,31 @@
                      (long long*)num_batches_tracked, c, cs);
   CGAN_CHECK_LAUNCH("bn_train_prepare");
   return CGAN_OK;
+}
+
+static void bn_bwd_finalize_apply(const void* x, const void* out, const void* dy, const float* partial, int chunks,
+                                  const float* batch_mean, const float* batch_rstd, const float* gamma,
+                                  const float* fold_mean, const float* fold_rstd, void* dx, float* dgamma, float* dbeta,
+                                  void* dz_out, uint16_t* dz_early, float* coef, int dtype, long npix, int c, int groups,
+                                  int mask, float gneg, hipStream_t s) {
+  const int cs = cgan_cs(c);
+  const int cg_total = cs / 8;
+  hipLaunchKernelGGL(bn_bwd_finalize_kernel, dim3(cs / 8), dim3(256), 0, s, partial, chunks, batch_mean, batch_rstd, gamma,
+                     1.f / (float)npix, coef, dgamma, dbeta, (int)c, cs, (int)groups);
+  const int tpp = cg_total < 256 ? cg_total : 256;
+  const int rows = 256 / tpp;
+  long blocks = (npix + (long)rows * 4 - 1) / ((long)rows * 4);
+  blocks = blocks < 1 ? 1 : (blocks > 4096 / groups ? 4096 / groups : blocks);
+#define BN_BWD_APPLY(M)                                                                                               \
+  DISPATCH_T2(dtype, bn_bwd_apply_kernel, M, dim3((unsigned)blocks, groups), dim3(256), 0, s, (const uint16_t*)x,     \
+              (const uint16_t*)out, (const uint16_t*)dy, (const float*)coef, fold_mean, fold_rstd, (uint16_t*)dx,     \
+              (uint16_t*)dz_out, (long)npix, cs, gneg)
+  if (dz_early) {
+    DISPATCH_T2(dtype, bn_bwd_apply_kernel, 0, dim3((unsigned)blocks, groups), dim3(256), 0, s, (const uint16_t*)x,
+                (const uint16_t*)nullptr, (const uint16_t*)dz_early, (const float*)coef, fold_mean, fold_rstd,
+                (uint16_t*)dx, (uint16_t*)nullptr, (long)npix, cs, gneg);
+  } else if (mask == 0) { BN_BWD_APPLY(0); } else if (mask == 1) { BN_BWD_APPLY(1); } else { BN_BWD_APPLY(2); }
+#undef BN_BWD_APPLY
 }
 
 extern "C" size_t cgan_batchnorm_act_bwd_workspace_bytes(int32_t c) {
@@ -712,23 +752,50 @@
               fold_rstd, partial, dz_early, (long)npix, cs, (int)ppb, gneg)
   if (mask == 0) { BN_BWD_REDUCE(0); } else if (mask == 1) { BN_BWD_REDUCE(1); } else { BN_BWD_REDUCE(2); }
 #undef BN_BWD_REDUCE
-  hipLaunchKernelGGL(bn_bwd_finalize_kernel, dim3(cs / 8), dim3(256), 0, s, (const float*)partial, (int)chunks,
-                     batch_mean, batch_rstd, gamma, 1.f / (float)npix, coef, dgamma, dbeta, (int)c, cs, (int)groups);
-  const int tpp = cg_total < 256 ? cg_total : 256;
-  const int rows = 256 / tpp;
-  long blocks = (npix + (long)rows * 4 - 1) / ((long)rows * 4);
-  blocks = blocks < 1 ? 1 : (blocks > 4096 / groups ? 4096 / groups : blocks);
-#define BN_BWD_APPLY(M)                                                                                               \
-  DISPATCH_T2(dtype, bn_bwd_apply_kernel, M, dim3((unsigned)blocks, groups), dim3(256), 0, s, (const uint16_t*)x,     \
-              (const uint16_t*)out, (const uint16_t*)dy, (const float*)coef, fold_mean, fold_rstd, (uint16_t*)dx,     \
-              (uint16_t*)dz_out, (long)npix, cs, gneg)
-  if (dz_early) {
-    DISPATCH_T2(dtype, bn_bwd_apply_kernel, 0, dim3((unsigned)blocks, groups), dim3(256), 0, s, (const uint16_t*)x,
-                (const uint16_t*)nullptr, (const uint16_t*)dz_early, (const float*)coef, fold_mean, fold_rstd,
-                (uint16_t*)dx, (uint16_t*)nullptr, (long)npix, cs, gneg);
-  } else if (mask == 0) { BN_BWD_APPLY(0); } else if (mask == 1) { BN_BWD_APPLY(1); } else { BN_BWD_APPLY(2); }
-#undef BN_BWD_APPLY
+  bn_bwd_finalize_apply(x, out, dy, partial, (int)chunks, batch_mean, batch_rstd, gamma, fold_mean, fold_rstd, dx, dgamma,
+                        dbeta, dz_out, dz_early, coef, dtype, npix, c, groups, mask, gneg, s);
   CGAN_CHECK_LAUNCH("batchnorm_act_bwd");
+  return CGAN_OK;
+}
+
+extern "C" size_t cgan_batchnorm_act_bwd_from_partials_workspace_bytes(int32_t c, int32_t rows) {
+  if (c <= 0 || rows <= 0) return 0;
+  const size_t merged = rows >= BN_BWD_MERGE_FROM ? (size_t)ceil_div(rows, BN_BWD_MERGE) * 2 : 0;
+  return (size_t)cgan_cs(c) * (3 + merged) * sizeof(float);
+}
+
+extern "C" int cgan_batchnorm_act_bwd_from_partials(const void* x, const void* dy, const float* partial, int32_t rows,
+                                                    const float* batch_mean, const float* batch_rstd, const float* gamma,
+                                                    const float* fold_mean, const float* fold_rstd, void* dx, float* dgamma,
+                                                    float* dbeta, int32_t dtype, int64_t npix_total, int32_t c,
+                                                    int32_t groups, int32_t act, float act_slope, void* workspace,
+                                                    size_t workspace_bytes, void* stream) {
+  CGAN_REQUIRE(x && dy && partial && batch_mean && batch_rstd && dx && workspace, "batchnorm_act_bwd_from_partials: null pointer");
+  CGAN_REQUIRE(act == CGAN_ACT_NONE || (fold_mean && fold_rstd),
+               "batchnorm_act_bwd_from_partials: the activation mask needs fold_mean / fold_rstd");
+  CGAN_REQUIRE(dtype == CGAN_F16 || dtype == CGAN_BF16, "batchnorm_act_bwd_from_partials: bad dtype %d", dtype);
+  CGAN_REQUIRE(groups >= 1 && groups <= 16 && npix_total > 0 && c > 0 && rows > 0 && npix_total % groups == 0,
+               "batchnorm_act_bwd_from_partials: bad shape (the pixel count must divide into the groups)");
+  CGAN_REQUIRE(act == CGAN_ACT_NONE || act == CGAN_ACT_RELU || act == CGAN_ACT_LRELU,
+               "batchnorm_act_bwd_from_partials: Unsupported activation: %d", act);
+  CGAN_REQUIRE(workspace_bytes >= (size_t)groups * cgan_batchnorm_act_bwd_from_partials_workspace_bytes(c, rows),
+               "batchnorm_act_bwd_from_partials: workspace too small");
+  const long npix = npix_total / groups;
+  const int cs = cgan_cs(c);
+  hipStream_t s = (hipStream_t)stream;
+  float* coef = (float*)workspace;
+  int chunks = rows;
+  if (rows >= BN_BWD_MERGE_FROM) {
+    float* merged = coef + (size_t)groups * 3 * cs;
+    chunks = ceil_div(rows, BN_BWD_MERGE);
+    hipLaunchKernelGGL(bn_bwd_premerge_kernel, dim3(chunks, groups), dim3(256), 0, s, partial, merged, (int)rows, cs);
+    partial = merged;
+  }
+  const int mask = act == CGAN_ACT_NONE ? 0 : 2;
+  const float gneg = act == CGAN_ACT_RELU ? 0.f : act_slope;
+  bn_bwd_finalize_apply(x, nullptr, dy, partial, chunks, batch_mean, batch_rstd, gamma, fold_mean, fold_rstd, dx, dgamma,
+                        dbeta, nullptr, nullptr, coef, dtype, npix, c, groups, mask, gneg, s);
+  CGAN_CHECK_LAUNCH("batchnorm_act_bwd_from_partials");
   return CGAN_OK;
 }
 
diff --git a/climategan_amd/deeplab/resnet101_v3.py b/climategan_amd/deeplab/resnet101_v3.py
--- a/climategan_amd/deeplab/resnet101_v3.py
+++ b/climategan_amd/deeplab/resnet101_v3.py
@@ -34,10 +34,10 @@
             x = residual
         else:
             out = conv_bn_forward(self.conv1, self.bn1, self._c[0], x, act=ops.ACT_RELU)
-        out = conv_bn_forward(self.conv2, self.bn2, self._c[1], out, act=ops.ACT_RELU)
+        out = conv_bn_forward(self.conv2, self.bn2, self._c[1], out, act=ops.ACT_RELU, bn_input=True)
         if self.downsample is not None:
             residual = conv_bn_forward(self.downsample[0], self.downsample[1], self._c[3], x)
-        return conv_bn_forward(self.conv3, self.bn3, self._c[2], out, act=ops.ACT_RELU, residual=residual)
+        return conv_bn_forward(self.conv3, self.bn3, self._c[2], out, act=ops.ACT_RELU, residual=residual, bn_input=True)
 
 
 class ResNet(nn.Module):
diff --git a/climategan_amd/norms.py b/climategan_amd/norms.py
--- a/climategan_amd/norms.py
+++ b/climategan_amd/norms.py
@@ -31,6 +31,8 @@
                residual_upsample=bool(kw.get("residual_upsample", False)), pad_mode=pad_mode,
                sn_owned=bool(kw.get("sn_owned", False)), pair_in=bool(kw.get("pair_in", False)),
                want_stats=bool(kw.get("want_stats", False)))
+    if kw.get("bn_src") is not None:
+        cfg["bn_src"] = kw["bn_src"]
     y_t = ConvFn.apply(x.t, weight, bias, res.t if res is not None else None, packed, cfg, sn)
     if kw.get("want_stats"):
         return ops.NHWC(y_t, weight.shape[0]), cfg.get("stats_out")
@@ -229,6 +231,7 @@
 
 
 def conv_bn_forward(conv: nn.Conv2d, bn, cache: _PackCache, x: ops.NHWC, pad_mode=ops.PAD_ZERO, pad=None, **kw) -> ops.NHWC:
+    bn_input = kw.pop("bn_input", False)
     train_bn = bn is not None and bn.training
     grad = needs_grad(conv, x.t) or (bn is not None and needs_grad(bn))
     p = conv.padding[0] if pad is None else pad
@@ -271,6 +274,9 @@
         if sole_consumer and FUSE_RELU_MASK:
             from .autograd import claim_relu_mask
             pcfg["mask_input"] = claim_relu_mask(x.t)
+            if pcfg["mask_input"]:
+                from .autograd import claim_bn_bwd_stats
+                pcfg["bn_src"] = claim_bn_bwd_stats(x.t, masked=True)
         y_t, pass_t = ConvPassFn.apply(x.t, conv.weight, conv.bias, pw, pcfg)
         y, passthrough = ops.NHWC(y_t, conv.weight.shape[0]), ops.NHWC(pass_t, x.c)
         conv_stats = pcfg.get("stats_out")
@@ -279,11 +285,16 @@
                            dict(act=act, slope=slope, residual=residual, pad_mode=pad_mode))
     if passthrough is None:
         conv_stats = None
+        bn_src = None
+        if bn_input:
+            from .autograd import claim_bn_bwd_stats
+            bn_src = claim_bn_bwd_stats(x.t)
         if FUSE_BN_STATS:
             y, conv_stats = _conv_train(x, conv.weight, conv.bias, pw, None, conv.stride[0], p, conv.dilation[0],
-                                        dict(pad_mode=pad_mode, want_stats=True))
+                                        dict(pad_mode=pad_mode, want_stats=True, bn_src=bn_src))
         else:
-            y = _conv_train(x, conv.weight, conv.bias, pw, None, conv.stride[0], p, conv.dilation[0], dict(pad_mode=pad_mode))
+            y = _conv_train(x, conv.weight, conv.bias, pw, None, conv.stride[0], p, conv.dilation[0],
+                            dict(pad_mode=pad_mode, bn_src=bn_src))
     if residual is not None and not FUSE_BN_RESIDUAL:
         from . import functional as Fn
         out_t = BatchNormActFn.apply(y.t, bn.weight if bn.affine else None, bn.bias if bn.affine else None,
diff --git a/climategan_amd/ops.py b/climategan_amd/ops.py
--- a/climategan_amd/ops.py
+++ b/climategan_amd/ops.py
@@ -1143,9 +1143,32 @@
     return NHWC(dx, dxp.c)
 
 
+class BnBwdStats:
+
+    def __init__(self, x_t, mean, rstd, mean_f, rstd_f, mask_mode: int, gneg: float, groups: int):
+        self.x_t, self.mean, self.rstd, self.mean_f, self.rstd_f = x_t, mean, rstd, mean_f, rstd_f
+        self.mask_mode, self.gneg, self.groups = int(mask_mode), float(gneg), int(groups)
+        self.partial, self.rows = None, 0
+
+
+def _bn_stats_arm(lib, d, res_mode: int, st: BnBwdStats, dx: torch.Tensor) -> None:
+    if (st.x_t.shape != dx.shape or st.x_t.dtype != dx.dtype or not st.x_t.is_contiguous() or dx.shape[0] % st.groups
+            or (st.mask_mode == 2 and (st.mean_f is None or st.rstd_f is None))):
+        return
+    rows = lib.cgan_conv2d_bwd_data_bn_stats_rows(C.byref(d), res_mode, st.groups, _stream())
+    if rows <= 0:
+        return
+    partial = _empty((st.groups * rows, dx.shape[3], 2), dtype=torch.float32, device=dx.device)
+    _lib.check(lib.cgan_conv2d_bwd_data_bn_stats_bind(
+        _stream(), _ptr(st.x_t), _ptr(st.mean), _ptr(st.rstd), _ptr(st.mean_f), _ptr(st.rstd_f), st.gneg, st.mask_mode,
+        st.groups, _ptr(partial), partial.numel() * 4), "cgan_conv2d_bwd_data_bn_stats_bind")
+    st.partial, st.rows = partial, rows
+
+
 def conv2d_bwd_data(dy: NHWC, w: torch.Tensor, x_shape, stride=1, pad=0, dilation=1,
                     sigma: Optional[torch.Tensor] = None, pad_mode=PAD_ZERO, add: Optional[NHWC] = None,
-                    prepacked: Optional[DgradPack] = None, relu_out: Optional[NHWC] = None) -> NHWC:
+                    prepacked: Optional[DgradPack] = None, relu_out: Optional[NHWC] = None,
+                    bn_stats: Optional[BnBwdStats] = None) -> NHWC:
     same = stride == 1 and pad_mode == PAD_ZERO and 2 * pad == dilation * (w.shape[2] - 1) and w.shape[2] == w.shape[3]
     if relu_out is not None:
         if not same:
@@ -1195,6 +1218,8 @@
         if add is not None:
             if add.t.shape != dx.shape or add.t.dtype != dx.dtype or not add.t.is_contiguous():
                 raise RuntimeError("conv2d_bwd_data: ``add`` %s does not match dx %s" % (tuple(add.t.shape), tuple(dx.shape)))
+            if bn_stats is not None:
+                _bn_stats_arm(lib, d, 3, bn_stats, dx)
             _lib.check(lib.cgan_conv2d_nhwc_bwd_data_add_relu(_ptr(dy.t), _ptr(packed), _ptr(add.t), _ptr(relu_out.t), _ptr(dx),
                                                               C.byref(d), _stream()), "cgan_conv2d_nhwc_bwd_data_add_relu")
             return NHWC(dx, c_in)
@@ -1204,9 +1229,13 @@
     if add is not None:
         if add.t.shape != dx.shape or add.t.dtype != dx.dtype or not add.t.is_contiguous():
             raise RuntimeError("conv2d_bwd_data: ``add`` %s does not match dx %s" % (tuple(add.t.shape), tuple(dx.shape)))
+        if bn_stats is not None:
+            _bn_stats_arm(lib, d, 1, bn_stats, dx)
         _lib.check(lib.cgan_conv2d_nhwc_bwd_data_add(_ptr(dy.t), _ptr(packed), _ptr(add.t), _ptr(dx), C.byref(d), _stream()),
                    "cgan_conv2d_nhwc_bwd_data_add")
         return NHWC(dx, c_in)
+    if bn_stats is not None:
+        _bn_stats_arm(lib, d, 0, bn_stats, dx)
     _lib.check(lib.cgan_conv2d_nhwc_bwd_data(_ptr(dy.t), _ptr(packed), _ptr(dx), C.byref(d), _stream()),
                "cgan_conv2d_nhwc_bwd_data")
     return NHWC(dx, c_in)
diff --git a/include/climategan_hip.h b/include/climategan_hip.h
--- a/include/climategan_hip.h
+++ b/include/climategan_hip.h
@@ -79,6 +79,10 @@
                                    const CganConvDesc* fwd, void* stream);
 int cgan_conv2d_nhwc_bwd_data_add_relu(const void* dy, const void* packed_w_dgrad, const void* dx_add, const void* relu_out,
                                        void* dx, const CganConvDesc* fwd, void* stream);
+int32_t cgan_conv2d_bwd_data_bn_stats_rows(const CganConvDesc* fwd, int32_t res_mode, int32_t groups, void* stream);
+int cgan_conv2d_bwd_data_bn_stats_bind(void* stream, const void* x, const float* mean, const float* rstd, const float* fmean,
+                                       const float* frstd, float gneg, int32_t mask_mode, int32_t groups, float* partial,
+                                       size_t partial_bytes);
 size_t cgan_conv2d_bwd_weight_workspace_bytes(const CganConvDesc* fwd);
 int cgan_conv2d_nhwc_bwd_weight(const void* x, const void* dy, float* dw_oihw, float* dbias, const CganConvDesc* fwd,
                                 void* workspace, size_t workspace_bytes,
@@ -219,6 +223,12 @@
                                    const float* fold_rstd, void* dx, float* dgamma, float* dbeta, void* dz_out,
                                    int32_t dtype, int64_t npix_total, int32_t c, int32_t groups, int32_t act,
                                    float act_slope, void* workspace, size_t workspace_bytes, void* stream);
+size_t cgan_batchnorm_act_bwd_from_partials_workspace_bytes(int32_t c, int32_t rows);
+int cgan_batchnorm_act_bwd_from_partials(const void* x, const void* dy, const float* partial, int32_t rows,
+                                         const float* batch_mean, const float* batch_rstd, const float* gamma,
+                                         const float* fold_mean, const float* fold_rstd, void* dx, float* dgamma,
+                                         float* dbeta, int32_t dtype, int64_t npix_total, int32_t c, int32_t groups,
+                                         int32_t act, float act_slope, void* workspace, size_t workspace_bytes, void* stream);
 int cgan_bce_logits_nhwc(const void* x, int32_t dtype, int64_t npix, int32_t c, float target, float weight,
                          float* loss_accum, void* dx, void* stream);
 int cgan_hinge_nhwc(const void* x, int32_t dtype, int64_t npix, int32_t c, int32_t target_is_real,
```

Result: no change. 57.60 (median of 3 runs) (+0.2%).
